# dot-comma-hyphen/oaxaca-blinder-rs

Hardware: NVIDIA B200
Metric: bootstrap_reps_per_sec (higher is better)
Workload: dtype f64

## Files before the change

### include/obboot.h

```cpp
#ifndef OBBOOT_H
#define OBBOOT_H
#include <stddef.h>
#include <stdint.h>

#ifdef __cplusplus
extern "C" {
#endif

#define OBBOOT_ABI_VERSION 6

typedef enum ob_status {
    OB_OK = 0,
    OB_ERR_POLARS = 1,
    OB_ERR_COLUMN_NOT_FOUND = 2,
    OB_ERR_INVALID_GROUP = 3,
    OB_ERR_NALGEBRA = 4,
    OB_ERR_DIAGNOSTIC = 5,
    OB_ERR_INSUFFICIENT_DATA = 6,
    OB_ERR_INVALID_ARG = 7,
    OB_ERR_CUDA = 8,
    OB_ERR_NCCL = 9,
    OB_ERR_NO_DEVICE = 10,
    OB_ERR_UNSUPPORTED = 11
} ob_status;
// ... 133 lines not shown
typedef enum { OB_CACHE_NONE = 0, OB_CACHE_FILLED = 1, OB_CACHE_OUTCOME_ONLY = 2, OB_CACHE_SOLVE_ONLY = 3 } ob_cache_use;
ob_status ob_gram_cache_create(ob_ctx* ctx, ob_gram_cache** out);
void ob_gram_cache_destroy(ob_gram_cache* c);
ob_status ob_gram_cache_last_use(const ob_gram_cache* c, int32_t* use, int64_t* bytes);
ob_status ob_bootstrap_run_cached(ob_ctx* ctx, const ob_design* design, const ob_boot_opts* opts, ob_gram_cache* cache,
                                  ob_result* res);

typedef struct ob_bayes_opts {
    const float* wt_a;
    const float* wt_b;
} ob_bayes_opts;
ob_status ob_bootstrap_run_bayes(ob_ctx* ctx, const ob_design* design, const ob_boot_opts* opts, const ob_bayes_opts* bayes,
                                 ob_gram_cache* cache, ob_result* res);

ob_status ob_reduce_stats(ob_ctx* ctx, const double* rep_stats, const int32_t* rep_status, int64_t reps, int32_t S,
                          const double* point_stats, int64_t* n_ok, double* std_err, double* p_value,
                          double* ci_lower, double* ci_upper, double* t_stat);

typedef struct ob_mm_opts {
    int32_t simulations;
    int32_t n_quantiles;
    const double* quantiles;
    int64_t reps;
    uint64_t seed;
    const uint32_t* idx_a;
    const uint32_t* idx_b;
    const double* taus;
    const uint32_t* draw_a;
    const uint32_t* draw_b;
    int64_t rep_begin;
    int64_t rep_end;
    int32_t skip_reduce;
    int32_t count_bits;
    int64_t max_workspace_bytes;
    int32_t shard_replicates;
} ob_mm_opts;

typedef struct ob_mm_result {
    double* point_stats;
    int64_t n_ok;
    double* std_err;
    double* p_value;
    double* ci_lower;
    double* ci_upper;
    double* t_stat;
    double* rep_stats;
    int32_t* rep_status;
    double* point_betas_a;
    double* point_betas_b;
    int32_t* point_qr_info_a;
    int32_t* point_qr_info_b;
    int64_t qr_total, qr_vertex, qr_approx, qr_failed, qr_iterations;
    double ms_counts, ms_qr, ms_effects, ms_reduce, ms_total;
    int32_t gpu_launches;
} ob_mm_result;

ob_status ob_mm_run(ob_ctx* ctx, const ob_design* design, const ob_mm_opts* opts, ob_mm_result* res);

#define OB_COMM_ID_BYTES 128
ob_status ob_replicate_shard(int64_t reps, int32_t world, int32_t rank, int64_t* rep_begin, int64_t* rep_end);
ob_status ob_comm_unique_id(uint8_t* id128);
ob_status ob_comm_init_nccl(ob_ctx* ctx, const uint8_t* id128, int32_t rank, int32_t world);
typedef struct ob_local_group ob_local_group;
ob_status ob_local_group_create(int32_t world, ob_local_group** out);
void ob_local_group_destroy(ob_local_group* group);
ob_status ob_comm_init_local(ob_ctx* ctx, ob_local_group* group, int32_t rank);
void ob_comm_destroy(ob_ctx* ctx);
ob_status ob_row_shard_plan(int64_t n_group, int32_t world, int32_t rank, int64_t* row_begin, int64_t* row_end);
ob_status ob_design_set_row_shard(ob_design* d, int64_t n_a_global, int64_t n_b_global, int32_t world, int32_t rank);

ob_status ob_design_allgather_rows(ob_ctx* ctx, const ob_design* local_slice, ob_design** out);

ob_status ob_design_row_shard(const ob_design* d, int64_t* n_a_global, int64_t* n_b_global, int32_t* world, int32_t* rank);

ob_status ob_design_redistribute_rows(ob_ctx* ctx, const ob_design* local_slice, ob_design** out);

int64_t ob_debug_gram_schedule(int32_t K, int64_t n_a, int64_t n_b, int64_t slots, int32_t world, int32_t rank, int32_t grid,
                               int64_t* out8, int64_t cap);

int64_t ob_debug_gram_columns(int32_t K, int32_t T, int32_t n_cont, const int32_t* cat_levels, int32_t n_cat,
                              uint16_t* pairs_out, int32_t* colmap_out, int64_t cap, int32_t* tiling_out);
int64_t ob_debug_gram_outcome_columns(int32_t K, int32_t T, uint16_t* pairs_out, int32_t* colmap_out, int64_t cap,
                                      int32_t* tiling_out);

ob_status ob_debug_counts(ob_ctx* ctx, const ob_design* d, uint64_t seed, int64_t rep, int32_t group,
                          uint16_t* counts_out);

ob_status ob_debug_bayes_weights(ob_ctx* ctx, const ob_design* d, uint64_t seed, int64_t rep, int32_t group, float* out);
ob_status ob_debug_counts_from_indices(ob_ctx* ctx, const ob_design* d, int32_t group, const uint32_t* idx, int64_t reps,
                                       int32_t count_bits, uint16_t* counts_out, int32_t* flags_out);

ob_status ob_debug_gram_cache_read(ob_ctx* ctx, const ob_gram_cache* c, int64_t* shape_out, double* xx_out, double* yy_out,
                                   int64_t* rows_out);

#ifdef __cplusplus
}
#endif
#endif
```

### oaxaca_blinder_rs_b200/csrc/api.cu

```cuda
#include "internal.h"

#include <algorithm>
#include <chrono>
#include <cmath>
#include <cstdio>
#include <cstring>
#include <exception>
#include <memory>
#include <atomic>
#include <mutex>
#include <optional>
#include <set>
#include <type_traits>

using namespace ob;

static constexpr int MAX_DESIGN_COLS = 280;

struct ob_ctx {
    int device = 0;
    int num_sms = 0;
    cudaStream_t stream = nullptr;
    cudaStream_t stream_side = nullptr;
    cudaStream_t stream_copy = nullptr;
    static constexpr int PACK_SLOTS = 8;
    int* h_pack_flags = nullptr;
    ob_design* pack_slot_owner[PACK_SLOTS] = {};
    unsigned pack_seq = 0;
    cudaMemPool_t pool = nullptr;
    cudaMemPool_t pool_pack = nullptr;
    cudaMemPool_t pool_design = nullptr;
    std::unique_ptr<Comm> comm;
    std::string err;
    std::mutex designs_mu;
    std::set<ob_design*> designs;
    std::set<ob_gram_cache*> caches;
};

struct ob_local_group { LocalGroup* g = nullptr; int world = 0; };

struct PendingPack;

struct ob_design {
    PendingPack* pending = nullptr;
    ob_status failed = OB_OK;
    std::string fail_msg;
    ob_ctx* owner = nullptr;
    cudaStream_t stream = nullptr;
    int device = 0;
    int K = 0, n_cont = 0, V = 0, ldx = 0;
    int T = 1;
    int K1 = 0;
    std::vector<int> cat_levels;
    bool weighted = false;
    int64_t n_frame = 0;
    int world = 1, rank = 0;
    double ms_h2d = 0.0, ms_pack = 0.0;
    GroupData g[2];
    int cl_strata = OB_CLUSTER_NONE;
    int64_t cl_units[2] = {0, 0};
    uint64_t id = 0, x_gen = 0, y_gen = 0;
};

struct ob_gram_cache {
    ob_ctx* owner = nullptr;
    int device = 0;
    int last_use = OB_CACHE_NONE;
    double* xx = nullptr; size_t xx_bytes = 0;
    double* yy = nullptr; size_t yy_bytes = 0;
    long long* rows = nullptr; size_t rows_bytes = 0;
    double* esum = nullptr; size_t esum_bytes = 0;
    bool xx_ok = false;
    uint64_t design_id = 0, x_gen = 0, seed = 0;
    int64_t reps = 0, rep_begin = 0, rep_end = 0, slots = 0;
    int shard_reps = 0, rep_world = 1, rep_rank = 0, row_world = 1, row_rank = 0, K = 0;
    int count_bytes = 1;
    bool bayes = false;
    bool y_ok = false;
    uint64_t y_gen = 0; int T = 0;
};

namespace {

thread_local ob_ctx* g_alloc_ctx = nullptr;
thread_local bool g_alloc_pack = false;

struct DevBuf {
    void* p = nullptr; size_t bytes = 0;
    ob_ctx* ctx = nullptr;
    bool pack = false;
    DevBuf() : ctx(g_alloc_ctx), pack(g_alloc_pack) {}
    explicit DevBuf(size_t b) : ctx(g_alloc_ctx), pack(g_alloc_pack) { alloc(b); }
    DevBuf(const DevBuf&) = delete;
    DevBuf& operator=(const DevBuf&) = delete;
    DevBuf(DevBuf&& o) noexcept : p(o.p), bytes(o.bytes), ctx(o.ctx), pack(o.pack) { o.p = nullptr; o.bytes = 0; }
    ~DevBuf() { release(); }
    void release() {
        if (p) { cudaFreeAsync(p, ctx->stream); p = nullptr; }
        bytes = 0;
    }
    void alloc(size_t b) {
        release();
        bytes = b;
        if (b) OB_CUDA(cudaMallocFromPoolAsync(&p, b, pack ? ctx->pool_pack : ctx->pool, ctx->stream));
    }
    template <typename T> T* as() const { return static_cast<T*>(p); }
};

struct StagedFrame {
    int64_t n = 0; int n_cont = 0, n_cat = 0;
    std::vector<DevBuf> cols, cats;
    DevBuf y, w, grp;
    bool weighted = false;
    double ms_h2d = 0.0;
};

}

struct PendingPack {
    StagedFrame sf;
    DevBuf d_bc, d_tot, d_flags, d_cont_ptrs, d_cat_ptrs, d_levels, d_dstart;
    std::vector<cudaEvent_t> chunk_done;
    int64_t ready_lo[2] = {0, 0};
    std::vector<int64_t> rows_ready[2];
    bool exchange_pending = false;
    DevBuf EX[2], Ew[2], Esrc[2];
    std::vector<size_t> ex_rows[2], ex_send_row[2], ex_recv_row[2];
    std::vector<long long> ex_frame_off;
    cudaEvent_t ev_begin = nullptr, ev_h2d_end = nullptr;
    int* h_flags = nullptr;
    int slot = -1;
    ~PendingPack() {
        for (cudaEvent_t e : chunk_done) cudaEventDestroy(e);
        if (ev_begin) cudaEventDestroy(ev_begin);
        if (ev_h2d_end) cudaEventDestroy(ev_h2d_end);
    }
};

namespace {

size_t pool_idle_bytes(ob_ctx* ctx) {
    unsigned long long reserved = 0, used = 0;
    cudaMemPoolGetAttribute(ctx->pool, cudaMemPoolAttrReservedMemCurrent, &reserved);
    cudaMemPoolGetAttribute(ctx->pool, cudaMemPoolAttrUsedMemCurrent, &used);
    return reserved > used ? (size_t)(reserved - used) : 0;
}

struct Timer {
    cudaEvent_t a, b; cudaStream_t st; double* acc;
    Timer(cudaStream_t s, double* accum) : st(s), acc(accum) {
        cudaEventCreate(&a); cudaEventCreate(&b); cudaEventRecord(a, st);
    }
    void stop() { cudaEventRecord(b, st); }
    void collect() { float ms = 0; cudaEventSynchronize(b); cudaEventElapsedTime(&ms, a, b); *acc += ms; }
    ~Timer() { cudaEventDestroy(a); cudaEventDestroy(b); }
};

struct Trace {
    bool on; std::chrono::steady_clock::time_point t0, last;
    Trace() : on(getenv("OBBOOT_TRACE") != nullptr), t0(std::chrono::steady_clock::now()), last(t0) {}
    void mark(const char* what, cudaStream_t st = nullptr, bool sync = false) {
        if (!on) return;
        if (sync) cudaStreamSynchronize(st);
        const auto now = std::chrono::steady_clock::now();
        fprintf(stderr, "[obboot] %-28s +%8.3f ms  (t = %9.3f ms)\n", what,
                std::chrono::duration<double, std::milli>(now - last).count(),
                std::chrono::duration<double, std::milli>(now - t0).count());
        last = now;
    }
};

template <typename F>
ob_status guarded(ob_ctx* ctx, F&& f) {
    try {
        if (ctx) OB_CUDA(cudaSetDevice(ctx->device));
        g_alloc_ctx = ctx;
        g_alloc_pack = false;
        f();
        return OB_OK;
    } catch (const CudaError& e) {
        if (ctx) {
            char buf[512];
            snprintf(buf, sizeof buf, "CUDA error: %s (%s) at %s:%d", cudaGetErrorString(e.code), e.what, e.file, e.line);
            ctx->err = buf;
        }
        cudaGetLastError();
        return (e.code == cudaErrorNoDevice || e.code == cudaErrorInsufficientDriver) ? OB_ERR_NO_DEVICE : OB_ERR_CUDA;
    } catch (const StatusError& e) {
        if (ctx) ctx->err = e.msg;
        return e.code;
    } catch (const std::bad_alloc&) {
        if (ctx) ctx->err = "host allocation failed";
        return OB_ERR_INVALID_ARG;
    }
}

[[noreturn]] void fail(ob_status c, const std::string& m) { throw StatusError{c, m}; }

void alloc_group(ob_ctx* ctx, GroupData& g, int64_t n, int ldx, bool weighted, bool zero_all = true) {
    cudaStream_t st = ctx->stream;
    g.n = n; g.n_pad = pad_rows(n);
    g.shard = row_shard(n, 0, 1);
    const size_t xbytes = sizeof(double) * (size_t)g.n_pad * ldx;
    const size_t tail_off = zero_all ? 0 : sizeof(double) * (size_t)n * ldx;
    OB_CUDA(cudaMallocFromPoolAsync((void**)&g.X, xbytes, ctx->pool_design, st));
    OB_CUDA(cudaMemsetAsync(reinterpret_cast<char*>(g.X) + tail_off, 0, xbytes - tail_off, st));
    if (weighted) {
        OB_CUDA(cudaMallocFromPoolAsync((void**)&g.w, sizeof(double) * (size_t)g.n_pad, ctx->pool_design, st));
        OB_CUDA(cudaMemsetAsync(g.w, 0, sizeof(double) * (size_t)g.n_pad, st));
        OB_CUDA(cudaMallocFromPoolAsync((void**)&g.Xs, xbytes, ctx->pool_design, st));
        OB_CUDA(cudaMemsetAsync(reinterpret_cast<char*>(g.Xs) + tail_off, 0, xbytes - tail_off, st));
    }
    OB_CUDA(cudaMallocFromPoolAsync((void**)&g.src, sizeof(uint32_t) * (size_t)g.n_pad, ctx->pool_design, st));
}

void design_register(ob_ctx* ctx, ob_design* d) {
    static std::atomic<uint64_t> next_id{0};
    d->id = ++next_id;
    d->owner = ctx;
    std::lock_guard<std::mutex> lk(ctx->designs_mu);
    ctx->designs.insert(d);
}

void design_release_device(ob_design* d) {
    cudaStream_t st = d->stream;
    for (auto& g : d->g) {
        if (g.X) cudaFreeAsync(g.X, st);
        if (g.w) cudaFreeAsync(g.w, st);
        if (g.Xs) cudaFreeAsync(g.Xs, st);
        if (g.src) cudaFreeAsync(g.src, st);
        if (g.y_raw) cudaFreeAsync(g.y_raw, st);
        if (g.hk_Z) cudaFreeAsync(g.hk_Z, st);
        if (g.hk_sel) cudaFreeAsync(g.hk_sel, st);
        if (g.hk_Xm) cudaFreeAsync(g.hk_Xm, st);
        if (g.uid) cudaFreeAsync(g.uid, st);
        g.X = g.w = g.Xs = g.y_raw = g.hk_Z = g.hk_Xm = nullptr; g.src = g.uid = nullptr; g.hk_sel = nullptr;
    }
}

void cache_release_device(ob_gram_cache* c) {
    if (c->owner) {
        cudaStream_t st = c->owner->stream;
        if (c->xx) cudaFreeAsync(c->xx, st);
        if (c->yy) cudaFreeAsync(c->yy, st);
        if (c->rows) cudaFreeAsync(c->rows, st);
        if (c->esum) cudaFreeAsync(c->esum, st);
    }
    c->xx = c->yy = nullptr; c->rows = nullptr; c->esum = nullptr; c->xx_bytes = c->yy_bytes = c->rows_bytes = c->esum_bytes = 0;
    c->xx_ok = c->y_ok = false;
}

void pending_exchange(ob_design* d) {
    PendingPack* P = d->pending;
    if (!P || !P->exchange_pending) return;
    ob_ctx* ctx = d->owner;
    Comm* comm = ctx->comm.get();
    if (!comm) fail(OB_ERR_NCCL, "the communicator of an asynchronous row-shard pack was destroyed before its exchange");
    cudaStream_t st = ctx->stream;
    const int world = comm->world, me = comm->rank;
    OB_CUDA(cudaStreamWaitEvent(st, P->chunk_done.back(), 0));
    for (int g = 0; g < 2; ++g) {
        GroupData& G = d->g[g];
        auto exchange = [&](const void* sendbuf, void* recvbuf, size_t row_bytes) {
            std::vector<size_t> b(P->ex_rows[g].size()), so((size_t)world), ro((size_t)world);
            for (size_t i = 0; i < b.size(); ++i) b[i] = P->ex_rows[g][i] * row_bytes;
            for (int r = 0; r < world; ++r) { so[r] = P->ex_send_row[g][r] * row_bytes; ro[r] = P->ex_recv_row[g][r] * row_bytes; }
            comm->alltoallv(sendbuf, so.data(), recvbuf, ro.data(), b.data(), st);
        };
        exchange(P->EX[g].p, G.X, sizeof(double) * (size_t)d->ldx);
        if (d->weighted) exchange(P->Ew[g].p, G.w, sizeof(double));
        exchange(P->Esrc[g].p, G.src, sizeof(uint32_t));
        for (int r = 0; r < world; ++r) {
            const int64_t rows = (int64_t)P->ex_rows[g][(size_t)r * world + me];
            if (!rows) continue;
            scale_rows_range_launch(G, d->ldx, (int64_t)P->ex_recv_row[g][r], rows, st);
        }
    }
    OB_CUDA(cudaStreamSynchronize(st));
    P->exchange_pending = false;
}

void pending_finish(ob_design* d, bool quiet = false) {
    PendingPack* P = d->pending;
    if (!P) return;
    ob_ctx* ctx = d->owner;
    if (P->exchange_pending && ctx && !quiet) pending_exchange(d);
    d->pending = nullptr;
    cudaEvent_t last = P->chunk_done.back();
    if (ctx) cudaStreamWaitEvent(ctx->stream, last, 0);
    const cudaError_t e = cudaEventSynchronize(last);
    float ms_all = 0, ms_h2d = 0;
    cudaEventElapsedTime(&ms_all, P->ev_begin, last);
    cudaEventElapsedTime(&ms_h2d, P->ev_begin, P->ev_h2d_end);
    d->ms_h2d = ms_h2d; d->ms_pack = ms_all - ms_h2d;
    const int f0 = P->h_flags[0], f1 = P->h_flags[1];
    if (ctx && P->slot >= 0 && ctx->pack_slot_owner[P->slot] == d) ctx->pack_slot_owner[P->slot] = nullptr;
    g_alloc_ctx = ctx;
    const auto t_del = std::chrono::steady_clock::now();
    delete P;
    if (getenv("OBBOOT_TRACE"))
        fprintf(stderr, "[obboot] async pack: staging released in %.3f ms (host)\n",
                std::chrono::duration<double, std::milli>(std::chrono::steady_clock::now() - t_del).count());
    if (e != cudaSuccess) { d->failed = OB_ERR_CUDA; d->fail_msg = std::string("asynchronous pack failed: ") + cudaGetErrorString(e); }
    else if (f0) { d->failed = OB_ERR_INVALID_GROUP; d->fail_msg = "Invalid group variable: Weights cannot be negative"; }
    else if (f1) { d->failed = OB_ERR_INVALID_ARG; d->fail_msg = "categorical code outside [0, levels)"; }
    if (d->failed != OB_OK && !quiet) fail(d->failed, d->fail_msg);
}

void design_alive(const ob_design* d) {
    if (!d->owner) fail(OB_ERR_INVALID_ARG, "this design's context has been destroyed (designs die with their context)");
    if (d->failed != OB_OK) fail(d->failed, d->fail_msg);
}

void design_ready(const ob_design* d) {
    design_alive(d);
    pending_finish(const_cast<ob_design*>(d));
}

const char* status_text(int s) {
    switch (s) {
    case OB_ERR_INVALID_GROUP: return "Invalid group variable: No data in groups for weighted coefficients.";
    case OB_ERR_NALGEBRA: return "Nalgebra error: Failed to perform Cholesky decomposition. Matrix may be singular or not positive definite due to multicollinearity.";
    case OB_ERR_INSUFFICIENT_DATA: return "Insufficient data: Insufficient data for OLS calculation: n_obs must be strictly greater than k";
    default: return "error";
    }
}


struct RepRange {
    bool shard_reps; int64_t rb, re, nrep;
    bool index_mode; int count_bytes;
};

template <typename Opts>
RepRange replicate_range(const ob_ctx* ctx, const ob_design* d, const Opts* o) {
    if (o->reps < 0) fail(OB_ERR_INVALID_ARG, "negative reps");
    RepRange r;
    r.shard_reps = o->shard_replicates != 0 && ctx->comm && ctx->comm->world > 1;
    if (r.shard_reps && (o->rep_begin != 0 || o->rep_end != 0 || o->skip_reduce))
        fail(OB_ERR_INVALID_ARG, "shard_replicates computes the shard itself: rep_begin / rep_end / skip_reduce must be 0");
    r.rb = o->rep_begin; r.re = o->rep_end > 0 ? o->rep_end : o->reps;
    if (r.rb < 0 || r.re < r.rb || r.re > o->reps) fail(OB_ERR_INVALID_ARG, "bad replicate shard");
    r.nrep = r.re - r.rb;
    r.index_mode = o->idx_a != nullptr || o->idx_b != nullptr;
    if (d->cl_strata == OB_CLUSTER_JOINT) {
        if (o->idx_b) fail(OB_ERR_INVALID_ARG, "a JOINT cluster design takes one unit stream: idx_a [reps x M] and idx_b = NULL");
    } else if (r.index_mode && r.nrep > 0 && (!o->idx_a || !o->idx_b)) fail(OB_ERR_INVALID_ARG, "index stream needs both idx_a and idx_b");
    if (o->count_bits != 0 && o->count_bits != 8 && o->count_bits != 16) fail(OB_ERR_INVALID_ARG, "count_bits must be 0, 8 or 16");
    if (o->count_bits == 16 && !gram_fits(d->ldx, 2)) fail(OB_ERR_UNSUPPORTED, "16-bit multiplicities need K + outcomes <= 268");
    r.count_bytes = o->count_bits == 16 ? 2 : 1;
    return r;
}

struct Batch {
    int64_t pn, slot_lo, slot_hi, bslots;
    int first_slot;
    int64_t brep;
    int64_t rep0;
    Batch(int64_t p0, int64_t ppb, int64_t panels_total, int64_t slots, int64_t rb)
        : pn(std::min(ppb, panels_total - p0)), slot_lo(p0 * BM), slot_hi(std::min(slots, (p0 + pn) * BM)),
          bslots(slot_hi - slot_lo), first_slot(p0 == 0 ? 1 : 0), brep(bslots - first_slot), rep0(rb + slot_lo - 1) {}
    int tail_mi() const {
        const int64_t last = bslots - (pn - 1) * BM;
        return (int)std::min<int64_t>(16, ((last + 7) / 8 + 3) / 4 * 4);
    }
};

struct ClusterWork {
    DevBuf U[2];
    long long* rows = nullptr;
};
int unit_mats(const ob_design* d) { return d->cl_strata == OB_CLUSTER_JOINT ? 1 : 2; }

template <typename Opts>
int generate_counts(const ob_design* d, const Opts* o, const Batch& b, int count_bytes, int64_t ppb, DevBuf (&C)[2],
                    DevBuf (&idx)[2], DevBuf& colsum, DevBuf& lut, int* flags, Comm* row_comm, double* ms_comm, cudaStream_t st,
                    ClusterWork* cw = nullptr) {
    CountsArgs ca[2];
    const int mats = cw ? unit_mats(d) : 2;
    for (int g = 0; g < mats; ++g) {
        const GroupData& G = d->g[g];
        ca[g].C = C[g].p; ca[g].count_bytes = count_bytes; ca[g].n = G.n; ca[g].n_pad = G.n_pad;
        ca[g].n_global = G.shard.n_global; ca[g].row_begin = G.shard.row_begin;
        ca[g].panels = (int)b.pn; ca[g].slots = b.bslots; ca[g].first_slot = b.first_slot; ca[g].rep0 = b.rep0;
        ca[g].group = g; ca[g].seed = o->seed;
        if (cw) {
            const int64_t M = d->cl_units[g];
            ca[g].C = cw->U[g].p; ca[g].n = ca[g].n_global = M; ca[g].n_pad = pad_rows(M); ca[g].row_begin = 0;
            ca[g].group = mats == 1 ? 2 : g;
        }
    }
    int launches = 0;
    auto expand = [&] {
        if (!cw) return;
        OB_CUDA(cudaMemsetAsync(cw->rows, 0, sizeof(long long) * 2 * (size_t)b.pn * BM, st));
        for (int g = 0; g < 2; ++g) {
            const int m = mats == 1 ? 0 : g;
            ExpandArgs ea{C[g].p, cw->U[m].p, d->g[g].uid, count_bytes, d->g[g].n, d->g[g].n_pad, pad_rows(d->cl_units[m]),
                          (int)b.pn, b.bslots, cw->rows + (size_t)g * b.pn * BM};
            counts_expand_launch(ea, st);
            launches += 1;
        }
    };
    if (o->idx_a || o->idx_b) {
        for (int g = 0; g < mats; ++g) {
            const uint32_t* h = g == 0 ? o->idx_a : o->idx_b;
            const int64_t n_glob = ca[g].n_global;
            const size_t nb = sizeof(uint32_t) * (size_t)std::max<int64_t>(b.brep, 1) * n_glob;
            if (idx[g].bytes < nb) idx[g].alloc(nb);
            if (b.brep > 0)
                OB_CUDA(cudaMemcpyAsync(idx[g].p, h + (size_t)(b.rep0 + b.first_slot) * n_glob,
                                        sizeof(uint32_t) * (size_t)b.brep * n_glob, cudaMemcpyHostToDevice, st));
            counts_from_indices(ca[g], idx[g].as<uint32_t>(), flags, st);
            launches += 1 + (b.brep > 0 ? (int)((b.brep + 32767) / 32768) : 0);
        }
        expand();
        return launches;
    }
    long long* sums[2] = {colsum.as<long long>(), colsum.as<long long>() + (size_t)ppb * BM};
    OB_CUDA(cudaMemsetAsync(colsum.p, 0, colsum.bytes, st));
    for (int g = 0; g < mats; ++g) {
        counts_philox_body_launch(ca[g], sums[g], lut.as<unsigned char>() + (size_t)g * counts_lut_bytes(), st);
        launches += 2;
    }
    if (row_comm) {
        Timer t_c(st, ms_comm);
        row_comm->allreduce(colsum.p, 2 * (size_t)ppb * BM, CommDType::I64, CommOp::SUM, st);
        t_c.stop(); OB_CUDA(cudaStreamSynchronize(st)); t_c.collect();
    }
    for (int g = 0; g < mats; ++g) {
        counts_philox_fixup_launch(ca[g], sums[g], flags, st);
        launches += b.brep > 0 ? 1 : 0;
    }
    expand();
    return launches;
}

struct BayesWork {
    DevBuf wt[2], part, esum, esum_local, gathered;
    int ranks_with_rows[2];
};
int generate_weights(const ob_design* d, const ob_boot_opts* o, const ob_bayes_opts* bo, const Batch& b, DevBuf (&C)[2],
                     BayesWork& w, int* flags, Comm* row_comm, double* ms_comm, cudaStream_t st) {
    const int64_t spad = b.pn * BM;
    int segs[2];
    int64_t leaf0 = 0;
    for (int g = 0; g < 2; ++g) {
        const GroupData& G = d->g[g];
        BayesArgs a;
        a.C = C[g].as<float>(); a.n = G.n; a.n_pad = G.n_pad; a.panels = (int)b.pn;
        a.n_global = G.shard.n_global; a.row_begin = G.shard.row_begin;
        a.slots = b.bslots; a.first_slot = b.first_slot; a.rep0 = b.rep0; a.group = g; a.seed = o->seed;
        a.segs = segs[g] = G.shard.leaf_hi - G.shard.leaf_lo; a.seg_rows = G.shard.seg_rows;
        a.wt = nullptr; a.flags = flags;
        a.part = w.part.as<double>() + (size_t)leaf0 * spad;
        leaf0 += a.segs;
        const float* h = bo ? (g == 0 ? bo->wt_a : bo->wt_b) : nullptr;
        if (h) {
            const size_t nb = sizeof(float) * (size_t)std::max<int64_t>(b.brep, 1) * a.n_global;
            if (w.wt[g].bytes < nb) w.wt[g].alloc(nb);
            if (b.brep > 0)
                OB_CUDA(cudaMemcpyAsync(w.wt[g].p, h + (size_t)(b.rep0 + b.first_slot) * a.n_global,
                                        sizeof(float) * (size_t)b.brep * a.n_global, cudaMemcpyHostToDevice, st));
            a.wt = w.wt[g].as<float>();
        }
// ... 1417 lines not shown
            if (rr.shard_reps) {
                Comm* cm = ctx->comm.get();
                ma.betas = allgather_shards(cm, nprob, (size_t)K, d_betas.as<double>() + (size_t)ma.p_begin * K, d_betas_all, st);
                ma.info = allgather_shards(cm, nprob, 1, d_info.as<int>() + ma.p_begin, d_info_all, st);
            }
            Timer t_eff(st, &res->ms_effects);
            mm_effects_launch(ma, d_rows_a.as<uint32_t>(), d_rows_b.as<uint32_t>(), nq, d_q.as<double>(), d_stats.as<double>() + (size_t)b.slot_lo * S,
                              d_status.as<int>() + b.slot_lo, nullptr, st);
            res->gpu_launches += 1;
            t_eff.stop();
            int flags[4];
            h_info.resize((size_t)2 * bslots * sims);
            OB_CUDA(cudaMemcpyAsync(flags, d_flags.p, sizeof flags, cudaMemcpyDeviceToHost, st));
            OB_CUDA(cudaMemcpyAsync(h_info.data(), ma.info, sizeof(int) * h_info.size(), cudaMemcpyDeviceToHost, st));
            if (p0 == 0 && (res->point_betas_a || res->point_betas_b)) {
                h_pbetas.resize((size_t)2 * sims * K);
                OB_CUDA(cudaMemcpyAsync(h_pbetas.data(), ma.betas, sizeof(double) * h_pbetas.size(), cudaMemcpyDeviceToHost, st));
            }
            OB_CUDA(cudaStreamSynchronize(st));
            t_counts.collect(); t_qr.collect(); t_eff.collect();
            saturated = check_batch_flags(flags, count_bytes, o->count_bits, d->ldx);
            if (saturated) break;
            if (p0 == 0 && (res->point_betas_a || res->point_betas_b))
                for (int s_ = 0; s_ < sims; ++s_) {
                    if (res->point_betas_a) memcpy(res->point_betas_a + (size_t)s_ * K, h_pbetas.data() + ((size_t)2 * s_ + 0) * K, sizeof(double) * (size_t)K);
                    if (res->point_betas_b) memcpy(res->point_betas_b + (size_t)s_ * K, h_pbetas.data() + ((size_t)2 * s_ + 1) * K, sizeof(double) * (size_t)K);
                }
            for (size_t i = 0; i < h_info.size(); ++i) {
                const int st_ = h_info[i] & 0xff;
                ++res->qr_total;
                if (st_ == 0) ++res->qr_vertex; else if (st_ == 1) ++res->qr_approx; else ++res->qr_failed;
                res->qr_iterations += (h_info[i] >> 8) & 0xff;
            }
            if (p0 == 0)
                for (int s_ = 0; s_ < sims; ++s_) {
                    if (res->point_qr_info_a) res->point_qr_info_a[s_] = h_info[(size_t)2 * s_];
                    if (res->point_qr_info_b) res->point_qr_info_b[s_] = h_info[(size_t)2 * s_ + 1];
                }
        }
        if (!saturated) break;
        count_bytes = 2;
        res->ms_counts = res->ms_qr = res->ms_effects = 0.0;
        res->qr_total = res->qr_vertex = res->qr_approx = res->qr_failed = res->qr_iterations = 0;
    }
    int point_status = 0;
    OB_CUDA(cudaMemcpyAsync(&point_status, d_status.p, sizeof(int), cudaMemcpyDeviceToHost, st));
    OB_CUDA(cudaStreamSynchronize(st));
    if (point_status != OB_OK)
        fail(OB_ERR_NALGEBRA, "Nalgebra error: Failed to estimate a sufficient number of quantile regressions.");
    };
    agree_on_status(rr.shard_reps ? ctx->comm.get() : nullptr, st, run_batches, "another rank of the replicate-sharded run failed");
    if (res->point_stats) OB_CUDA(cudaMemcpyAsync(res->point_stats, d_stats.p, sizeof(double) * S, cudaMemcpyDeviceToHost, st));
    const int64_t reps_all = rr.nrep;
    const double* stats_rows = d_stats.as<double>() + S;
    const int* status_rows = d_status.as<int>() + 1;
    if (!o->skip_reduce) {
        double* dst[5] = {res->std_err, res->p_value, res->ci_lower, res->ci_upper, res->t_stat};
        reduce_to_host(st, stats_rows, status_rows, reps_all, S, d_stats.as<double>(), dst, &res->n_ok, &res->ms_reduce);
        res->gpu_launches += 1;
    }
    if (reps_all > 0) {
        if (res->rep_stats) OB_CUDA(cudaMemcpyAsync(res->rep_stats, stats_rows, sizeof(double) * (size_t)reps_all * S, cudaMemcpyDeviceToHost, st));
        if (res->rep_status) OB_CUDA(cudaMemcpyAsync(res->rep_status, status_rows, sizeof(int) * (size_t)reps_all, cudaMemcpyDeviceToHost, st));
    }
    t_total.stop();
    OB_CUDA(cudaStreamSynchronize(st));
    t_total.collect();
}

}

extern "C" {

ob_status ob_mm_run(ob_ctx* ctx, const ob_design* d, const ob_mm_opts* o, ob_mm_result* res) {
    if (!ctx || !d || !o || !res) return OB_ERR_INVALID_ARG;
    return guarded(ctx, [&] {
        design_ready(d);
        if (d->cl_strata != OB_CLUSTER_NONE)
            fail(OB_ERR_UNSUPPORTED, "Machado-Mata on a clustered design: its row draws assume constant group sizes (detach the clusters)");
        mm_run(ctx, d, o, res);
    });
}

static void bootstrap_body(ob_ctx* ctx, const ob_design* d, const ob_boot_opts* o, ob_gram_cache* cache, ob_result* res,
                           bool bayes = false, const ob_bayes_opts* bo = nullptr) {
        design_alive(d);
        const bool bayes_explicit = bayes && bo && (bo->wt_a || bo->wt_b);
        if (bayes) {
            if (d->cl_strata != OB_CLUSTER_NONE)
                fail(OB_ERR_UNSUPPORTED, "Bayesian bootstrap on a clustered design: cluster weights are not built (detach the clusters)");
            if (d->K1 > 0)
                fail(OB_ERR_UNSUPPORTED, "Bayesian bootstrap on a design with a selection equation: the Heckman estimator is not built for it");
            if (o->idx_a || o->idx_b)
                fail(OB_ERR_INVALID_ARG, "the Bayesian bootstrap takes no index stream (idx_a / idx_b must be NULL; explicit weights go in ob_bayes_opts)");
            if (o->count_bits != 0) fail(OB_ERR_INVALID_ARG, "the Bayesian bootstrap has fp32 weights: count_bits must be 0");
            if (!gram_fits(d->ldx, 4))
                fail(OB_ERR_UNSUPPORTED, "design too wide for the Bayesian bootstrap: K + outcomes <= 236 with fp32 weights");
            if (cache && bayes_explicit)
                fail(OB_ERR_UNSUPPORTED, "a Gram cache needs the native weight stream (explicit weight streams cannot be keyed)");
        }
        if (cache && d->K1 > 0) fail(OB_ERR_UNSUPPORTED, "a Gram cache does not apply to designs with a selection equation (Heckman)");
        if (cache && (o->idx_a || o->idx_b)) fail(OB_ERR_UNSUPPORTED, "a Gram cache needs the native resampling stream (explicit index streams cannot be keyed)");
        if (d->K1 > 0) {
            design_ready(d);
            heckman_run(ctx, d, o, res);
            return;
        }
        cudaStream_t st = ctx->stream;
        const int K = d->K, T = d->T;
        const bool clustered = d->cl_strata != OB_CLUSTER_NONE;
        if (clustered && d->world > 1)
            fail(OB_ERR_UNSUPPORTED, "clusters on a row-sharded design (mode N): a unit's rows may sit on several ranks");
        if (o->ref_kind < 0 || o->ref_kind > 3) fail(OB_ERR_INVALID_ARG, "ref_kind out of range");
        if (o->n_norm < 0) fail(OB_ERR_INVALID_ARG, "negative n_norm");
        RepRange rr = replicate_range(ctx, d, o);
        if (o->shard_replicates && d->world > 1) fail(OB_ERR_INVALID_ARG, "shard_replicates on a row-sharded design (its communicator shards rows)");
        if (rr.shard_reps) { ob_replicate_shard(o->reps, ctx->comm->world, ctx->comm->rank, &rr.rb, &rr.re); rr.nrep = rr.re - rr.rb; }
        if (d->g[0].shard.n_global == 0 || d->g[1].shard.n_global == 0) fail(OB_ERR_INVALID_GROUP, "Invalid group variable: One group has no data");
        Comm* comm = d->world > 1 ? ctx->comm.get() : nullptr;
        if (d->world > 1 && (!comm || comm->world != d->world || comm->rank != d->rank))
            fail(OB_ERR_NCCL, "row-sharded design needs ob_comm_init_* on this context with the same world/rank");
        const int world = d->world;
        int n_base = 0, n_idx = 0;
        int mode = OB_CACHE_NONE;
        const int rep_world = rr.shard_reps ? ctx->comm->world : 1, rep_rank = rr.shard_reps ? ctx->comm->rank : 0;
        if (cache) {
            const bool xx_hit = cache->xx_ok && cache->design_id == d->id && cache->x_gen == d->x_gen && cache->seed == o->seed &&
                                cache->reps == o->reps && cache->rep_begin == rr.rb && cache->rep_end == rr.re &&
                                cache->shard_reps == (rr.shard_reps ? 1 : 0) && cache->rep_world == rep_world && cache->rep_rank == rep_rank &&
                                cache->row_world == d->world && cache->row_rank == d->rank && cache->K == d->K && cache->bayes == bayes &&
                                !(o->count_bits == 8 && cache->count_bytes == 2);
            mode = !xx_hit ? OB_CACHE_FILLED : (cache->y_ok && cache->y_gen == d->y_gen && cache->T == d->T) ? OB_CACHE_SOLVE_ONLY
                                                                                                           : OB_CACHE_OUTCOME_ONLY;
            if (Comm* ac = rr.shard_reps ? ctx->comm.get() : comm) mode = allreduce_scalar(ac, mode, CommOp::MIN, st);
        }
        const bool solve_only = mode == OB_CACHE_SOLVE_ONLY, outcome_only = mode == OB_CACHE_OUTCOME_ONLY;
        for (int v = 0; v < o->n_norm; ++v) {
            n_base += o->norm_has_base[v] ? 1 : 0;
            if (o->norm_off[v + 1] < o->norm_off[v]) fail(OB_ERR_INVALID_ARG, "norm_off not monotone");
        }
        if (o->n_norm) n_idx = o->norm_off[o->n_norm];
        for (int t = 0; t < n_idx; ++t)
            if (o->norm_idx[t] < 0 || o->norm_idx[t] >= K) fail(OB_ERR_INVALID_ARG, "norm_idx outside the design");
        const int D = K + n_base, S = 5 + 2 * D;
        const int SE = T * S, KE = T * K;
        int count_bytes = bayes ? 4 : rr.count_bytes;
        if (outcome_only && o->count_bits == 0) count_bytes = cache->count_bytes;
        if (bayes && rr.nrep > 0 && bayes_explicit && (!bo->wt_a || !bo->wt_b))
            fail(OB_ERR_INVALID_ARG, "an explicit weight stream needs both wt_a and wt_b");

        res->ms_counts = res->ms_gram = res->ms_solve = res->ms_reduce = res->ms_total = res->ms_gram_kernel = res->ms_comm = 0.0;
        res->gpu_launches = 0;
        res->n_ok = 0;
        Timer t_total(st, &res->ms_total);
        Trace tr;

        const int nn = std::max(o->n_norm, 1);
        DevBuf d_nm(sizeof(int) * nn), d_noff(sizeof(int) * (nn + 1)), d_nidx(sizeof(int) * std::max(n_idx, 1)), d_nhb(sizeof(int) * nn);
        if (o->n_norm) {
            OB_CUDA(cudaMemcpyAsync(d_nm.p, o->norm_m, sizeof(int) * o->n_norm, cudaMemcpyHostToDevice, st));
            OB_CUDA(cudaMemcpyAsync(d_noff.p, o->norm_off, sizeof(int) * (o->n_norm + 1), cudaMemcpyHostToDevice, st));
            if (n_idx) OB_CUDA(cudaMemcpyAsync(d_nidx.p, o->norm_idx, sizeof(int) * n_idx, cudaMemcpyHostToDevice, st));
            OB_CUDA(cudaMemcpyAsync(d_nhb.p, o->norm_has_base, sizeof(int) * o->n_norm, cudaMemcpyHostToDevice, st));
        }

        const int64_t slots = 1 + rr.nrep;
        const bool want_beta = res->rep_beta_a || res->rep_beta_b || res->beta_a || res->beta_b;
        DevBuf d_stats(sizeof(double) * (size_t)slots * SE), d_status(sizeof(int) * (size_t)slots);
        DevBuf d_ba(want_beta ? sizeof(double) * (size_t)slots * KE : 0), d_bb(want_beta ? sizeof(double) * (size_t)slots * KE : 0);
        const size_t PE = 5 * (size_t)K + 1;
        DevBuf d_point(sizeof(double) * PE * T);
        DevBuf d_flags(sizeof(int) * 4);

        const int nx = gram_cache_xx_cells(K), ny = gram_cache_y_cells(K, T);
        size_t cache_new_bytes = 0;
        if (mode == OB_CACHE_FILLED) {
            cache_release_device(cache);
            cache->xx_bytes = sizeof(double) * 2 * (size_t)slots * nx;
            OB_CUDA(cudaMallocFromPoolAsync((void**)&cache->xx, cache->xx_bytes, ctx->pool_design, st));
            cache_new_bytes += cache->xx_bytes;
            if (clustered) {
                cache->rows_bytes = sizeof(long long) * 2 * (size_t)slots;
                OB_CUDA(cudaMallocFromPoolAsync((void**)&cache->rows, cache->rows_bytes, ctx->pool_design, st));
                cache_new_bytes += cache->rows_bytes;
            }
            if (bayes) {
                cache->esum_bytes = sizeof(double) * 2 * (size_t)slots;
                OB_CUDA(cudaMallocFromPoolAsync((void**)&cache->esum, cache->esum_bytes, ctx->pool_design, st));
                cache_new_bytes += cache->esum_bytes;
            }
        }
        if (mode == OB_CACHE_FILLED || outcome_only) {
            cache->y_ok = false;
            const size_t yb = sizeof(double) * 2 * (size_t)slots * ny;
            if (cache->yy_bytes != yb) {
                if (cache->yy) cudaFreeAsync(cache->yy, st);
                cache->yy = nullptr; cache->yy_bytes = yb;
                OB_CUDA(cudaMallocFromPoolAsync((void**)&cache->yy, yb, ctx->pool_design, st));
                cache_new_bytes += yb;
            }
        }

        const GramColumns gcols = solve_only ? GramColumns() : outcome_only ? gram_outcome_columns(K, T)
                                                                              : gram_columns(K, T, d->n_cont, d->cat_levels);
        const int ntiles = gcols.ntiles;
        const int Pld = gram_pld(K, T);
        const int64_t panels_total = (slots + BM - 1) / BM;
        const int64_t n_pad[2] = {d->g[0].n_pad, d->g[1].n_pad};
        const int64_t n_glob[2] = {d->g[0].shard.n_global, d->g[1].shard.n_global};
        const int mats = clustered ? unit_mats(d) : 0;
        int64_t u_pad_all = 0;
        for (int m = 0; m < mats; ++m) u_pad_all += pad_rows(d->cl_units[m]);
        const int64_t idx_len = clustered ? d->cl_units[0] + (mats == 2 ? d->cl_units[1] : 0) : n_glob[0] + n_glob[1];
        int ranks_with_rows[2];
        for (int g = 0; g < 2; ++g)
            ranks_with_rows[g] = (d->g[g].shard.segs + d->g[g].shard.leaf_span - 1) / d->g[g].shard.leaf_span;
        const int64_t local_leaves = (int64_t)(d->g[0].shard.leaf_hi - d->g[0].shard.leaf_lo) +
                                     (d->g[1].shard.leaf_hi - d->g[1].shard.leaf_lo);
        auto per_panel_bytes = [&](int cb) {
            double cl = clustered ? (solve_only ? 0.0 : (double)u_pad_all * BM * cb) + 2.0 * BM * 8.0 : 0.0;
            if (bayes)
                cl = 2.0 * BM * 8.0 + (solve_only ? 0.0 : (double)local_leaves * BM * 8.0 + (comm ? world + 1 : 0) * 2.0 * BM * 8.0 +
                                                          (bayes_explicit ? (double)(n_glob[0] + n_glob[1]) * BM * 4.0 : 0.0));
            if (solve_only) return 2.0 * BM * Pld * 8.0 + cl;
            return (double)(n_pad[0] + n_pad[1]) * BM * cb + (rr.index_mode ? (double)idx_len * BM * 4.0 : 0.0) +
                   2.0 * BM * Pld * 8.0 * (comm ? world + 2 : 1) + (double)local_leaves * ntiles * (BM * BN * 8.0) + 2.0 * BM * 8.0 + cl;
        };
        double budget = (double)o->max_workspace_bytes - (double)cache_new_bytes;
        if (o->max_workspace_bytes <= 0) {
            const double idle = (double)pool_idle_bytes(ctx);
            const double need_all = per_panel_bytes(count_bytes) * (double)panels_total;
            if (idle >= 1.02 * need_all) budget = 1.01 * need_all;
            else {
                size_t free_b = 0, total_b = 0;
                OB_CUDA(cudaMemGetInfo(&free_b, &total_b));
                budget = 0.6 * ((double)free_b + idle) - (double)cache_new_bytes;
            }
        }
        DevBuf d_lut(2 * counts_lut_bytes());

        std::vector<double> point(PE * T);
        cudaEvent_t ev_point = nullptr;
        struct EvGuard { cudaEvent_t& e; ~EvGuard() { if (e) cudaEventDestroy(e); } } ev_point_guard{ev_point};
        OB_CUDA(cudaEventCreateWithFlags(&ev_point, cudaEventDisableTiming));
        auto run_batches = [&] {
        for (int attempt = 0; attempt < 2; ++attempt) {
            const double per_panel = per_panel_bytes(count_bytes);
            int64_t ppb = (int64_t)std::floor(budget / per_panel);
            ppb = std::max<int64_t>(1, std::min<int64_t>(ppb, panels_total));
            if (comm) ppb = allreduce_scalar(comm, (long long)ppb, CommOp::MIN, st);
            tr.mark("setup", st, true);
            DevBuf d_C[2], d_idx[2], d_colsum, d_gram, d_gram_local, d_gathered, d_rows;
            ClusterWork cw;
            BayesWork bw;
            bw.ranks_with_rows[0] = ranks_with_rows[0]; bw.ranks_with_rows[1] = ranks_with_rows[1];
            const size_t gram_elems = 2 * (size_t)ppb * BM * Pld;
            bool saturated = false;
            GramPlan plan; int64_t plan_panels = -1;
            DevBuf d_partials, d_pairs, d_colmap, d_cmap;
            auto allocate_workspace = [&] {
                if (!solve_only) {
                    if (!bayes) d_colsum.alloc(sizeof(long long) * 2 * (size_t)ppb * BM);
                    for (int g = 0; g < 2; ++g) d_C[g].alloc((size_t)ppb * n_pad[g] * BM * count_bytes);
                    for (int m = 0; m < mats; ++m) cw.U[m].alloc((size_t)ppb * pad_rows(d->cl_units[m]) * BM * count_bytes);
                }
                if (clustered) { d_rows.alloc(sizeof(long long) * 2 * (size_t)ppb * BM); cw.rows = d_rows.as<long long>(); }
                if (bayes) {
                    bw.esum.alloc(sizeof(double) * 2 * (size_t)ppb * BM);
                    if (!solve_only) bw.part.alloc(sizeof(double) * (size_t)std::max<int64_t>(local_leaves, 1) * ppb * BM);
                    if (!solve_only && comm) { bw.esum_local.alloc(sizeof(double) * 2 * (size_t)ppb * BM); bw.gathered.alloc(sizeof(double) * 2 * (size_t)ppb * BM * world); }
                }
                d_gram.alloc(sizeof(double) * gram_elems);
                if (cache) {
                    const std::vector<int32_t> cmap = gram_cache_map(K, T);
                    d_cmap.alloc(sizeof(int32_t) * cmap.size());
                    OB_CUDA(cudaMemcpyAsync(d_cmap.p, cmap.data(), sizeof(int32_t) * cmap.size(), cudaMemcpyHostToDevice, st));
                }
                if (solve_only) { OB_CUDA(cudaStreamSynchronize(st)); return; }
                if (comm) { d_gram_local.alloc(sizeof(double) * gram_elems); d_gathered.alloc(sizeof(double) * gram_elems * world); }
                plan = gram_make_plan(K, T, d->ldx, (int)std::min<int64_t>(ppb, panels_total), d->g, count_bytes, ctx->num_sms, gcols);
                plan_panels = plan.panels;
                d_partials.alloc(sizeof(double) * (size_t)std::max<int64_t>(plan.num_partials, 1) * BM * BN);
                d_pairs.alloc(sizeof(uint16_t) * gcols.pairs.size());
                d_colmap.alloc(sizeof(int32_t) * gcols.colmap.size());
                OB_CUDA(cudaMemcpyAsync(d_pairs.p, gcols.pairs.data(), sizeof(uint16_t) * gcols.pairs.size(), cudaMemcpyHostToDevice, st));
                OB_CUDA(cudaMemcpyAsync(d_colmap.p, gcols.colmap.data(), sizeof(int32_t) * gcols.colmap.size(), cudaMemcpyHostToDevice, st));
                OB_CUDA(cudaStreamSynchronize(st));
            };
            agree_on_status(comm, st, allocate_workspace, "another rank of the row-sharded run could not allocate its workspace");

            tr.mark("workspace + pair table", st, true);
            for (int64_t p0 = 0; p0 < panels_total && !saturated; p0 += ppb) {
                const Batch b(p0, ppb, panels_total, slots, rr.rb);
                const int64_t pn = b.pn, bslots = b.bslots;
                OB_CUDA(cudaMemsetAsync(d_flags.p, 0, sizeof(int) * 4, st));

                Timer t_counts(st, &res->ms_counts);
                if (!solve_only && bayes)
                    res->gpu_launches += generate_weights(d, o, bo, b, d_C, bw, d_flags.as<int>(), comm, &res->ms_comm, st);
                else if (!solve_only)
                    res->gpu_launches += generate_counts(d, o, b, count_bytes, ppb, d_C, d_idx, d_colsum, d_lut, d_flags.as<int>(), comm,
                                                         &res->ms_comm, st, clustered ? &cw : nullptr);
                t_counts.stop();
                tr.mark("counts", st, true);

                if (!solve_only && plan_panels != pn) {
                    plan = gram_make_plan(K, T, d->ldx, (int)pn, d->g, count_bytes, ctx->num_sms, gcols);
                    plan_panels = pn;
                    d_partials.alloc(sizeof(double) * (size_t)std::max<int64_t>(plan.num_partials, 1) * BM * BN);
                }
                Timer t_gram(st, &res->ms_gram);
                GramArgs ga;
                for (int g = 0; g < 2; ++g) { ga.X[g] = d->g[g].gram_operand(); ga.C[g] = d_C[g].p; }
                ga.count_bytes = count_bytes; ga.partials = d_partials.as<double>();
                ga.d_pairs = d_pairs.as<uint16_t>(); ga.d_colmap = d_colmap.as<int32_t>();
                ga.gram = comm ? d_gram_local.as<double>() : d_gram.as<double>();
                ga.tail_mi = b.tail_mi();
                struct EventPair {
                    cudaEvent_t a = nullptr, b = nullptr;
                    EventPair() { OB_CUDA(cudaEventCreate(&a)); OB_CUDA(cudaEventCreate(&b)); }
                    ~EventPair() { if (a) cudaEventDestroy(a); if (b) cudaEventDestroy(b); }
                } ev;
                ob_design* dm = const_cast<ob_design*>(d);
                if (solve_only) {
                    OB_CUDA(cudaEventRecord(ev.a, st));
                    OB_CUDA(cudaMemsetAsync(d_gram.p, 0, sizeof(double) * 2 * (size_t)pn * BM * Pld, st));
                    OB_CUDA(cudaEventRecord(ev.b, st));
                } else if (PendingPack* P = dm->pending) {
                    int la[2] = {0, 0}, na[2] = {0, 0};
                    const bool split = P->chunk_done.size() > 1;
                    for (int g = 0; g < 2; ++g) {
                        if (!split || plan.segs[g] == 0) continue;
                        const int64_t sr = plan.seg_rows[g];
                        const int64_t lo = (P->ready_lo[g] + sr - 1) / sr, hi = std::min<int64_t>(plan.segs[g], P->rows_ready[g][0] / sr);
                        if (hi > lo) { la[g] = (int)lo; na[g] = (int)(hi - lo); }
                    }
                    EventPair evA, evB;
                    OB_CUDA(cudaEventRecord(ev.a, st));
                    if (na[0] + na[1] > 0) {
                        OB_CUDA(cudaStreamWaitEvent(st, P->chunk_done.front(), 0));
                        if (tr.on) OB_CUDA(cudaEventRecord(evA.a, st));
                        gram_launch_leaves(plan, ga, la, na, st);
                        if (tr.on) OB_CUDA(cudaEventRecord(evA.b, st));
                        res->gpu_launches += 1;
                    }
                    OB_CUDA(cudaStreamWaitEvent(st, P->chunk_done.back(), 0));
                    pending_exchange(dm);
                    if (tr.on) OB_CUDA(cudaEventRecord(evB.a, st));
                    {
                        int lo0[2] = {0, 0}, n0[2] = {na[0] ? la[0] : 0, na[1] ? la[1] : 0};
                        int lo1[2] = {la[0] + na[0], la[1] + na[1]}, n1[2] = {plan.segs[0] - lo1[0], plan.segs[1] - lo1[1]};
                        if (n0[0] + n0[1] > 0) { gram_launch_leaves(plan, ga, lo0, n0, st); res->gpu_launches += 1; }
                        gram_launch_leaves(plan, ga, lo1, n1, st);
                    }
                    OB_CUDA(cudaEventRecord(ev.b, st));
                    gram_reduce_launch(plan, ga, st);
                    res->gpu_launches += 2;
                    if (tr.on) {
                        OB_CUDA(cudaEventSynchronize(ev.b));
                        auto rel = [&](cudaEvent_t e) { float ms = -1.f; if (cudaEventElapsedTime(&ms, P->ev_begin, e) != cudaSuccess) { cudaGetLastError(); ms = -1.f; } return ms; };
                        fprintf(stderr, "[obboot] async pack (ms after its start): chunk 0 packed %.1f, upload done %.1f, all packed %.1f | "
                                        "first gram launch %.1f..%.1f (leaves %d+%d of %d+%d), rest %.1f..%.1f\n",
                                rel(P->chunk_done.front()), rel(P->ev_h2d_end), rel(P->chunk_done.back()), rel(evA.a), rel(evA.b), na[0], na[1],
                                plan.segs[0], plan.segs[1], rel(evB.a), rel(ev.b));
                    }
                    pending_finish(dm);
                } else {
                    gram_launch(plan, ga, st, ev.a, ev.b);
                    res->gpu_launches += 2;
                }
                t_gram.stop();
                tr.mark("gram", st, true);
                if (comm && !solve_only) {
                    Timer t_c(st, &res->ms_comm);
                    const size_t batch_elems = 2 * (size_t)pn * BM * Pld;
                    comm->allgather(d_gram_local.p, d_gathered.p, sizeof(double) * batch_elems, st);
                    gram_combine_launch(d_gathered.as<double>(), world, ranks_with_rows, (int64_t)pn * BM * Pld, d_gram.as<double>(), st);
                    res->gpu_launches += 1;
                    t_c.stop(); OB_CUDA(cudaStreamSynchronize(st)); t_c.collect();
                }
                if (cache) {
                    Timer t_cc(st, &res->ms_gram);
                    GramCacheCopy cc{d_gram.as<double>(), pn * BM, Pld, b.slot_lo, bslots, cache->xx, cache->yy, slots,
                                     d_cmap.as<int32_t>(), nx, ny, 0, nx + ny};
                    for (int g = 0; clustered && g < 2 && (mode == OB_CACHE_FILLED || solve_only); ++g) {
                        long long* batch_rows = d_rows.as<long long>() + (size_t)g * pn * BM;
                        long long* kept = cache->rows + (size_t)g * slots + b.slot_lo;
                        OB_CUDA(cudaMemcpyAsync(solve_only ? batch_rows : kept, solve_only ? kept : batch_rows, sizeof(long long) * (size_t)bslots,
                                                cudaMemcpyDeviceToDevice, st));
                    }
                    for (int g = 0; bayes && g < 2 && (mode == OB_CACHE_FILLED || solve_only); ++g) {
                        double* batch_esum = bw.esum.as<double>() + (size_t)g * pn * BM;
                        double* kept = cache->esum + (size_t)g * slots + b.slot_lo;
                        OB_CUDA(cudaMemcpyAsync(solve_only ? batch_esum : kept, solve_only ? kept : batch_esum, sizeof(double) * (size_t)bslots,
                                                cudaMemcpyDeviceToDevice, st));
                    }
                    if (mode == OB_CACHE_FILLED) gram_cache_extract_launch(cc, st);
                    else if (solve_only) gram_cache_assemble_launch(cc, st);
                    else {
                        cc.c_hi = nx; gram_cache_assemble_launch(cc, st);
                        cc.c_lo = nx; cc.c_hi = nx + ny; gram_cache_extract_launch(cc, st);
                        res->gpu_launches += 1;
                    }
                    res->gpu_launches += 1;
                    t_cc.stop(); OB_CUDA(cudaStreamSynchronize(st)); t_cc.collect();
                }

                Timer t_solve(st, &res->ms_solve);
                SolveArgs sa;
                sa.gram = d_gram.as<double>(); sa.slots_pad = pn * BM; sa.Pld = Pld; sa.slots = bslots;
                sa.K = K; sa.n_cont = d->n_cont; sa.ref_kind = o->ref_kind; sa.T = T;
                sa.n_norm = o->n_norm; sa.d_norm_m = d_nm.as<int>(); sa.d_norm_off = d_noff.as<int>();
                sa.d_norm_idx = d_nidx.as<int>(); sa.d_norm_has_base = d_nhb.as<int>();
                sa.n_base = n_base; sa.S = S; sa.weighted = d->weighted ? 1 : 0;
                sa.na = (double)n_glob[0]; sa.nb = (double)n_glob[1];
                sa.rows = clustered ? d_rows.as<long long>() : nullptr;
                sa.esum = bayes ? bw.esum.as<double>() : nullptr;
                sa.stats = d_stats.as<double>() + (size_t)b.slot_lo * SE;
                sa.status = d_status.as<int>() + b.slot_lo;
                sa.beta_a = want_beta ? d_ba.as<double>() + (size_t)b.slot_lo * KE : nullptr;
                sa.beta_b = want_beta ? d_bb.as<double>() + (size_t)b.slot_lo * KE : nullptr;
                sa.point_extra = (p0 == 0) ? d_point.as<double>() : nullptr;
                DevBuf d_solve_scratch(solve_scratch_bytes(K, o->ref_kind == OB_REF_POOLED, o->n_norm, T, bslots));
                sa.scratch = d_solve_scratch.as<double>();
                solve_launch(sa, st);
                res->gpu_launches += 1;
                t_solve.stop();

                if (comm) comm->allreduce(d_flags.p, 4, CommDType::I32, CommOp::MAX, st);
                int flags[4];
                OB_CUDA(cudaMemcpyAsync(flags, d_flags.p, sizeof flags, cudaMemcpyDeviceToHost, st));
                OB_CUDA(cudaStreamSynchronize(st));
                tr.mark("solve + flags", st, false);
                t_counts.collect(); t_gram.collect(); t_solve.collect();
                { float ms = 0; cudaEventElapsedTime(&ms, ev.a, ev.b); res->ms_gram_kernel += ms; }
                saturated = check_batch_flags(flags, count_bytes, o->count_bits, d->ldx);
            }
            if (!saturated) break;
            count_bytes = 2;
            res->ms_counts = res->ms_gram = res->ms_solve = res->ms_gram_kernel = res->ms_comm = 0.0;
        }

        tr.mark("batches done (buffers freed)", st, true);
        int point_status = 0;
        OB_CUDA(cudaMemcpyAsync(&point_status, d_status.p, sizeof(int), cudaMemcpyDeviceToHost, st));
        OB_CUDA(cudaMemcpyAsync(point.data(), d_point.p, sizeof(double) * point.size(), cudaMemcpyDeviceToHost, st));
        OB_CUDA(cudaStreamSynchronize(st));
        if (point_status != OB_OK) fail((ob_status)point_status, status_text(point_status));
        };

        agree_on_status(rr.shard_reps ? ctx->comm.get() : nullptr, st, run_batches, "another rank of the replicate-sharded run failed");
        if (cache) {
            if (mode == OB_CACHE_FILLED) {
                cache->design_id = d->id; cache->x_gen = d->x_gen; cache->seed = o->seed;
                cache->reps = o->reps; cache->rep_begin = rr.rb; cache->rep_end = rr.re; cache->slots = slots;
                cache->shard_reps = rr.shard_reps ? 1 : 0; cache->rep_world = rep_world; cache->rep_rank = rep_rank;
                cache->row_world = d->world; cache->row_rank = d->rank; cache->K = K; cache->count_bytes = count_bytes;
                cache->bayes = bayes;
                cache->xx_ok = true;
            }
            if (!solve_only) { cache->y_gen = d->y_gen; cache->T = T; cache->y_ok = true; }
            cache->last_use = mode;
        }
        res->total_gap = point[5 * K];
        if (res->xa_mean) memcpy(res->xa_mean, point.data(), sizeof(double) * K);
        if (res->xb_mean) memcpy(res->xb_mean, point.data() + K, sizeof(double) * K);
        for (int t = 0; t < T; ++t) {
            if (res->beta_star) memcpy(res->beta_star + (size_t)t * K, point.data() + t * PE + 2 * K, sizeof(double) * K);
            if (res->total_gap_multi) res->total_gap_multi[t] = point[t * PE + 5 * K];
        }

        DevBuf d_res;
        struct SideJoin { cudaStream_t s; bool armed = false; ~SideJoin() { if (armed) cudaStreamSynchronize(s); } } side_join{ctx->stream_side};
        if (res->residuals_b) {
            side_join.armed = true;
            d_res.alloc(sizeof(double) * (size_t)std::max<int64_t>(d->g[1].n, 1) * T);
            cudaStream_t s2 = ctx->stream_side;
            OB_CUDA(cudaEventRecord(ev_point, st));
            OB_CUDA(cudaStreamWaitEvent(s2, ev_point, 0));
            for (int t = 0; t < T; ++t)
                residuals_launch(d->g[1], K, K + t, d->ldx, d_point.as<double>() + t * PE + 4 * K, d_res.as<double>() + (size_t)t * d->g[1].n, s2);
            res->gpu_launches += T;
            if (d->g[1].n) OB_CUDA(cudaMemcpyAsync(res->residuals_b, d_res.p, sizeof(double) * (size_t)d->g[1].n * T, cudaMemcpyDeviceToHost, s2));
        }
        if (res->point_stats) OB_CUDA(cudaMemcpyAsync(res->point_stats, d_stats.p, sizeof(double) * SE, cudaMemcpyDeviceToHost, st));
        if (res->beta_a) OB_CUDA(cudaMemcpyAsync(res->beta_a, d_ba.p, sizeof(double) * KE, cudaMemcpyDeviceToHost, st));
        if (res->beta_b) OB_CUDA(cudaMemcpyAsync(res->beta_b, d_bb.p, sizeof(double) * KE, cudaMemcpyDeviceToHost, st));
        tr.mark("point + residuals queued", st, false);

        const int64_t reps_all = rr.shard_reps ? o->reps : rr.nrep;
        DevBuf d_gstats, d_gstatus, d_gba, d_gbb;
        const double* stats_rows = d_stats.as<double>() + SE;
        const int* status_rows = d_status.as<int>() + 1;
        const double* ba_rows = want_beta ? d_ba.as<double>() + KE : nullptr;
        const double* bb_rows = want_beta ? d_bb.as<double>() + KE : nullptr;
        if (rr.shard_reps) {
            Timer t_c(st, &res->ms_comm);
            Comm* cm = ctx->comm.get();
            stats_rows = allgather_shards(cm, o->reps, SE, stats_rows, d_gstats, st);
            status_rows = allgather_shards(cm, o->reps, 1, status_rows, d_gstatus, st);
            if (res->rep_beta_a) ba_rows = allgather_shards(cm, o->reps, KE, ba_rows, d_gba, st);
            if (res->rep_beta_b) bb_rows = allgather_shards(cm, o->reps, KE, bb_rows, d_gbb, st);
            t_c.stop(); OB_CUDA(cudaStreamSynchronize(st)); t_c.collect();
            tr.mark("replicate all-gather", st, false);
        }

        if (!o->skip_reduce) {
            double* dst[5] = {res->std_err, res->p_value, res->ci_lower, res->ci_upper, res->t_stat};
            reduce_to_host(st, stats_rows, status_rows, reps_all, SE, d_stats.as<double>(), dst, &res->n_ok, &res->ms_reduce);
            res->gpu_launches += 1;
        }
        if (reps_all > 0) {
            if (res->rep_stats) OB_CUDA(cudaMemcpyAsync(res->rep_stats, stats_rows, sizeof(double) * (size_t)reps_all * SE, cudaMemcpyDeviceToHost, st));
            if (res->rep_status) OB_CUDA(cudaMemcpyAsync(res->rep_status, status_rows, sizeof(int) * (size_t)reps_all, cudaMemcpyDeviceToHost, st));
            if (res->rep_beta_a) OB_CUDA(cudaMemcpyAsync(res->rep_beta_a, ba_rows, sizeof(double) * (size_t)reps_all * KE, cudaMemcpyDeviceToHost, st));
            if (res->rep_beta_b) OB_CUDA(cudaMemcpyAsync(res->rep_beta_b, bb_rows, sizeof(double) * (size_t)reps_all * KE, cudaMemcpyDeviceToHost, st));
        }
        if (res->residuals_b) {
            OB_CUDA(cudaEventRecord(ev_point, ctx->stream_side));
            OB_CUDA(cudaStreamWaitEvent(st, ev_point, 0));
        }
        t_total.stop();
        OB_CUDA(cudaStreamSynchronize(st));
        t_total.collect();
        tr.mark("reduce + replicate D2H", st, false);
}

ob_status ob_bootstrap_run(ob_ctx* ctx, const ob_design* d, const ob_boot_opts* o, ob_result* res) {
    if (!ctx || !d || !o || !res) return OB_ERR_INVALID_ARG;
    return guarded(ctx, [&] { bootstrap_body(ctx, d, o, nullptr, res); });
}

ob_status ob_gram_cache_create(ob_ctx* ctx, ob_gram_cache** out) {
    if (!ctx || !out) return OB_ERR_INVALID_ARG;
    auto* c = new ob_gram_cache;
    c->owner = ctx; c->device = ctx->device;
    {
        std::lock_guard<std::mutex> lk(ctx->designs_mu);
        ctx->caches.insert(c);
    }
    *out = c;
// ... 29 lines not shown
        if (cache->owner != ctx) fail(OB_ERR_INVALID_ARG, "this Gram cache belongs to another context");
        try {
            bootstrap_body(ctx, d, o, cache, res);
        } catch (...) {
            cache_release_device(cache);
            cache->last_use = OB_CACHE_NONE;
            throw;
        }
    });
}

ob_status ob_bootstrap_run_bayes(ob_ctx* ctx, const ob_design* d, const ob_boot_opts* o, const ob_bayes_opts* bo,
                                 ob_gram_cache* cache, ob_result* res) {
    if (!ctx || !d || !o || !res) return OB_ERR_INVALID_ARG;
    return guarded(ctx, [&] {
        if (!cache) { bootstrap_body(ctx, d, o, nullptr, res, true, bo); return; }
        if (cache->owner != ctx) fail(OB_ERR_INVALID_ARG, "this Gram cache belongs to another context");
        try {
            bootstrap_body(ctx, d, o, cache, res, true, bo);
        } catch (...) {
            cache_release_device(cache);
            cache->last_use = OB_CACHE_NONE;
            throw;
        }
    });
}

ob_status ob_reduce_stats(ob_ctx* ctx, const double* rep_stats, const int32_t* rep_status, int64_t reps, int32_t S,
                          const double* point_stats, int64_t* n_ok, double* std_err, double* p_value,
                          double* ci_lower, double* ci_upper, double* t_stat) {
    if (!ctx || S < 1 || reps < 0 || !point_stats || (reps && (!rep_stats || !rep_status))) return OB_ERR_INVALID_ARG;
    return guarded(ctx, [&] {
        cudaStream_t st = ctx->stream;
        DevBuf d_stats(sizeof(double) * (size_t)std::max<int64_t>(reps, 1) * S), d_status(sizeof(int) * (size_t)std::max<int64_t>(reps, 1));
        DevBuf d_point(sizeof(double) * S);
        if (reps) {
            OB_CUDA(cudaMemcpyAsync(d_stats.p, rep_stats, sizeof(double) * (size_t)reps * S, cudaMemcpyHostToDevice, st));
            OB_CUDA(cudaMemcpyAsync(d_status.p, rep_status, sizeof(int) * (size_t)reps, cudaMemcpyHostToDevice, st));
        }
        OB_CUDA(cudaMemcpyAsync(d_point.p, point_stats, sizeof(double) * S, cudaMemcpyHostToDevice, st));
        double* dst[5] = {std_err, p_value, ci_lower, ci_upper, t_stat};
        reduce_to_host(st, d_stats.as<double>(), d_status.as<int>(), reps, S, d_point.as<double>(), dst, n_ok, nullptr);
    });
}

int64_t ob_debug_gram_columns(int32_t K, int32_t T, int32_t n_cont, const int32_t* cat_levels, int32_t n_cat,
                              uint16_t* pairs_out, int32_t* colmap_out, int64_t cap, int32_t* tiling_out) {
    if (K < 1 || T < 1 || n_cont < 0 || n_cat < 0 || (n_cat > 0 && !cat_levels) || K + T > 65535) return -1;
    const GramColumns gc = gram_columns(K, T, n_cont, std::vector<int>(cat_levels, cat_levels + n_cat));
    const int64_t len = (int64_t)gc.colmap.size();
    for (int64_t c = 0; c < len && c < cap; ++c) {
        if (pairs_out) { pairs_out[2 * c] = gc.pairs[2 * (size_t)c]; pairs_out[2 * c + 1] = gc.pairs[2 * (size_t)c + 1]; }
        if (colmap_out) colmap_out[c] = gc.colmap[(size_t)c];
    }
    if (tiling_out) { tiling_out[0] = gc.Pc; tiling_out[1] = gc.nfull; tiling_out[2] = gc.tail_q; }
    return len;
}

int64_t ob_debug_gram_outcome_columns(int32_t K, int32_t T, uint16_t* pairs_out, int32_t* colmap_out, int64_t cap,
                                      int32_t* tiling_out) {
    if (K < 1 || T < 1 || K + T > 65535) return -1;
    const GramColumns gc = gram_outcome_columns(K, T);
    const int64_t len = (int64_t)gc.colmap.size();
    for (int64_t c = 0; c < len && c < cap; ++c) {
        if (pairs_out) { pairs_out[2 * c] = gc.pairs[2 * (size_t)c]; pairs_out[2 * c + 1] = gc.pairs[2 * (size_t)c + 1]; }
        if (colmap_out) colmap_out[c] = gc.colmap[(size_t)c];
    }
    if (tiling_out) { tiling_out[0] = gc.Pc; tiling_out[1] = gc.nfull; tiling_out[2] = gc.tail_q; }
    return len;
}

int64_t ob_debug_gram_schedule(int32_t K, int64_t n_a, int64_t n_b, int64_t slots, int32_t world, int32_t rank, int32_t grid,
                               int64_t* out8, int64_t cap) {
    if (K < 1 || n_a < 0 || n_b < 0 || slots < 1 || world < 1 || (world & (world - 1)) || world > MAX_WORLD || rank < 0 ||
        rank >= world || grid < 1) return -1;
    GroupData gd[2];
    const int64_t ns[2] = {n_a, n_b};
    for (int g = 0; g < 2; ++g) {
        gd[g].shard = row_shard(ns[g], rank, world);
        gd[g].n = gd[g].shard.n_local; gd[g].n_pad = pad_rows(gd[g].n);
    }
    const int64_t panels = (slots + BM - 1) / BM;
    return gram_schedule_debug(K, (int)panels, slots - (panels - 1) * BM, gd, grid, out8, cap);
}

ob_status ob_debug_counts(ob_ctx* ctx, const ob_design* d, uint64_t seed, int64_t rep, int32_t group,
                          uint16_t* counts_out) {
    if (!ctx || !d || !counts_out || group < 0 || group > 1 || rep < 0) return OB_ERR_INVALID_ARG;
    return guarded(ctx, [&] {
        design_ready(d);
        cudaStream_t st = ctx->stream;
        const GroupData& G = d->g[group];
        DevBuf d_C((size_t)G.n_pad * BM * 2), d_colsum(sizeof(long long) * BM), d_flags(sizeof(int) * 4), d_lut(counts_lut_bytes());
        OB_CUDA(cudaMemsetAsync(d_flags.p, 0, sizeof(int) * 4, st));
        CountsArgs ca;
        ca.C = d_C.p; ca.count_bytes = 2; ca.n = G.n; ca.n_pad = G.n_pad; ca.panels = 1; ca.slots = 2;
        ca.first_slot = 1; ca.rep0 = rep - 1; ca.group = group; ca.seed = seed;
        ca.n_global = G.shard.n_global; ca.row_begin = G.shard.row_begin;
        if (d->world > 1) fail(OB_ERR_UNSUPPORTED, "ob_debug_counts on a row-sharded design");
        DevBuf d_U, d_rows;
        const int m = d->cl_strata == OB_CLUSTER_JOINT ? 0 : group;
        if (d->cl_strata != OB_CLUSTER_NONE) {
            const int64_t M = d->cl_units[m];
            d_U.alloc((size_t)pad_rows(M) * BM * 2);
            d_rows.alloc(sizeof(long long) * 2 * BM);
            ca.C = d_U.p; ca.n = ca.n_global = M; ca.n_pad = pad_rows(M); ca.row_begin = 0;
            ca.group = d->cl_strata == OB_CLUSTER_JOINT ? 2 : group;
        }
        OB_CUDA(cudaMemsetAsync(d_colsum.p, 0, d_colsum.bytes, st));
        counts_philox_body_launch(ca, d_colsum.as<long long>(), d_lut.as<unsigned char>(), st);
        counts_philox_fixup_launch(ca, d_colsum.as<long long>(), d_flags.as<int>(), st);
        if (d->cl_strata != OB_CLUSTER_NONE) {
            OB_CUDA(cudaMemsetAsync(d_rows.p, 0, d_rows.bytes, st));
            ExpandArgs ea{d_C.p, d_U.p, G.uid, 2, G.n, G.n_pad, ca.n_pad, 1, 2, d_rows.as<long long>()};
            counts_expand_launch(ea, st);
        }
        OB_CUDA(cudaMemcpy2DAsync(counts_out, sizeof(uint16_t), d_C.as<uint16_t>() + 1, sizeof(uint16_t) * BM,
                                  sizeof(uint16_t), (size_t)G.n, cudaMemcpyDeviceToHost, st));
        OB_CUDA(cudaStreamSynchronize(st));
    });
}

ob_status ob_debug_bayes_weights(ob_ctx* ctx, const ob_design* d, uint64_t seed, int64_t rep, int32_t group, float* out) {
    if (!ctx || !d || !out || group < 0 || group > 1 || rep < 0) return OB_ERR_INVALID_ARG;
    return guarded(ctx, [&] {
        design_ready(d);
        if (d->world > 1) fail(OB_ERR_UNSUPPORTED, "ob_debug_bayes_weights on a row-sharded design");
        cudaStream_t st = ctx->stream;
        const GroupData& G = d->g[group];
        const int segs = G.shard.leaf_hi - G.shard.leaf_lo;
        DevBuf d_C((size_t)G.n_pad * BM * sizeof(float)), d_part(sizeof(double) * (size_t)std::max(segs, 1) * BM);
        BayesArgs a;
        a.C = d_C.as<float>(); a.n = G.n; a.n_pad = G.n_pad; a.panels = 1;
        a.n_global = G.shard.n_global; a.row_begin = G.shard.row_begin;
        a.slots = 2; a.first_slot = 1; a.rep0 = rep - 1; a.group = group; a.seed = seed;
        a.segs = segs; a.seg_rows = G.shard.seg_rows; a.wt = nullptr; a.part = d_part.as<double>();
        bayes_weights_launch(a, st);
        OB_CUDA(cudaMemcpy2DAsync(out, sizeof(float), d_C.as<float>() + 1, sizeof(float) * BM, sizeof(float), (size_t)G.n,
                                  cudaMemcpyDeviceToHost, st));
        OB_CUDA(cudaStreamSynchronize(st));
    });
}

ob_status ob_debug_counts_from_indices(ob_ctx* ctx, const ob_design* d, int32_t group, const uint32_t* idx, int64_t reps,
                                       int32_t count_bits, uint16_t* counts_out, int32_t* flags_out) {
    if (!ctx || !d || !counts_out || group < 0 || group > 1 || reps < 0 || (reps && !idx) || (count_bits != 8 && count_bits != 16))
        return OB_ERR_INVALID_ARG;
    return guarded(ctx, [&] {
        design_ready(d);
        cudaStream_t st = ctx->stream;
        const GroupData& G = d->g[group];
        const int cb = count_bits / 8;
        const int64_t slots = 1 + reps, panels = (slots + BM - 1) / BM;
        const int64_t n_glob = G.shard.n_global;
        DevBuf d_C((size_t)panels * G.n_pad * BM * cb), d_flags(sizeof(int) * 4);
        DevBuf d_idx(sizeof(uint32_t) * (size_t)std::max<int64_t>(reps * n_glob, 1));
        OB_CUDA(cudaMemsetAsync(d_flags.p, 0, sizeof(int) * 4, st));
        if (reps) OB_CUDA(cudaMemcpyAsync(d_idx.p, idx, sizeof(uint32_t) * (size_t)reps * n_glob, cudaMemcpyHostToDevice, st));
        CountsArgs ca;
        ca.C = d_C.p; ca.count_bytes = cb; ca.n = G.n; ca.n_pad = G.n_pad; ca.panels = (int)panels; ca.slots = slots;
        ca.first_slot = 1; ca.rep0 = -1; ca.group = group; ca.seed = 0;
        ca.n_global = n_glob; ca.row_begin = G.shard.row_begin;
        counts_from_indices(ca, d_idx.as<uint32_t>(), d_flags.as<int>(), st);
        std::vector<uint8_t> h((size_t)panels * G.n_pad * BM * cb);
        int flags[4];
        OB_CUDA(cudaMemcpyAsync(h.data(), d_C.p, h.size(), cudaMemcpyDeviceToHost, st));
// ... 38 lines not shown
```

### oaxaca_blinder_rs_b200/csrc/gram.cu

```cuda
#include "common.cuh"
#include "internal.h"

#include <algorithm>
#include <cstdlib>
#include <type_traits>

namespace ob {

constexpr int LGS = 18;
constexpr int LDA2 = 148;
constexpr int A_TILE = KT * LDA2;

struct GramKernelParams {
    const double* X[2];
    const void* C[2];
    long long n_pad[2];
    int segs[2];
    int seg_lo[2], seg_n[2];
    int seg_rows[2];
    long long units0;
    long long units_total;
    int ldx, panels, ntiles;
    int nfull, tail_q;
    int tail_mi;
    double* partials;
    const uint16_t* pairs;
};

template <typename CountT>
__device__ __forceinline__ double count_to_f64(CountT c, const double* __restrict__ tab) {
    if constexpr (std::is_same<CountT, float>::value) {
        const uint32_t f = __float_as_uint(c);
        return __hiloint2double(f ? (int)((f >> 3) + (896u << 20)) : 0, (int)(f << 29));
    } else if constexpr (sizeof(CountT) == 1) {
        return tab[(unsigned)c];
    } else {
        return __hiloint2double(0x43300000, (int)(unsigned)c) - 4503599627370496.0;
    }
}

constexpr int WS_R = 3;
constexpr int WS_PRODUCER_WARPS = 4;
constexpr int WS_THREADS = GRAM_THREADS + 32 * WS_PRODUCER_WARPS;
#define OB_WS_CONSUMER_REGS 224
#define OB_WS_PRODUCER_REGS 56

struct GramUnit { const double* Xg; const void* Cg; double* out; int nstages, nt, mi, tq; };

__host__ __device__ __forceinline__ bool ws_decode(const GramKernelParams& p, long long i, int ldx, size_t count_bytes, GramUnit& u) {
    const int pt = p.tail_mi < 16 ? 1 : 0, pf = p.panels - pt;
    const long long segs01 = (long long)p.seg_n[0] + p.seg_n[1];
    const long long n0 = segs01 * pf * p.nfull, n1 = segs01 * pt * p.nfull;
    const long long n2 = p.tail_q ? segs01 * pf : 0, n3 = p.tail_q ? segs01 * pt : 0;
    if (i >= n0 + n1 + n2 + n3) return false;
    int np, p0, nt_cnt, nt0;
    if (i < n0) { np = pf; p0 = 0; nt_cnt = p.nfull; nt0 = 0; }
    else if ((i -= n0) < n1) { np = pt; p0 = pf; nt_cnt = p.nfull; nt0 = 0; }
    else if ((i -= n1) < n2) { np = pf; p0 = 0; nt_cnt = 1; nt0 = p.nfull; }
    else { i -= n2; np = pt; p0 = pf; nt_cnt = 1; nt0 = p.nfull; }
    const long long per_seg = (long long)np * nt_cnt;
    const long long g0 = (long long)p.seg_n[0] * per_seg;
    const int g = i >= g0 ? 1 : 0;
    const long long r = i - (g ? g0 : 0);
    const int sidx = (int)(r / per_seg);
    const long long r2 = r - (long long)sidx * per_seg;
    const int seg = (g ? p.seg_lo[1] : p.seg_lo[0]) + sidx;
    const int panel = p0 + (int)(r2 / nt_cnt), nt = nt0 + (int)(r2 % nt_cnt);
    const int segs = g ? p.segs[1] : p.segs[0], seg_rows = g ? p.seg_rows[1] : p.seg_rows[0];
    const long long n_pad = g ? p.n_pad[1] : p.n_pad[0];
    const long long row0 = (long long)seg * seg_rows;
    const long long row1 = row0 + seg_rows < n_pad ? row0 + seg_rows : n_pad;
    u.nstages = (int)((row1 - row0) / KT);
    u.nt = nt; u.tq = (p.tail_q && nt == p.nfull) ? p.tail_q : 4;
    u.mi = panel >= pf ? p.tail_mi : 16;
    u.Xg = (g ? p.X[1] : p.X[0]) + row0 * ldx;
    u.Cg = reinterpret_cast<const unsigned char*>(g ? p.C[1] : p.C[0]) + (((long long)panel * n_pad + row0) * BM) * (long long)count_bytes;
    u.out = p.partials + (size_t)((g ? p.units0 : 0) + ((long long)panel * segs + seg) * p.ntiles + nt) * (BM * BN);
    return true;
}

template <typename CountT, int LDXC, int NI, int MI, int R>
__device__ __forceinline__ void ws_consume_unit(const GramKernelParams& p, const GramUnit& u, const double* As, const double* Xs,
                                                uint64_t* full, uint64_t* ready, uint64_t* consumed, int ldx_rt, uint32_t& jc,
                                                int sub0, int tw) {
    constexpr int KSTEPS = KT / 4;
    const int lane = threadIdx.x & 31;
    const int lk = lane & 3, lg = lane >> 2;
    const int ldx = LDXC ? LDXC : ldx_rt;
    int oj[NI], ol[NI];
#pragma unroll
    for (int s = 0; s < NI; ++s) {
        const int col = u.nt * BN + (sub0 + s) * 8 + lg;
        const uint32_t pr = *reinterpret_cast<const uint32_t*>(p.pairs + 2 * col);
        oj[s] = pr & 0xFFFFu; ol[s] = pr >> 16;
    }
    double acc[MI][NI][2];
#pragma unroll
    for (int i = 0; i < MI; ++i)
#pragma unroll
        for (int s = 0; s < NI; ++s) { acc[i][s][0] = 0.0; acc[i][s][1] = 0.0; }

    for (int s = 0; s < u.nstages; ++s) {
        const uint32_t slot = jc % R, par = (jc / R) & 1u;
        mbar_wait(&full[slot], par);
        mbar_wait(&ready[slot], par);
        const double* abase = As + (size_t)slot * A_TILE + lk * LDA2 + lg * LGS;
        const double* xbase = Xs + (size_t)slot * KT * ldx + lk * ldx;
#pragma unroll
        for (int kk = 0; kk < KSTEPS; ++kk) {
            double a[MI], b[NI];
            const double* arow = abase + kk * 4 * LDA2;
            const double* xrow = xbase + kk * 4 * ldx;
#pragma unroll
            for (int i = 0; i < MI; i += 2) {
                const double2 v = *reinterpret_cast<const double2*>(arow + i);
                a[i] = v.x; a[i + 1] = v.y;
            }
#pragma unroll
            for (int t = 0; t < NI; ++t) b[t] = xrow[oj[t]] * xrow[ol[t]];
#pragma unroll
            for (int i = 0; i < MI; ++i)
#pragma unroll
                for (int t = 0; t < NI; ++t) dmma884(acc[i][t][0], acc[i][t][1], a[i], b[t]);
        }
        __syncwarp();
        if (lane == 0) mbar_arrive(&consumed[slot]);
        ++jc;
    }
#pragma unroll
    for (int i = 0; i < MI; ++i)
#pragma unroll
        for (int t = 0; t < NI; ++t) {
            const int m = i * 8 + lg, n = (sub0 + t) * 8 + 2 * lk;
            *reinterpret_cast<double2*>(u.out + m * tw + n) = make_double2(acc[i][t][0], acc[i][t][1]);
        }
}

template <typename CountT, int LDXC, int NI, int R>
__device__ __forceinline__ void ws_consume_dispatch(const GramKernelParams& p, const GramUnit& u, const double* As, const double* Xs,
                                                    uint64_t* full, uint64_t* ready, uint64_t* consumed, int ldx_rt, uint32_t& jc,
                                                    int sub0, int tw) {
    switch (u.mi) {
    case 4: ws_consume_unit<CountT, LDXC, NI, 4, R>(p, u, As, Xs, full, ready, consumed, ldx_rt, jc, sub0, tw); break;
    case 8: ws_consume_unit<CountT, LDXC, NI, 8, R>(p, u, As, Xs, full, ready, consumed, ldx_rt, jc, sub0, tw); break;
    case 12: ws_consume_unit<CountT, LDXC, NI, 12, R>(p, u, As, Xs, full, ready, consumed, ldx_rt, jc, sub0, tw); break;
    default: ws_consume_unit<CountT, LDXC, NI, 16, R>(p, u, As, Xs, full, ready, consumed, ldx_rt, jc, sub0, tw); break;
    }
}

template <int R>
__device__ __forceinline__ void ws_idle_unit(const GramUnit& u, uint64_t* full, uint64_t* consumed, uint32_t& jc) {
    const int lane = threadIdx.x & 31;
    for (int s = 0; s < u.nstages; ++s) {
        const uint32_t slot = jc % R, par = (jc / R) & 1u;
        mbar_wait(&full[slot], par);
        __syncwarp();
        if (lane == 0) mbar_arrive(&consumed[slot]);
        ++jc;
    }
}
// ... 57 lines not shown
        while (is_ok && ji < (uint32_t)R) issue_next();
        while (wi_ok) {
            const uint32_t slot = jw % R, par = (jw / R) & 1u;
            mbar_wait(&full[slot], par);
            {
                const CountT* src = Cr + (size_t)slot * KT * BM;
                double* dst = As + (size_t)slot * A_TILE;
#pragma unroll 4
                for (int it = lane; it < (KT / WS_PRODUCER_WARPS) * 8 * 8; it += 32) {
                    const int e = it >> 6, rem = it & 63, r = pw * (KT / WS_PRODUCER_WARPS) + (rem >> 3), lgq = rem & 7;
                    const CountT* sp = src + r * BM + lgq;
                    double2 o;
                    o.x = count_to_f64<CountT>(sp[e * 16], Tab);
                    o.y = count_to_f64<CountT>(sp[e * 16 + 8], Tab);
                    *reinterpret_cast<double2*>(dst + r * LDA2 + lgq * LGS + e * 2) = o;
                }
            }
            __syncwarp();
            if (lane == 0) mbar_arrive(&ready[slot]);
            ++jw;
            if (++wi_s == wi_u.nstages) { wi_s = 0; wi_i += gridDim.x; wi_ok = ws_decode(p, wi_i, ldx, sizeof(CountT), wi_u); }
            if (is_ok && ji <= jw + (uint32_t)(R - 2)) {
                const uint32_t prev = ji - R;
                if (pw == 0) mbar_wait(&consumed[prev % R], (prev / R) & 1u);
                issue_next();
            }
        }
    }
}

static constexpr size_t gram_ws_smem(int ldx, int count_bytes, int ring = WS_R) {
    return sizeof(double) * ((size_t)ring * A_TILE + 256 + (size_t)ring * KT * ldx) + (size_t)ring * KT * BM * count_bytes +
           sizeof(uint64_t) * 3 * ring;
}
constexpr size_t GRAM_SMEM_MAX = 227 * 1024;
constexpr int gram_ring_f32(int ldx) { return gram_ws_smem(ldx, 4, WS_R) <= GRAM_SMEM_MAX ? WS_R : 2; }

bool gram_fits(int ldx, int count_bytes) { return gram_ws_smem(ldx, count_bytes, 2) <= GRAM_SMEM_MAX; }

template <int LEN>
__device__ __forceinline__ double2 tree_sum(const double2* __restrict__ base, size_t stride, int lo, int cnt);

__device__ __noinline__ double2 tree_sum64_call(const double2* __restrict__ base, size_t stride, int lo, int cnt);

template <int LEN>
__device__ __forceinline__ double2 tree_sum(const double2* __restrict__ base, size_t stride, int lo, int cnt) {
    if constexpr (LEN == 1) {
        return base[(size_t)lo * stride];
    } else if constexpr (LEN == 128) {
        double2 a = tree_sum64_call(base, stride, lo, cnt);
        if (lo + 64 < cnt) {
            const double2 b = tree_sum64_call(base, stride, lo + 64, cnt);
            a.x += b.x; a.y += b.y;
        }
        return a;
    } else {
        double2 a = tree_sum<LEN / 2>(base, stride, lo, cnt);
        if (lo + LEN / 2 < cnt) {
            const double2 b = tree_sum<LEN / 2>(base, stride, lo + LEN / 2, cnt);
            a.x += b.x; a.y += b.y;
        }
        return a;
    }
}

__device__ __noinline__ double2 tree_sum64_call(const double2* __restrict__ base, size_t stride, int lo, int cnt) {
    return tree_sum<64>(base, stride, lo, cnt);
}

__device__ __forceinline__ double2 tree_sum_span(const double2* __restrict__ base, size_t stride, int cnt, int span) {
    switch (span) {
    case 256: return tree_sum<256>(base, stride, 0, cnt);
    case 128: return tree_sum<128>(base, stride, 0, cnt);
    case 64: return tree_sum<64>(base, stride, 0, cnt);
    case 32: return tree_sum<32>(base, stride, 0, cnt);
    case 16: return tree_sum<16>(base, stride, 0, cnt);
    case 8: return tree_sum<8>(base, stride, 0, cnt);
    case 4: return tree_sum<4>(base, stride, 0, cnt);
    case 2: return tree_sum<2>(base, stride, 0, cnt);
    default: return tree_sum<1>(base, stride, 0, cnt);
    }
}

__global__ void __launch_bounds__(256) gram_reduce_kernel(const double* __restrict__ partials, int segs0, int segs1,
                                                          double* __restrict__ gram, int panels, int ntiles, int span,
                                                          int Pld, int tail_q, const int32_t* __restrict__ colmap) {
    const int tile_id = blockIdx.x;
    const int tiles_g = panels * ntiles;
    const int g = tile_id / tiles_g, t = tile_id - g * tiles_g;
    const int panel = t / ntiles, nt = t - panel * ntiles;
    const int cnt = g ? segs1 : segs0;
    const size_t first = (g ? (size_t)tiles_g * segs0 : 0) + (size_t)panel * cnt * ntiles + nt;
    const size_t slots_pad = (size_t)panels * BM;
    const int tw = (tail_q && nt == ntiles - 1) ? tail_q * BQ : BN;
    for (int e = threadIdx.x + blockIdx.y * blockDim.x; e < BM * tw / 2; e += blockDim.x * gridDim.y) {
        double2 s = make_double2(0.0, 0.0);
        if (cnt > 0) s = tree_sum_span(reinterpret_cast<const double2*>(partials + first * (BM * BN)) + e, (size_t)ntiles * (BM * BN / 2), cnt, span);
        const int m = (2 * e) / tw, n = (2 * e) % tw;
        double* dst = gram + ((size_t)g * slots_pad + (size_t)panel * BM + m) * (size_t)Pld;
        const int c0 = colmap[nt * BN + n], c1 = colmap[nt * BN + n + 1];
        if (c0 >= 0) dst[c0] = s.x;
        if (c1 >= 0) dst[c1] = s.y;
    }
}

__global__ void __launch_bounds__(256) leaf_sum_kernel(const double* __restrict__ part, int segs0, int segs1, long long half,
                                                       int span, double* __restrict__ out) {
    for (long long e = (long long)blockIdx.x * blockDim.x + threadIdx.x; e < 2 * half; e += (long long)gridDim.x * blockDim.x) {
        const int g = e >= half ? 1 : 0;
        const int cnt = g ? segs1 : segs0;
        const double2* base = reinterpret_cast<const double2*>(part + (g ? (size_t)segs0 * 2 * half : 0)) + (e - (g ? half : 0));
        reinterpret_cast<double2*>(out)[e] = cnt > 0 ? tree_sum_span(base, (size_t)half, cnt, span) : make_double2(0.0, 0.0);
    }
}

__global__ void __launch_bounds__(256) gram_combine_kernel(const double* __restrict__ gathered, int world, int ranks0,
                                                           int ranks1, long long per_group2, double* __restrict__ gram) {
    const long long total = 2 * per_group2;
    for (long long e = (long long)blockIdx.x * blockDim.x + threadIdx.x; e < total; e += (long long)gridDim.x * blockDim.x) {
        const int g = e >= per_group2 ? 1 : 0;
        const int cnt = g ? ranks1 : ranks0;
        double2 s = make_double2(0.0, 0.0);
        if (cnt > 0) s = tree_sum_span(reinterpret_cast<const double2*>(gathered) + e, (size_t)total, cnt, world);
        reinterpret_cast<double2*>(gram)[e] = s;
    }
}

GramColumns gram_columns(int K, int T, int n_cont, const std::vector<int>& cat_levels) {
    std::vector<int> block((size_t)K, -1);
    {
        int64_t dummies = 0;
        for (int m : cat_levels) dummies += m > 1 ? m - 1 : 0;
        if (!cat_levels.empty() && 1 + (int64_t)n_cont + dummies == K) {
            int c = 1 + n_cont;
            for (size_t q = 0; q < cat_levels.size(); ++q)
                for (int lvl = 1; lvl < cat_levels[q]; ++lvl) block[(size_t)c++] = (int)q;
        }
    }
    GramColumns gc;
    std::vector<uint16_t> pj, pl; std::vector<int32_t> cm;
    for (int j = 0; j < K; ++j) {
        const int64_t base = pair_base(K, T, j);
        for (int l = j; l < K; ++l) {
            if (l > j && block[(size_t)j] >= 0 && block[(size_t)j] == block[(size_t)l]) continue;
            pj.push_back((uint16_t)j); pl.push_back((uint16_t)l); cm.push_back((int32_t)(base + (l - j)));
        }
        for (int o = 0; o < T; ++o) { pj.push_back((uint16_t)j); pl.push_back((uint16_t)(K + o)); cm.push_back((int32_t)(base + (K - j) + o)); }
    }
    pj.push_back((uint16_t)K); pl.push_back((uint16_t)K); cm.push_back((int32_t)(num_pairs(K, T) - 1));
    gc.Pc = (int)cm.size();
    gram_col_tiling(gc.Pc, gc.nfull, gc.tail_q);
    gc.ntiles = gc.nfull + (gc.tail_q > 0);
    const size_t cols = (size_t)gc.ntiles * BN;
    gc.pairs.assign(cols * 2, (uint16_t)K);
    gc.colmap.assign(cols, -1);
    for (size_t c = 0; c < cm.size(); ++c) { gc.pairs[2 * c] = pj[c]; gc.pairs[2 * c + 1] = pl[c]; gc.colmap[c] = cm[c]; }
    return gc;
}

GramColumns gram_outcome_columns(int K, int T) {
    GramColumns gc;
    std::vector<uint16_t> pj, pl; std::vector<int32_t> cm;
    for (int j = 0; j < K; ++j) {
        const int64_t base = pair_base(K, T, j);
        for (int o = 0; o < T; ++o) { pj.push_back((uint16_t)j); pl.push_back((uint16_t)(K + o)); cm.push_back((int32_t)(base + (K - j) + o)); }
    }
    pj.push_back((uint16_t)K); pl.push_back((uint16_t)K); cm.push_back((int32_t)(num_pairs(K, T) - 1));
    gc.Pc = (int)cm.size();
    gram_col_tiling(gc.Pc, gc.nfull, gc.tail_q);
    gc.ntiles = gc.nfull + (gc.tail_q > 0);
    const size_t cols = (size_t)gc.ntiles * BN;
    gc.pairs.assign(cols * 2, (uint16_t)K);
    gc.colmap.assign(cols, -1);
    for (size_t c = 0; c < cm.size(); ++c) { gc.pairs[2 * c] = pj[c]; gc.pairs[2 * c + 1] = pl[c]; gc.colmap[c] = cm[c]; }
    return gc;
}

std::vector<int32_t> gram_cache_map(int K, int T) {
    std::vector<int32_t> m;
    m.reserve((size_t)gram_cache_xx_cells(K) + gram_cache_y_cells(K, T));
    for (int j = 0; j < K; ++j)
        for (int l = j; l < K; ++l) m.push_back((int32_t)(pair_base(K, T, j) + (l - j)));
    for (int j = 0; j < K; ++j)
        for (int o = 0; o < T; ++o) m.push_back((int32_t)(pair_base(K, T, j) + (K - j) + o));
    m.push_back((int32_t)(num_pairs(K, T) - 1));
    return m;
}

template <bool TO_CACHE>
__device__ __forceinline__ void gram_cache_copy_cells(const GramCacheCopy& a) {
    const long long ncell = a.c_hi - a.c_lo, per_g = a.nslots * ncell, total = 2 * per_g;
    for (long long e = (long long)blockIdx.x * blockDim.x + threadIdx.x; e < total; e += (long long)gridDim.x * blockDim.x) {
        const int g = e >= per_g ? 1 : 0;
        const long long r = e - (g ? per_g : 0);
        const long long s = r / ncell;
        const int c = a.c_lo + (int)(r - s * ncell);
        double* gcell = a.gram + ((size_t)g * a.slots_pad + (size_t)s) * (size_t)a.Pld + a.map[c];
        const size_t slot = (size_t)g * a.cslots + (size_t)(a.slot_lo + s);
        double* ccell = c < a.nx ? a.xx + slot * a.nx + c : a.yy + slot * a.ny + (c - a.nx);
        if (TO_CACHE) *ccell = *gcell; else *gcell = *ccell;
    }
}
__global__ void __launch_bounds__(256) gram_cache_extract_kernel(const GramCacheCopy a) { gram_cache_copy_cells<true>(a); }
__global__ void __launch_bounds__(256) gram_cache_assemble_kernel(const GramCacheCopy a) { gram_cache_copy_cells<false>(a); }

static void gram_cache_copy(const GramCacheCopy& a, bool to_cache, cudaStream_t st) {
    const long long total = 2 * a.nslots * (long long)(a.c_hi - a.c_lo);
    if (total <= 0) return;
    const unsigned blocks = (unsigned)std::min<long long>((total + 255) / 256, 148 * 8);
    if (to_cache) gram_cache_extract_kernel<<<blocks, 256, 0, st>>>(a);
    else gram_cache_assemble_kernel<<<blocks, 256, 0, st>>>(a);
    OB_CUDA(cudaGetLastError());
}
void gram_cache_extract_launch(const GramCacheCopy& a, cudaStream_t st) { gram_cache_copy(a, true, st); }
void gram_cache_assemble_launch(const GramCacheCopy& a, cudaStream_t st) { gram_cache_copy(a, false, st); }

GramPlan gram_make_plan(int K, int T, int ldx, int panels, const GroupData gd[2], int count_bytes, int num_sms,
                        const GramColumns& cols) {
    GramPlan pl;
    pl.K = K; pl.T = T; pl.ldx = ldx; pl.panels = panels;
    pl.nfull = cols.nfull; pl.tail_q = cols.tail_q; pl.ntiles = cols.ntiles;
    pl.Pld = gram_pld(K, T);
    int64_t total = 0;
    pl.leaf_span = gd[0].shard.leaf_span;
    for (int g = 0; g < 2; ++g) {
        pl.n_pad[g] = gd[g].n_pad;
        pl.segs[g] = gd[g].shard.leaf_hi - gd[g].shard.leaf_lo;
        pl.seg_rows[g] = gd[g].shard.seg_rows;
        pl.units[g] = (int64_t)pl.segs[g] * panels * pl.ntiles;
        total += pl.units[g];
    }
    pl.grid = (int)std::min<int64_t>(num_sms, std::max<int64_t>(total, 1));
    pl.ring = gram_ws_smem(pl.ldx, count_bytes, WS_R) <= GRAM_SMEM_MAX ? WS_R : 2;
    pl.smem_bytes = gram_ws_smem(pl.ldx, count_bytes, pl.ring);
    pl.num_partials = (int64_t)total;
    return pl;
}

static GramKernelParams gram_params(const GramPlan& pl, const GramArgs& a, const int seg_lo[2], const int seg_n[2]) {
    GramKernelParams p;
    for (int g = 0; g < 2; ++g) {
        p.X[g] = a.X[g]; p.C[g] = a.C[g];
        p.n_pad[g] = pl.n_pad[g]; p.segs[g] = pl.segs[g]; p.seg_rows[g] = pl.seg_rows[g];
        p.seg_lo[g] = seg_lo ? seg_lo[g] : 0; p.seg_n[g] = seg_n ? seg_n[g] : pl.segs[g];
    }
    p.units0 = pl.units[0];
    p.units_total = pl.units[0] + pl.units[1];
    p.ldx = pl.ldx; p.panels = pl.panels; p.ntiles = pl.ntiles;
    p.nfull = pl.nfull; p.tail_q = pl.tail_q;
    p.partials = a.partials; p.pairs = a.d_pairs;
    p.tail_mi = a.tail_mi >= 1 && a.tail_mi <= 16 ? a.tail_mi : 16;
    return p;
}

void gram_launch_leaves(const GramPlan& pl, const GramArgs& a, const int seg_lo[2], const int seg_n[2], cudaStream_t st) {
    const GramKernelParams p = gram_params(pl, a, seg_lo, seg_n);
    const int64_t units = ((int64_t)p.seg_n[0] + p.seg_n[1]) * pl.panels * pl.ntiles;
    if (units <= 0) return;
    const int grid = (int)std::min<int64_t>(pl.grid, units);
    const size_t ws_smem = pl.smem_bytes;
    if (!gram_fits(pl.ldx, a.count_bytes))
        throw StatusError{OB_ERR_UNSUPPORTED, "design too wide for the Gram kernel's shared-memory ring (K + outcomes <= 280 with "
                                              "8-bit multiplicities, <= 268 with 16-bit, <= 236 with fp32 Bayesian weights)"};
    auto launch_ws = [&](auto kernel) {
        OB_CUDA(cudaFuncSetAttribute(kernel, cudaFuncAttributeMaxDynamicSharedMemorySize, (int)ws_smem));
        kernel<<<grid, WS_THREADS, ws_smem, st>>>(p);
    };
#define OB_GRAM_WS_CASE(L) case L: if (a.count_bytes == 4) launch_ws(gram_ws_kernel<float, L, gram_ring_f32(L)>); \
                                   else if (a.count_bytes == 1) launch_ws(gram_ws_kernel<uint8_t, L>); else launch_ws(gram_ws_kernel<uint16_t, L>); break;
    switch (pl.ldx) {
        OB_GRAM_WS_CASE(12) OB_GRAM_WS_CASE(20) OB_GRAM_WS_CASE(28) OB_GRAM_WS_CASE(36) OB_GRAM_WS_CASE(44) OB_GRAM_WS_CASE(52)
        OB_GRAM_WS_CASE(60) OB_GRAM_WS_CASE(68) OB_GRAM_WS_CASE(76) OB_GRAM_WS_CASE(84) OB_GRAM_WS_CASE(92)
        default:
            if (a.count_bytes == 4) { if (pl.ring == WS_R) launch_ws(gram_ws_kernel<float, 0, WS_R>); else launch_ws(gram_ws_kernel<float, 0, 2>); }
            else if (pl.ring == WS_R) { if (a.count_bytes == 1) launch_ws(gram_ws_kernel<uint8_t, 0, WS_R>); else launch_ws(gram_ws_kernel<uint16_t, 0, WS_R>); }
            else { if (a.count_bytes == 1) launch_ws(gram_ws_kernel<uint8_t, 0, 2>); else launch_ws(gram_ws_kernel<uint16_t, 0, 2>); }
    }
#undef OB_GRAM_WS_CASE
    OB_CUDA(cudaGetLastError());
}

void gram_reduce_launch(const GramPlan& pl, const GramArgs& a, cudaStream_t st) {
    OB_CUDA(cudaMemsetAsync(a.gram, 0, sizeof(double) * 2 * (size_t)pl.panels * BM * (size_t)pl.Pld, st));
    dim3 rgw(2 * pl.panels * pl.ntiles, 16);
    gram_reduce_kernel<<<rgw, 256, 0, st>>>(a.partials, pl.segs[0], pl.segs[1], a.gram, pl.panels, pl.ntiles, pl.leaf_span,
                                            pl.Pld, pl.tail_q, a.d_colmap);
    OB_CUDA(cudaGetLastError());
}

void gram_launch(const GramPlan& pl, const GramArgs& a, cudaStream_t st, cudaEvent_t ev_main_begin, cudaEvent_t ev_main_end) {
    if (ev_main_begin) OB_CUDA(cudaEventRecord(ev_main_begin, st));
    gram_launch_leaves(pl, a, nullptr, nullptr, st);
    if (ev_main_end) OB_CUDA(cudaEventRecord(ev_main_end, st));
    gram_reduce_launch(pl, a, st);
}

void leaf_sum_launch(const double* part, const int segs[2], int64_t slots_pad, int span, double* out, cudaStream_t st) {
    const long long half = slots_pad / 2;
    const unsigned blocks = (unsigned)std::min<long long>((2 * half + 255) / 256, 148 * 8);
    leaf_sum_kernel<<<std::max(blocks, 1u), 256, 0, st>>>(part, segs[0], segs[1], half, span, out);
    OB_CUDA(cudaGetLastError());
}

void gram_combine_launch(const double* gathered, int world, const int ranks_with_rows[2], int64_t per_group_elems,
                         double* gram, cudaStream_t st) {
    const long long per2 = per_group_elems / 2;
    const unsigned blocks = (unsigned)std::min<long long>((2 * per2 + 255) / 256, 148 * 8);
    gram_combine_kernel<<<std::max(blocks, 1u), 256, 0, st>>>(gathered, world, ranks_with_rows[0], ranks_with_rows[1], per2, gram);
    OB_CUDA(cudaGetLastError());
}

int64_t gram_schedule_debug(int K, int panels, int64_t slots_last_panel, const GroupData gd[2], int grid, int64_t* out7, int64_t cap) {
    const GramColumns cols = gram_columns(K, 1, K - 1, std::vector<int>());
    GramPlan pl = gram_make_plan(K, 1, design_ldx(K + 1), panels, gd, 1, grid, cols);
    GramKernelParams p{};
    for (int g = 0; g < 2; ++g) { p.n_pad[g] = pl.n_pad[g]; p.segs[g] = pl.segs[g]; p.seg_rows[g] = pl.seg_rows[g]; p.seg_lo[g] = 0; p.seg_n[g] = pl.segs[g]; }
    p.units0 = pl.units[0]; p.units_total = pl.units[0] + pl.units[1];
    p.ldx = pl.ldx; p.panels = pl.panels; p.ntiles = pl.ntiles; p.nfull = pl.nfull; p.tail_q = pl.tail_q;
    p.tail_mi = (int)std::min<int64_t>(16, ((slots_last_panel + 7) / 8 + 3) / 4 * 4);
    p.partials = nullptr;
    int64_t count = 0;
    for (int b = 0; b < grid; ++b) {
        GramUnit u;
        for (long long i = b; ws_decode(p, i, pl.ldx, 1, u); i += grid) {
            if (count < cap) {
                const long long idx = (long long)(u.out - (double*)nullptr) / (BM * BN);
                const int g = idx >= p.units0 ? 1 : 0;
                const long long r = idx - (g ? p.units0 : 0);
                const int segs = p.segs[g];
                const long long sweep = r / p.ntiles;
                int64_t* o = out7 + 8 * count;
                o[0] = b; o[1] = g; o[2] = sweep / segs; o[3] = r % p.ntiles; o[4] = sweep % segs; o[5] = u.nstages; o[6] = u.mi; o[7] = u.tq < 4 ? u.tq : 0;
            }
            ++count;
        }
    }
    return count;
}

}
```

### oaxaca_blinder_rs_b200/csrc/internal.h

```cpp
#pragma once
#include <cstdint>
#include <cuda_runtime.h>
#include <string>
#include <vector>

#include "../../include/obboot.h"

namespace ob {

constexpr int BM = 128;
constexpr int BN = 128;
constexpr int KT = 32;
constexpr int GRAM_THREADS = 256;

struct CudaError { cudaError_t code; const char* what; const char* file; int line; };

#define OB_CUDA(expr)                                                          \
    do {                                                                       \
        cudaError_t e__ = (expr);                                              \
        if (e__ != cudaSuccess) throw ::ob::CudaError{e__, #expr, __FILE__, __LINE__}; \
    } while (0)

struct StatusError { ob_status code; std::string msg; };

inline int64_t num_pairs(int K, int T) { return (int64_t)K * (K + 1) / 2 + (int64_t)K * T + 1; }
inline int design_ldx(int V) { int l = V; while ((l & 7) != 4) ++l; return l; }
inline int64_t pair_base(int K, int T, int j) { return (int64_t)j * (K + T) - (int64_t)j * (j - 1) / 2; }

constexpr int MAX_SEGS = 256;
constexpr int MAX_WORLD = 64;
inline int64_t pad_rows(int64_t n) { return n <= KT ? KT : (n + KT - 1) / KT * KT; }
inline void segment_rows(int64_t n_pad, int& segs, int& seg_rows) {
    const int64_t stages = n_pad / KT;
    int64_t s = stages / 4 < 1 ? 1 : (stages / 4 > MAX_SEGS ? MAX_SEGS : stages / 4);
    const int64_t per = (stages + s - 1) / s;
    s = (stages + per - 1) / per;
    segs = (int)s; seg_rows = (int)(per * KT);
}
struct RowShard {
    int64_t n_global = 0;
    int64_t row_begin = 0;
    int64_t n_local = 0;
    int segs = 1, seg_rows = KT;
    int leaf_lo = 0, leaf_hi = 1;
    int leaf_span = MAX_SEGS;
};
inline RowShard row_shard(int64_t n_global, int rank, int world) {
    RowShard r;
    r.n_global = n_global;
    const int64_t n_pad = pad_rows(n_global);
    segment_rows(n_pad, r.segs, r.seg_rows);
    r.leaf_span = MAX_SEGS / world;
    r.leaf_lo = rank * r.leaf_span < r.segs ? rank * r.leaf_span : r.segs;
    r.leaf_hi = (rank + 1) * r.leaf_span < r.segs ? (rank + 1) * r.leaf_span : r.segs;
    const int64_t lo = (int64_t)r.leaf_lo * r.seg_rows, hi = (int64_t)r.leaf_hi * r.seg_rows;
    r.row_begin = lo < n_global ? lo : n_global;
    const int64_t row_end = hi < n_global ? hi : n_global;
    r.n_local = row_end - r.row_begin;
    return r;
}

struct GroupData {
    int64_t n = 0;
    int64_t n_pad = 0;
    RowShard shard;
    double* X = nullptr;
    double* w = nullptr;
    double* Xs = nullptr;
    uint32_t* src = nullptr;
    double* y_raw = nullptr;
    double* hk_Z = nullptr; uint8_t* hk_sel = nullptr; double* hk_Xm = nullptr;
    uint32_t* uid = nullptr;
    const double* gram_operand() const { return Xs ? Xs : X; }
};

struct CountsArgs {
    void* C; int count_bytes; int64_t n; int64_t n_pad; int panels;
    int64_t n_global = 0;
    int64_t row_begin = 0;
    int64_t slots;
    int first_slot;
    int64_t rep0;
    int group; uint64_t seed;
};
void counts_clear(const CountsArgs& a, cudaStream_t st);
void counts_from_indices(const CountsArgs& a, const uint32_t* d_idx, int* d_overflow, cudaStream_t st);
size_t counts_lut_bytes();
void counts_philox_body_launch(const CountsArgs& a, long long* d_colsum, unsigned char* d_lut, cudaStream_t st);
void counts_philox_fixup_launch(const CountsArgs& a, const long long* d_colsum, int* d_flags, cudaStream_t st);

struct BayesArgs {
    float* C; int64_t n, n_pad; int panels;
    int64_t n_global, row_begin;
    int64_t slots; int first_slot; int64_t rep0;
    int group; uint64_t seed;
    int segs, seg_rows;
    const float* wt;
    double* part;
    int* flags = nullptr;
};
void bayes_weights_launch(const BayesArgs& a, cudaStream_t st);

void cluster_gather_launch(const int32_t* d_codes_frame, const uint32_t* src, int64_t n, int32_t n_codes, uint32_t* uid,
                           uint8_t* present, int* d_flags, cudaStream_t st);
void cluster_scan_launch(const uint8_t* present, int32_t n_codes, uint32_t* unit, long long* d_units, cudaStream_t st);
void cluster_remap_launch(uint32_t* uid, int64_t n, const uint32_t* unit, cudaStream_t st);
struct ExpandArgs {
    void* C; const void* U; const uint32_t* uid; int count_bytes;
    int64_t n, n_pad, u_pad; int panels; int64_t slots;
    long long* rows;
};
void counts_expand_launch(const ExpandArgs& a, cudaStream_t st);

constexpr int BQ = 32;
struct GramColumns {
    int Pc = 0;
    int nfull = 0, tail_q = 0;
    int ntiles = 0;
    std::vector<uint16_t> pairs;
    std::vector<int32_t> colmap;
};
GramColumns gram_columns(int K, int T, int n_cont, const std::vector<int>& cat_levels);
GramColumns gram_outcome_columns(int K, int T);

inline int gram_cache_xx_cells(int K) { return K * (K + 1) / 2; }
inline int gram_cache_y_cells(int K, int T) { return K * T + 1; }
std::vector<int32_t> gram_cache_map(int K, int T);
struct GramCacheCopy {
    double* gram; int64_t slots_pad; int Pld;
    int64_t slot_lo, nslots;
    double* xx; double* yy; int64_t cslots;
    const int32_t* map; int nx, ny;
    int c_lo, c_hi;
};
void gram_cache_extract_launch(const GramCacheCopy& a, cudaStream_t st);
void gram_cache_assemble_launch(const GramCacheCopy& a, cudaStream_t st);
struct GramPlan {
    int K, T, ldx, panels, ntiles;
    int nfull, tail_q, Pld;
    int64_t n_pad[2];
    int segs[2], seg_rows[2];
    int leaf_span;
    int64_t units[2];
    int grid;
    int64_t num_partials;
    size_t smem_bytes; int ring;
};
inline void gram_col_tiling(int64_t Pc, int& nfull, int& tail_q) {
    const int64_t quanta = (Pc + BQ - 1) / BQ;
    nfull = (int)(quanta / 4); tail_q = (int)(quanta % 4);
}
inline int gram_ntiles(int K, int T) { int f, q; gram_col_tiling(num_pairs(K, T), f, q); return f + (q > 0); }
inline int gram_pld(int K, int T) { return (int)((num_pairs(K, T) + BQ - 1) / BQ * BQ); }
GramPlan gram_make_plan(int K, int T, int ldx, int panels, const GroupData g[2], int count_bytes, int num_sms,
                        const GramColumns& cols);
bool gram_fits(int ldx, int count_bytes);
struct GramArgs {
    const double* X[2]; const void* C[2];
    int count_bytes;
    double* partials;
    const uint16_t* d_pairs;
    const int32_t* d_colmap;
    double* gram;
    int tail_mi = 16;
};
void gram_launch(const GramPlan& plan, const GramArgs& args, cudaStream_t st, cudaEvent_t ev_main_begin = nullptr,
                 cudaEvent_t ev_main_end = nullptr);
void gram_launch_leaves(const GramPlan& plan, const GramArgs& args, const int seg_lo[2], const int seg_n[2], cudaStream_t st);
void gram_reduce_launch(const GramPlan& plan, const GramArgs& args, cudaStream_t st);
void leaf_sum_launch(const double* part, const int segs[2], int64_t slots_pad, int span, double* out, cudaStream_t st);
void gram_combine_launch(const double* gathered, int world, const int ranks_with_rows[2], int64_t per_group_elems,
                         double* gram, cudaStream_t st);
int64_t gram_schedule_debug(int K, int panels, int64_t slots_last_panel, const GroupData gd[2], int grid, int64_t* out8, int64_t cap);

struct SolveArgs {
    const double* gram;
    int64_t slots_pad; int Pld;
    int64_t slots;
    int K, n_cont, ref_kind;
    int T = 1;
    int n_norm; const int* d_norm_m; const int* d_norm_off; const int* d_norm_idx; const int* d_norm_has_base;
    int n_base; int S;
    int weighted;
    double na, nb;
    const long long* rows = nullptr;
    const double* esum = nullptr;
    double* stats;
    int* status;
    double* beta_a; double* beta_b;
    double* point_extra;
    double* scratch = nullptr;
};
void solve_launch(const SolveArgs& a, cudaStream_t st);
size_t solve_smem_bytes(int K, bool pooled, int n_norm);
size_t solve_scratch_bytes(int K, bool pooled, int n_norm, int T, int64_t slots);

constexpr int64_t REDUCE_MAX_REPS = 16384;
void reduce_stats_launch(const double* stats, const int* status, int64_t reps, int S,
                         const double* point_stats, double* out5S, long long* n_ok, cudaStream_t st,
                         double* d_scratch = nullptr);
size_t reduce_stats_scratch_bytes(int64_t reps, int S);

struct PackArgs {
    int64_t n; int n_cont, n_cat;
    const double* const* d_cont;
    const int32_t* const* d_cat;
    const int32_t* d_cat_levels;
    const int32_t* d_dummy_start;
    const double* d_y; const double* d_w; const uint8_t* d_group;
    int K, ldx;
};
int pack_num_blocks(int64_t n);
void pack_count_scan(const PackArgs& a, long long* d_block_counts, long long* d_totals, int* d_flags, cudaStream_t st);
struct PackWindow {
    long long shift[2], n_local[2], lo_add[2], hi_base[2];
    double* EX[2]; double* Ew[2]; uint32_t* Esrc[2];
    uint32_t src_add;
};
void pack_scatter(const PackArgs& a, const long long* d_block_base, GroupData ga, GroupData gb, int* d_flags,
                  cudaStream_t st, int blk0 = 0, int blk1 = -1, const PackWindow* win = nullptr);
constexpr int PACK_BLOCK_ROWS = 128;
void iota_launch(uint32_t* dst, int64_t n, uint32_t first, cudaStream_t st);
void add_u32_launch(uint32_t* p, int64_t n, uint32_t add, cudaStream_t st);
void update_outcome_launch(const GroupData& g, int K, int ldx, const double* d_y_frame, cudaStream_t st);
void scale_rows_launch(const GroupData& g, int ldx, cudaStream_t st);
void scale_rows_range_launch(const GroupData& g, int ldx, int64_t row0, int64_t rows, cudaStream_t st);
void residuals_launch(const GroupData& g, int K, int ycol, int ldx, const double* d_beta, double* d_out, cudaStream_t st);
void relayout_launch(const double* src, int ld_src, double* dst, int ld_dst, int64_t rows, int K, cudaStream_t st);

constexpr int INGEST_MAX_COLS = 288;
struct IngestScanArgs {
    long long n;
    int n_valid; const uint8_t* valid[INGEST_MAX_COLS];
    int n_nan; const double* nan_cols[INGEST_MAX_COLS];
    int n_dict; const int32_t* codes[INGEST_MAX_COLS];
    int dict_size[INGEST_MAX_COLS];
    uint8_t* present[INGEST_MAX_COLS];
    uint8_t* row_valid;
    long long* kept;
    int* flags;
};
struct IngestApplyArgs {
    long long n; int n_cat;
    const uint8_t* row_valid;
    const int32_t* group_codes; const int32_t* group_map;
    int32_t* cat_codes[INGEST_MAX_COLS];
    const int32_t* remap; int remap_off[INGEST_MAX_COLS];
    uint8_t* group_out;
    int* flags;
};
void ingest_scan_launch(const IngestScanArgs& a, cudaStream_t st);
void ingest_apply_launch(const IngestApplyArgs& a, cudaStream_t st);

enum class CommDType { I32, I64, F64 };
enum class CommOp { SUM, MAX, MIN };
struct Comm {
    int rank = 0, world = 1;
    virtual ~Comm() = default;
    virtual void allreduce(void* buf, size_t count, CommDType dt, CommOp op, cudaStream_t st) = 0;
    virtual void allgather(const void* send, void* recv, size_t bytes, cudaStream_t st) = 0;
    virtual void allgatherv(const void* send, void* recv, const size_t* offsets, const size_t* sizes, cudaStream_t st) = 0;
    virtual void alltoallv(const void* send, const size_t* send_off, void* recv, const size_t* recv_off, const size_t* bytes,
                           cudaStream_t st) = 0;
};
struct LocalGroup;
LocalGroup* local_group_create(int world);
void local_group_destroy(LocalGroup* g);
Comm* comm_create_local(LocalGroup* g, int rank, int device);
void nccl_unique_id(uint8_t* id128);
Comm* comm_create_nccl(const uint8_t* id128, int rank, int world);

constexpr int HK_MAX_SEL = 8;
struct HkGroup { const double* Z; const uint8_t* sel; int64_t n, n_pad; };
int hk_num_chunks(int64_t n);
void hk_gather_launch(const uint32_t* src, int64_t n, int K1, const double* const* d_pred, const double* d_outcome, double* Z, uint8_t* sel,
                      int* d_flags, cudaStream_t st);
void hk_mask_launch(const double* X, const uint8_t* sel, double* Xm, int64_t rows, int ldx, cudaStream_t st);
void hk_probit_accum_launch(const HkGroup& g, int K1, const void* C, int count_bytes, int panels, const double* gamma, const int* active,
                            int64_t slots_pad, double* partial, cudaStream_t st);
void hk_probit_update_launch(const double* partial, int nchunks, int panels, int K1, int64_t slots, double tol, int last_iter, double* gamma,
                             int* active, int* pstatus, int* n_active, cudaStream_t st);
void hk_terms_launch(const HkGroup& g, const double* X, int ldx, int ycol, int K1, const void* C, int count_bytes, int panels, const double* gamma,
                     double* L, double* partial, cudaStream_t st);
void hk_xterm_launch(const HkGroup& g, const double* X, int ldx, int K, int panels, const double* L, double* partial, cudaStream_t st);
void hk_reduce_launch(const double* partial, int nchunks, int panels, int nacc, double* out, int64_t slots_pad, cudaStream_t st);
struct HkSolveArgs {
    const double* gram; int64_t slots_pad; int Pld; int64_t slots;
    int K, K1, ref_kind;
    const double* terms[2]; const double* xterm[2]; const double* gamma[2]; const int* pstatus[2];
    double na, nb; int S;
    double* stats; int* status; double* beta_a; double* beta_b; double* point_extra;
};
void hk_solve_launch(const HkSolveArgs& a, cudaStream_t st);

constexpr int MM_MAX_COLS = 47;
constexpr int MM_MAX_SIMS = 4096;
struct MmArgs {
    const double* X[2]; const void* C[2]; int64_t n[2], n_pad[2];
    int ldx, K, count_bytes, sims;
    int64_t slots;
    const double* taus;
    double* state; int64_t state_stride;
    double* betas; int* info;
    int* counter;
    int64_t p_begin, p_end;
};
int mm_state_vectors();
int mm_blocks_per_sm(int K, int64_t rows);
void mm_qr_launch(const MmArgs& m, int grid, cudaStream_t st);
void mm_streams_launch(const MmArgs& m, long long pass0, int first_slot, uint64_t seed, double* taus, uint32_t* rows_a, uint32_t* rows_b, cudaStream_t st);
void mm_effects_launch(const MmArgs& m, const uint32_t* rows_a, const uint32_t* rows_b, int nq, const double* d_quantiles,
// ... 8 lines not shown
```

### oaxaca_blinder_rs_b200/csrc/pack.cu

```cuda
#include "common.cuh"
#include "internal.h"

#include <algorithm>

namespace ob {

constexpr int PK_ROWS = 128;
constexpr int PK_THREADS = 256;

__global__ void __launch_bounds__(PK_THREADS) pack_count_kernel(const uint8_t* __restrict__ group,
                                                                const double* __restrict__ w, long long n,
                                                                long long* __restrict__ block_counts,
                                                                int* __restrict__ flags) {
    __shared__ int ca, cb;
    if (threadIdx.x == 0) { ca = 0; cb = 0; }
    __syncthreads();
    const long long row0 = (long long)blockIdx.x * PK_ROWS;
    int a = 0, b = 0;
    for (int t = threadIdx.x; t < PK_ROWS; t += PK_THREADS) {
        const long long i = row0 + t;
        if (i < n) {
            const uint8_t g = group[i];
            a += g == 0; b += g == 1;
            if (w && g <= 1 && w[i] < 0.0) atomicOr(&flags[0], 1);
        }
    }
    if (a) atomicAdd(&ca, a);
    if (b) atomicAdd(&cb, b);
    __syncthreads();
    if (threadIdx.x == 0) { block_counts[2 * blockIdx.x] = ca; block_counts[2 * blockIdx.x + 1] = cb; }
}

__global__ void __launch_bounds__(1024) pack_scan_kernel(long long* __restrict__ bc, int nblocks, long long* totals) {
    __shared__ long long part[2][1024];
    const int t = threadIdx.x;
    const int per = (nblocks + 1023) / 1024;
    const int lo = t * per, hi = min(lo + per, nblocks);
    long long sa = 0, sb = 0;
    for (int i = lo; i < hi; ++i) { sa += bc[2 * i]; sb += bc[2 * i + 1]; }
    part[0][t] = sa; part[1][t] = sb;
    __syncthreads();
    if (t < 2) {
        long long run = 0;
        for (int i = 0; i < 1024; ++i) { const long long v = part[t][i]; part[t][i] = run; run += v; }
        totals[t] = run;
    }
    __syncthreads();
    long long ra = part[0][t], rb = part[1][t];
    for (int i = lo; i < hi; ++i) {
        const long long va = bc[2 * i], vb = bc[2 * i + 1];
        bc[2 * i] = ra; bc[2 * i + 1] = rb;
        ra += va; rb += vb;
    }
}

struct PackKernelParams {
    long long n; int n_cont, n_cat, K, ldx;
    const double* const* cont; const int32_t* const* cat; const int32_t* cat_levels; const int32_t* dummy_start;
    const double* y; const double* w; const uint8_t* group;
    const long long* block_base;
    int blk0;
    double* XA; double* XB; double* wA; double* wB;
    double* XsA; double* XsB;
    uint32_t* srcA; uint32_t* srcB;
    int* flags;
    long long shift[2], n_local[2], lo_add[2], hi_base[2];
    double* EX[2]; double* Ew[2]; uint32_t* Esrc[2];
    uint32_t src_add;
    int tile_cols;
};

__global__ void __launch_bounds__(PK_THREADS) pack_scatter_kernel(const PackKernelParams p) {
    extern __shared__ __align__(16) double tile[];
    __shared__ int lrank[PK_ROWS];
    __shared__ uint8_t lgrp[PK_ROWS];
    __shared__ int srcA[PK_ROWS], srcB[PK_ROWS];
    __shared__ int cnt[2];
    __shared__ const double* scont[288];
    const int V = p.K + 1, ts = V | 1;
    const int blk = blockIdx.x + p.blk0;
    const long long row0 = (long long)blk * PK_ROWS;
    const int rows = (int)min((long long)PK_ROWS, p.n - row0);
    const int tid = threadIdx.x;

    __shared__ int wcount[4][2];
    if (tid < PK_ROWS) {
// ... 154 lines not shown

void scale_rows_range_launch(const GroupData& g, int ldx, int64_t row0, int64_t rows, cudaStream_t st) {
    if (!g.Xs || rows <= 0) return;
    const long long total = rows * (long long)ldx;
    scale_rows_kernel<<<(unsigned)std::min<long long>((total + 255) / 256, 148 * 32), 256, 0, st>>>(g.X + row0 * ldx, g.w + row0, g.Xs + row0 * ldx,
                                                                                                  total, ldx);
    OB_CUDA(cudaGetLastError());
}

__global__ void __launch_bounds__(256) iota_kernel(uint32_t* __restrict__ dst, long long n, uint32_t first) {
    for (long long i = (long long)blockIdx.x * blockDim.x + threadIdx.x; i < n; i += (long long)gridDim.x * blockDim.x)
        dst[i] = first + (uint32_t)i;
}

__global__ void __launch_bounds__(256) add_u32_kernel(uint32_t* __restrict__ p, long long n, uint32_t add) {
    for (long long i = (long long)blockIdx.x * blockDim.x + threadIdx.x; i < n; i += (long long)gridDim.x * blockDim.x) p[i] += add;
}

void add_u32_launch(uint32_t* p, int64_t n, uint32_t add, cudaStream_t st) {
    if (n == 0 || add == 0) return;
    add_u32_kernel<<<(unsigned)std::min<long long>((n + 255) / 256, 148 * 16), 256, 0, st>>>(p, n, add);
    OB_CUDA(cudaGetLastError());
}

void iota_launch(uint32_t* dst, int64_t n, uint32_t first, cudaStream_t st) {
    if (n == 0) return;
    iota_kernel<<<(unsigned)std::min<long long>((n + 255) / 256, 148 * 16), 256, 0, st>>>(dst, n, first);
    OB_CUDA(cudaGetLastError());
}

__global__ void __launch_bounds__(256) update_outcome_kernel(double* __restrict__ X, double* __restrict__ Xs,
                                                             const double* __restrict__ w, const uint32_t* __restrict__ src,
                                                             const double* __restrict__ y, long long n, int K, int ldx) {
    for (long long r = (long long)blockIdx.x * blockDim.x + threadIdx.x; r < n; r += (long long)gridDim.x * blockDim.x) {
        const double v = y[src[r]];
        X[r * ldx + K] = v;
        if (Xs) Xs[r * ldx + K] = sqrt(w[r]) * v;
    }
}

void update_outcome_launch(const GroupData& g, int K, int ldx, const double* d_y_frame, cudaStream_t st) {
    if (g.n == 0) return;
    update_outcome_kernel<<<(unsigned)std::min<long long>((g.n + 255) / 256, 148 * 16), 256, 0, st>>>(g.X, g.Xs, g.w, g.src, d_y_frame,
                                                                                                     g.n, K, ldx);
    OB_CUDA(cudaGetLastError());
}

__global__ void __launch_bounds__(256) relayout_kernel(const double* __restrict__ src, int ld_src, double* __restrict__ dst, int ld_dst,
                                                       long long rows, int K) {
    const long long total = rows * ld_dst;
    for (long long e = (long long)blockIdx.x * blockDim.x + threadIdx.x; e < total; e += (long long)gridDim.x * blockDim.x) {
        const long long r = e / ld_dst; const int c = (int)(e - r * ld_dst);
        dst[e] = c < K ? src[r * ld_src + c] : 0.0;
    }
}

void relayout_launch(const double* src, int ld_src, double* dst, int ld_dst, int64_t rows, int K, cudaStream_t st) {
    if (rows == 0) return;
    const long long total = rows * (long long)ld_dst;
    relayout_kernel<<<(unsigned)std::min<long long>((total + 255) / 256, 148 * 32), 256, 0, st>>>(src, ld_src, dst, ld_dst, rows, K);
    OB_CUDA(cudaGetLastError());
}

__global__ void __launch_bounds__(256) residuals_kernel(const double* __restrict__ X, long long n, int K, int ycol, int ldx,
                                                        const double* __restrict__ beta, double* __restrict__ out) {
    const long long warp = ((long long)blockIdx.x * blockDim.x + threadIdx.x) >> 5;
    const int lane = threadIdx.x & 31;
    if (warp >= n) return;
    const double* row = X + warp * ldx;
    double s = 0.0;
    for (int j = lane; j < K; j += 32) s += row[j] * beta[j];
#pragma unroll
    for (int o = 16; o > 0; o >>= 1) s += __shfl_xor_sync(0xffffffffu, s, o);
    if (lane == 0) out[warp] = row[ycol] - s;
}

void residuals_launch(const GroupData& g, int K, int ycol, int ldx, const double* d_beta, double* d_out, cudaStream_t st) {
    if (g.n == 0) return;
    const long long threads = g.n * 32;
    residuals_kernel<<<(unsigned)((threads + 255) / 256), 256, 0, st>>>(g.X, g.n, K, ycol, ldx, d_beta, d_out);
    OB_CUDA(cudaGetLastError());
}

}
```

### oaxaca_blinder_rs_b200/csrc/resample.cu

```cuda
#include "common.cuh"
#include "internal.h"

#include <cstdlib>

#include <cmath>

namespace ob {

constexpr int KMAX = 24;

struct PoissonTable {
    unsigned long long T[KMAX];
    unsigned short T16[KMAX];
    int lambda_zero;
};

enum : uint32_t { STREAM_BODY = 0x0B0D1u, STREAM_REFINE = 0x0F19Eu, STREAM_FIXUP = 0x0F1Cu };

constexpr int LUT_BITS = 14;
constexpr int LUT_SIZE = 1 << LUT_BITS;
constexpr unsigned AMBIG = 255u;

__device__ __forceinline__ int cdf_count(unsigned long long U, const PoissonTable& t) {
    int c = 0;
#pragma unroll 1
    for (int k = 0; k < KMAX; ++k) c += (U >= t.T[k]) ? 1 : 0;
    return c;
}

struct PoissonDev { unsigned long long T[KMAX]; unsigned int T16[KMAX]; };

__global__ void __launch_bounds__(256) counts_lut_kernel(const PoissonTable tab, unsigned char* __restrict__ lut) {
    const int b = blockIdx.x * blockDim.x + threadIdx.x;
    if (b >= LUT_SIZE) return;
    if (b < KMAX) {
        PoissonDev* d = reinterpret_cast<PoissonDev*>(lut + LUT_SIZE);
        d->T[b] = tab.T[b]; d->T16[b] = tab.T16[b];
    }
    const unsigned long long lo = (unsigned long long)b << (64 - LUT_BITS);
    const unsigned long long hi = lo | ((1ull << (64 - LUT_BITS)) - 1ull);
    const int cl = cdf_count(lo, tab), ch = cdf_count(hi, tab);
    lut[b] = (unsigned char)(cl == ch ? cl : AMBIG);
}

__device__ __noinline__ unsigned poisson_resolve(uint32_t u16, const PoissonDev* __restrict__ t, uint64_t row, uint32_t c1,
                                                 uint64_t rep, uint32_t k0, uint32_t k1) {
    unsigned c = 0; bool tie = false;
#pragma unroll 1
    for (int k = 0; k < KMAX; ++k) { c += (u16 > t->T16[k]) ? 1u : 0u; tie |= (u16 == t->T16[k]); }
    if (!tie) return c;
    const Philox4 r = philox4x32_10((uint32_t)row, c1, (uint32_t)rep, STREAM_REFINE ^ (uint32_t)(rep >> 32), k0, k1);
    const unsigned long long U = ((unsigned long long)u16 << 48) | ((unsigned long long)r.x << 16) | (r.y >> 16);
    c = 0;
#pragma unroll 1
    for (int k = 0; k < KMAX; ++k) c += (U >= t->T[k]) ? 1u : 0u;
    return c;
}

template <typename CountT, int SH>
__global__ void __launch_bounds__(256, 3) counts_philox_body(CountT* __restrict__ C, long long n, long long n_pad,
                                                          long long slots, long long rep0, int first_slot, int group,
                                                          uint32_t k0, uint32_t k1, int lambda_zero,
                                                          const unsigned char* __restrict__ lut_g,
                                                          long long* __restrict__ colsum, int rows_per_block,
                                                          long long row_begin_global) {
    __shared__ __align__(16) unsigned char lut[LUT_SIZE];
    __shared__ int ssum[BM];
    for (int b = threadIdx.x; b < LUT_SIZE / 16; b += blockDim.x)
        reinterpret_cast<uint4*>(lut)[b] = reinterpret_cast<const uint4*>(lut_g)[b];
    if (threadIdx.x < BM) ssum[threadIdx.x] = 0;
    __syncthreads();

    const int panel = blockIdx.y;
    const int q = threadIdx.x & 7;
    const int rl = threadIdx.x >> 3;
    const long long slot0 = (long long)panel * BM + q * 16;
    const long long row_begin = (long long)blockIdx.x * rows_per_block;
    const uint32_t c1base = ((uint32_t)group << 8);
    const long long sid_lo = rep0 + 1 + slot0;
    const long long oct_first = (sid_lo - SH) >> 3;
    constexpr int NOCT = SH ? 3 : 2;
    unsigned valid = 0;
#pragma unroll
    for (int e = 0; e < 16; ++e)
        if (slot0 + e >= first_slot && slot0 + e < slots) valid |= 1u << e;
    const bool point_slot = (slot0 == 0 && first_slot == 1);
    int sums[16];
#pragma unroll
    for (int e = 0; e < 16; ++e) sums[e] = 0;

    for (long long row = row_begin + rl; row < row_begin + rows_per_block && row < n_pad; row += 32) {
        unsigned cnt[16];
#pragma unroll
        for (int e = 0; e < 16; ++e) cnt[e] = 0;
        if (row < n) {
            const unsigned long long grow = (unsigned long long)(row + row_begin_global);
            const uint32_t c1 = c1base | (uint32_t)(grow >> 32);
            if (!lambda_zero && valid) {
                uint32_t w[4 * NOCT];
#pragma unroll
                for (int gi = 0; gi < NOCT; ++gi) {
                    const long long oc = oct_first + gi;
                    const Philox4 r = philox4x32_10((uint32_t)grow, c1, (uint32_t)oc, STREAM_BODY ^ (uint32_t)(oc >> 32), k0, k1);
                    w[4 * gi] = r.x; w[4 * gi + 1] = r.y; w[4 * gi + 2] = r.z; w[4 * gi + 3] = r.w;
                }
                unsigned any = 0;
#pragma unroll
                for (int e = 0; e < 16; ++e) {
                    const int h = SH + e;
                    const uint32_t idx = (h & 1) ? (w[h >> 1] >> (32 - LUT_BITS)) : ((w[h >> 1] >> (16 - LUT_BITS)) & (LUT_SIZE - 1));
                    cnt[e] = lut[idx];
                    any |= cnt[e];
                }
                if (any & 0x80u) {
#pragma unroll
                    for (int e = 0; e < 16; ++e) {
                        if (cnt[e] != AMBIG) continue;
                        const int h = SH + e;
                        const uint32_t u16 = (h & 1) ? (w[h >> 1] >> 16) : (w[h >> 1] & 0xFFFFu);
                        cnt[e] = poisson_resolve(u16, reinterpret_cast<const PoissonDev*>(lut_g + LUT_SIZE), grow, c1,
                                                 (uint64_t)(rep0 + slot0 + e), k0, k1);
                    }
                }
                if (valid != 0xFFFFu) {
#pragma unroll
                    for (int e = 0; e < 16; ++e) cnt[e] = (valid & (1u << e)) ? cnt[e] : 0u;
                }
            }
            if (point_slot) cnt[0] = 1;
#pragma unroll
            for (int e = 0; e < 16; ++e) sums[e] += (int)cnt[e];
        }
        CountT* dst = C + ((long long)panel * n_pad + row) * BM + q * 16;
        if (sizeof(CountT) == 1) {
            uint4 v;
            v.x = cnt[0] | (cnt[1] << 8) | (cnt[2] << 16) | (cnt[3] << 24);
            v.y = cnt[4] | (cnt[5] << 8) | (cnt[6] << 16) | (cnt[7] << 24);
            v.z = cnt[8] | (cnt[9] << 8) | (cnt[10] << 16) | (cnt[11] << 24);
            v.w = cnt[12] | (cnt[13] << 8) | (cnt[14] << 16) | (cnt[15] << 24);
            *reinterpret_cast<uint4*>(dst) = v;
        } else {
            uint4 v0, v1;
            v0.x = cnt[0] | (cnt[1] << 16); v0.y = cnt[2] | (cnt[3] << 16);
            v0.z = cnt[4] | (cnt[5] << 16); v0.w = cnt[6] | (cnt[7] << 16);
            v1.x = cnt[8] | (cnt[9] << 16); v1.y = cnt[10] | (cnt[11] << 16);
            v1.z = cnt[12] | (cnt[13] << 16); v1.w = cnt[14] | (cnt[15] << 16);
            reinterpret_cast<uint4*>(dst)[0] = v0;
            reinterpret_cast<uint4*>(dst)[1] = v1;
        }
    }
#pragma unroll
    for (int e = 0; e < 16; ++e) {
        int s = sums[e];
        s += __shfl_xor_sync(0xffffffffu, s, 8);
        s += __shfl_xor_sync(0xffffffffu, s, 16);
        if ((threadIdx.x & 31) < 8 && s != 0) atomicAdd(&ssum[q * 16 + e], s);
    }
    __syncthreads();
    if (threadIdx.x < BM) {
        const long long slot = (long long)panel * BM + threadIdx.x;
        const int s = ssum[threadIdx.x];
        if (s != 0 && slot < slots) atomicAdd(reinterpret_cast<unsigned long long*>(colsum + slot), (unsigned long long)s);
    }
}

template <typename CountT>
__device__ __forceinline__ bool bump_count(CountT* C, long long elem) {
    unsigned int* word = reinterpret_cast<unsigned int*>(C) + (elem * (long long)sizeof(CountT)) / 4;
    const int shift = (int)((elem * (long long)sizeof(CountT)) & 3) * 8;
    const unsigned old = atomicAdd(word, 1u << shift);
    const unsigned mask = sizeof(CountT) == 1 ? 0xFFu : 0xFFFFu;
    return ((old >> shift) & mask) == mask;
}

template <typename CountT>
__global__ void __launch_bounds__(256) counts_philox_fixup(CountT* __restrict__ C, long long n, long long n_pad,
                                                           long long slots, long long rep0, int first_slot, int group,
                                                           uint32_t k0, uint32_t k1,
                                                           const long long* __restrict__ colsum, int* __restrict__ flags,
                                                           long long n_global, long long row_begin_global) {
    const long long slot = first_slot + blockIdx.x;
    if (slot >= slots) return;
    const long long need = n_global - colsum[slot];
    if (need < 0) { if (threadIdx.x == 0 && blockIdx.y == 0) atomicOr(&flags[0], 1); return; }
    const long long rep = rep0 + slot;
    const long long panel = slot / BM, col = slot % BM;
    const uint32_t c1base = ((uint32_t)group << 8);
    for (long long j = (long long)blockIdx.y * blockDim.x + threadIdx.x; j < need; j += (long long)gridDim.y * blockDim.x) {
        const Philox4 r = philox4x32_10((uint32_t)j, c1base | (uint32_t)((unsigned long long)j >> 32), (uint32_t)rep,
                                        STREAM_FIXUP ^ (uint32_t)((unsigned long long)rep >> 32), k0, k1);
        const unsigned long long U = ((unsigned long long)r.x << 32) | r.y;
        const long long row = (long long)__umul64hi(U, (unsigned long long)n_global) - row_begin_global;
        if (row < 0 || row >= n) continue;
        if (bump_count<CountT>(C, (panel * n_pad + row) * BM + col)) atomicOr(&flags[1], 1);
    }
}

template <typename CountT>
__global__ void __launch_bounds__(256) counts_point_kernel(CountT* __restrict__ C, long long n) {
    const long long i = (long long)blockIdx.x * blockDim.x + threadIdx.x;
    if (i < n) C[i * BM] = 1;
}

template <typename CountT>
__global__ void __launch_bounds__(256) counts_index_kernel(CountT* __restrict__ C, long long n, long long n_pad,
                                                           long long r0, int first_slot,
                                                           const uint32_t* __restrict__ idx, int* __restrict__ flags,
                                                           long long n_global, long long row_begin_global) {
    const long long r = r0 + blockIdx.y;
    const long long slot = first_slot + r, panel = slot / BM, col = slot % BM;
    for (long long i = (long long)blockIdx.x * blockDim.x + threadIdx.x; i < n_global; i += (long long)gridDim.x * blockDim.x) {
        long long row = idx[r * n_global + i];
        if (row >= n_global) { atomicOr(&flags[2], 1); continue; }
        row -= row_begin_global;
        if (row < 0 || row >= n) continue;
        if (bump_count<CountT>(C, (panel * n_pad + row) * BM + col)) atomicOr(&flags[1], 1);
    }
}

constexpr uint32_t STREAM_BAYES = 0x0BA7E5u;

__device__ __forceinline__ float exp1_from_u32(uint32_t u) {
    return -logf(((float)(u >> 9) + 0.5f) * 0x1p-23f);
}

template <int SH, bool EXPLICIT>
__global__ void __launch_bounds__(256) bayes_weights_kernel(const BayesArgs a, uint32_t k0, uint32_t k1) {
    __shared__ double red[8][BM];
    const int leaf = blockIdx.x, panel = blockIdx.y;
    const int q = threadIdx.x & 31, rl = threadIdx.x >> 5;
    const long long slot0 = (long long)panel * BM + 4 * q;
    const long long r_lo = (long long)leaf * a.seg_rows;
    const long long r_hi = r_lo + a.seg_rows < a.n_pad ? r_lo + a.seg_rows : a.n_pad;
    unsigned valid = 0;
#pragma unroll
    for (int e = 0; e < 4; ++e)
        if (slot0 + e >= a.first_slot && slot0 + e < a.slots) valid |= 1u << e;
    const bool point_slot = slot0 == 0 && a.first_slot == 1;
    const long long quad0 = (a.rep0 + 1 + slot0 - SH) >> 2;
    constexpr int NQ = SH ? 2 : 1;
    const uint32_t c1base = (uint32_t)a.group << 8;
    double acc[4] = {0.0, 0.0, 0.0, 0.0};
    for (long long row = r_lo + rl; row < r_hi; row += 8) {
        float E[4] = {0.f, 0.f, 0.f, 0.f};
        if (row < a.n) {
            const unsigned long long grow = (unsigned long long)(row + a.row_begin);
            if (EXPLICIT) {
#pragma unroll
                for (int e = 0; e < 4; ++e) {
                    if (!(valid & (1u << e))) continue;
                    E[e] = a.wt[(size_t)(slot0 + e - a.first_slot) * a.n_global + grow];
                    if (!(E[e] >= 1.17549435e-38f && E[e] <= 3.40282347e38f)) { atomicOr(&a.flags[3], 1); E[e] = 0.f; }
                }
            } else if (valid) {
                const uint32_t c1 = c1base | (uint32_t)(grow >> 32);
                uint32_t w[4 * NQ];
#pragma unroll
                for (int h = 0; h < NQ; ++h) {
                    const long long qd = quad0 + h;
                    const Philox4 r = philox4x32_10((uint32_t)grow, c1, (uint32_t)qd, STREAM_BAYES ^ (uint32_t)((unsigned long long)qd >> 32), k0, k1);
                    w[4 * h] = r.x; w[4 * h + 1] = r.y; w[4 * h + 2] = r.z; w[4 * h + 3] = r.w;
                }
#pragma unroll
                for (int e = 0; e < 4; ++e) E[e] = (valid & (1u << e)) ? exp1_from_u32(w[SH + e]) : 0.f;
            }
            if (point_slot) E[0] = 1.f;
        }
        *reinterpret_cast<float4*>(a.C + ((long long)panel * a.n_pad + row) * BM + 4 * q) = make_float4(E[0], E[1], E[2], E[3]);
#pragma unroll
        for (int e = 0; e < 4; ++e) acc[e] += (double)E[e];
    }
#pragma unroll
    for (int e = 0; e < 4; ++e) red[rl][4 * q + e] = acc[e];
    __syncthreads();
    if (threadIdx.x < BM) {
        double s = red[0][threadIdx.x];
#pragma unroll
        for (int l = 1; l < 8; ++l) s += red[l][threadIdx.x];
        a.part[(size_t)leaf * a.panels * BM + (size_t)panel * BM + threadIdx.x] = s;
    }
}

void bayes_weights_launch(const BayesArgs& a, cudaStream_t st) {
    if (a.segs <= 0 || a.panels <= 0) return;
    const uint32_t k0 = (uint32_t)a.seed, k1 = (uint32_t)(a.seed >> 32);
    const dim3 grid((unsigned)a.segs, (unsigned)a.panels);
    if (a.wt) {
        bayes_weights_kernel<0, true><<<grid, 256, 0, st>>>(a, k0, k1);
    } else {
        switch ((int)(((a.rep0 + 1) % 4 + 4) % 4)) {
        case 0: bayes_weights_kernel<0, false><<<grid, 256, 0, st>>>(a, k0, k1); break;
        case 1: bayes_weights_kernel<1, false><<<grid, 256, 0, st>>>(a, k0, k1); break;
        case 2: bayes_weights_kernel<2, false><<<grid, 256, 0, st>>>(a, k0, k1); break;
        default: bayes_weights_kernel<3, false><<<grid, 256, 0, st>>>(a, k0, k1); break;
        }
    }
    OB_CUDA(cudaGetLastError());
}

void counts_clear(const CountsArgs& a, cudaStream_t st) {
    OB_CUDA(cudaMemsetAsync(a.C, 0, (size_t)a.panels * a.n_pad * BM * a.count_bytes, st));
}

void counts_from_indices(const CountsArgs& a, const uint32_t* d_idx, int* d_flags, cudaStream_t st) {
    counts_clear(a, st);
    const int pb = (int)((a.n + 255) / 256);
    const int pbg = (int)std::max<long long>((a.n_global + 255) / 256, 1);
    const long long reps = a.slots - a.first_slot;
    if (a.first_slot == 1 && pb > 0) {
        if (a.count_bytes == 1) counts_point_kernel<uint8_t><<<pb, 256, 0, st>>>((uint8_t*)a.C, a.n);
        else counts_point_kernel<uint16_t><<<pb, 256, 0, st>>>((uint16_t*)a.C, a.n);
        OB_CUDA(cudaGetLastError());
    }
    for (long long done = 0; done < reps; done += 32768) {
        const long long nb = std::min<long long>(reps - done, 32768);
        dim3 grid((unsigned)std::min<long long>(pbg, 1024), (unsigned)nb);
        if (a.count_bytes == 1)
            counts_index_kernel<uint8_t><<<grid, 256, 0, st>>>((uint8_t*)a.C, a.n, a.n_pad, done, a.first_slot, d_idx, d_flags,
                                                               a.n_global, a.row_begin);
        else
            counts_index_kernel<uint16_t><<<grid, 256, 0, st>>>((uint16_t*)a.C, a.n, a.n_pad, done, a.first_slot, d_idx, d_flags,
                                                                a.n_global, a.row_begin);
        OB_CUDA(cudaGetLastError());
    }
}

static PoissonTable make_table(long long n) {
    PoissonTable t{};
    const long double delta = ceill(8.0L * sqrtl((long double)n));
    if (delta >= (long double)n) { t.lambda_zero = 1; return t; }
    const long double lam = ((long double)n - delta) / (long double)n;
    long double p = expl(-lam), cdf = 0.0L;
    const long double two64 = 18446744073709551616.0L;
    for (int k = 0; k < KMAX; ++k) {
        cdf += p;
        long double v = floorl(cdf * two64);
        t.T[k] = (v >= two64 || cdf >= 1.0L) ? 0xFFFFFFFFFFFFFFFFull : (unsigned long long)v;
        t.T16[k] = (unsigned short)(t.T[k] >> 48);
        p = p * lam / (long double)(k + 1);
    }
    t.lambda_zero = 0;
    return t;
}

size_t counts_lut_bytes() { return LUT_SIZE + ((sizeof(PoissonDev) + 255) / 256) * 256; }

void counts_philox_body_launch(const CountsArgs& a, long long* d_colsum, unsigned char* d_lut, cudaStream_t st) {
    const PoissonTable tab = make_table(a.n_global);
    counts_lut_kernel<<<LUT_SIZE / 256, 256, 0, st>>>(tab, d_lut);
    OB_CUDA(cudaGetLastError());
    const uint32_t k0 = (uint32_t)a.seed, k1 = (uint32_t)(a.seed >> 32);
    const int rows_per_block = 2048;
    dim3 grid((unsigned)((a.n_pad + rows_per_block - 1) / rows_per_block), (unsigned)a.panels);
    const int sh = (int)((((a.rep0 + 1) % 8) + 8) % 8);
    auto body = [&](auto ct) {
        using CT = decltype(ct);
#define OB_BODY(SHV) counts_philox_body<CT, SHV><<<grid, 256, 0, st>>>((CT*)a.C, a.n, a.n_pad, a.slots, a.rep0, \
            a.first_slot, a.group, k0, k1, tab.lambda_zero, d_lut, d_colsum, rows_per_block, a.row_begin)
        switch (sh) {
        case 0: OB_BODY(0); break; case 1: OB_BODY(1); break; case 2: OB_BODY(2); break; case 3: OB_BODY(3); break;
        case 4: OB_BODY(4); break; case 5: OB_BODY(5); break; case 6: OB_BODY(6); break; default: OB_BODY(7);
        }
#undef OB_BODY
    };
    if (a.count_bytes == 1) body(uint8_t{}); else body(uint16_t{});
    OB_CUDA(cudaGetLastError());
}

void counts_philox_fixup_launch(const CountsArgs& a, const long long* d_colsum, int* d_flags, cudaStream_t st) {
    const long long nrep = a.slots - a.first_slot;
    if (nrep <= 0) return;
    const uint32_t k0 = (uint32_t)a.seed, k1 = (uint32_t)(a.seed >> 32);
    dim3 fgrid((unsigned)nrep, 16);
    if (a.count_bytes == 1)
        counts_philox_fixup<uint8_t><<<fgrid, 256, 0, st>>>((uint8_t*)a.C, a.n, a.n_pad, a.slots, a.rep0, a.first_slot,
                                                            a.group, k0, k1, d_colsum, d_flags, a.n_global, a.row_begin);
    else
        counts_philox_fixup<uint16_t><<<fgrid, 256, 0, st>>>((uint16_t*)a.C, a.n, a.n_pad, a.slots, a.rep0, a.first_slot,
                                                             a.group, k0, k1, d_colsum, d_flags, a.n_global, a.row_begin);
    OB_CUDA(cudaGetLastError());
}

}
```

Measured before the change: 1247.

## Sort rows by categorical cell to shrink Gram work on one-hot columns

```diff
diff --git a/include/obboot.h b/include/obboot.h
--- a/include/obboot.h
+++ b/include/obboot.h
@@ -239,6 +239,12 @@
                               uint16_t* pairs_out, int32_t* colmap_out, int64_t cap, int32_t* tiling_out);
 int64_t ob_debug_gram_outcome_columns(int32_t K, int32_t T, uint16_t* pairs_out, int32_t* colmap_out, int64_t cap,
                                       int32_t* tiling_out);
+int64_t ob_debug_gram_cell_columns(int32_t K, int32_t T, int32_t n_cont, const int32_t* cat_levels, int32_t n_cat, int32_t outcome_only,
+                                   uint16_t* pairs_out, int32_t* colmap_out, int32_t* src_out, uint64_t* mask_out, int64_t cap,
+                                   int32_t* tiling_out);
+int64_t ob_debug_gram_cell_schedule(int32_t K, int32_t T, int32_t n_cont, const int32_t* cat_levels, int32_t n_cat,
+                                    const uint8_t* cell_a, int64_t n_a, const uint8_t* cell_b, int64_t n_b, int64_t slots,
+                                    int32_t grid, int64_t* out10, int64_t cap, int64_t* n_cpad_out);
 
 ob_status ob_debug_counts(ob_ctx* ctx, const ob_design* d, uint64_t seed, int64_t rep, int32_t group,
                           uint16_t* counts_out);
diff --git a/oaxaca_blinder_rs_b200/csrc/api.cu b/oaxaca_blinder_rs_b200/csrc/api.cu
--- a/oaxaca_blinder_rs_b200/csrc/api.cu
+++ b/oaxaca_blinder_rs_b200/csrc/api.cu
@@ -9,9 +9,9 @@
 #include <memory>
 #include <atomic>
 #include <mutex>
+#include <type_traits>
 #include <optional>
 #include <set>
-#include <type_traits>
 
 using namespace ob;
 
@@ -60,6 +60,8 @@
     int cl_strata = OB_CLUSTER_NONE;
     int64_t cl_units[2] = {0, 0};
     uint64_t id = 0, x_gen = 0, y_gen = 0;
+    CellLayout cells;
+    int cells_state = 0;
 };
 
 struct ob_gram_cache {
@@ -76,6 +78,7 @@
     int shard_reps = 0, rep_world = 1, rep_rank = 0, row_world = 1, row_rank = 0, K = 0;
     int count_bytes = 1;
     bool bayes = false;
+    bool cells = false;
     bool y_ok = false;
     uint64_t y_gen = 0; int T = 0;
 };
@@ -236,6 +239,16 @@
         if (g.uid) cudaFreeAsync(g.uid, st);
         g.X = g.w = g.Xs = g.y_raw = g.hk_Z = g.hk_Xm = nullptr; g.src = g.uid = nullptr; g.hk_sel = nullptr;
     }
+    CellLayout& cl = d->cells;
+    for (int g = 0; g < 2; ++g) {
+        if (cl.perm[g]) cudaFreeAsync(cl.perm[g], st);
+        if (cl.inv_perm[g]) cudaFreeAsync(cl.inv_perm[g], st);
+        if (cl.leaf_off[g]) cudaFreeAsync(cl.leaf_off[g], st);
+        cl.perm[g] = cl.inv_perm[g] = nullptr; cl.leaf_off[g] = nullptr;
+    }
+    if (cl.runs) cudaFreeAsync(cl.runs, st);
+    if (cl.leaf_run) cudaFreeAsync(cl.leaf_run, st);
+    cl.runs = nullptr; cl.leaf_run = nullptr; cl.ncells = 0;
 }
 
 void cache_release_device(ob_gram_cache* c) {
@@ -375,12 +388,13 @@
 template <typename Opts>
 int generate_counts(const ob_design* d, const Opts* o, const Batch& b, int count_bytes, int64_t ppb, DevBuf (&C)[2],
                     DevBuf (&idx)[2], DevBuf& colsum, DevBuf& lut, int* flags, Comm* row_comm, double* ms_comm, cudaStream_t st,
-                    ClusterWork* cw = nullptr) {
+                    ClusterWork* cw = nullptr, const CellLayout* cl = nullptr) {
     CountsArgs ca[2];
     const int mats = cw ? unit_mats(d) : 2;
     for (int g = 0; g < mats; ++g) {
         const GroupData& G = d->g[g];
         ca[g].C = C[g].p; ca[g].count_bytes = count_bytes; ca[g].n = G.n; ca[g].n_pad = G.n_pad;
+        if (cl) { ca[g].n_pad = cl->n_cpad[g]; ca[g].perm = cl->perm[g]; ca[g].inv_perm = cl->inv_perm[g]; }
         ca[g].n_global = G.shard.n_global; ca[g].row_begin = G.shard.row_begin;
         ca[g].panels = (int)b.pn; ca[g].slots = b.bslots; ca[g].first_slot = b.first_slot; ca[g].rep0 = b.rep0;
         ca[g].group = g; ca[g].seed = o->seed;
@@ -1964,6 +1978,63 @@
     });
 }
 
+const CellLayout* design_cells(ob_ctx* ctx, const ob_design* dc, int T, Comm* comm) {
+    ob_design* d = const_cast<ob_design*>(dc);
+    if (d->K1 > 0 || d->cl_strata != OB_CLUSTER_NONE || d->cells_state < 0) return nullptr;
+    if (gram_cell_columns(d->K, T, d->n_cont, d->cat_levels, false).nt_run < 0) return nullptr;
+    if (d->cells_state > 0) return &d->cells;
+    const GramColumns c1 = gram_cell_columns(d->K, 1, d->n_cont, d->cat_levels, false), dense1 = gram_columns(d->K, 1, d->n_cont, d->cat_levels);
+    const int64_t qc = gram_quanta(c1), qd = gram_quanta(dense1);
+    const int64_t n_all = d->g[0].shard.n_global + d->g[1].shard.n_global;
+    const int64_t n_pad_all = pad_rows(d->g[0].shard.n_global) + pad_rows(d->g[1].shard.n_global);
+    if (c1.nt_run < 0 || dense1.nfull < 1 || d->g[0].shard.n_global >= INT32_MAX || d->g[1].shard.n_global >= INT32_MAX ||
+        n_all * qc >= n_pad_all * qd) {
+        d->cells_state = -1;
+        return nullptr;
+    }
+    pending_finish(d);
+    cudaStream_t st = ctx->stream;
+    CellLayout& cl = d->cells;
+    cl.ncells = cell_count(d->cat_levels);
+    cl.h_runs.clear();
+    cl.h_leaf_run.clear();
+    std::vector<int32_t> perm[2], inv[2];
+    for (int g = 0; g < 2; ++g) {
+        const GroupData& G = d->g[g];
+        std::vector<uint8_t> h_cell((size_t)G.n);
+        {
+            DevBuf d_cell((size_t)std::max<int64_t>(G.n, 1));
+            cell_ids_launch(G.X, G.n, d->ldx, d->n_cont, d->cat_levels, d_cell.as<uint8_t>(), st);
+            if (G.n) OB_CUDA(cudaMemcpyAsync(h_cell.data(), d_cell.p, (size_t)G.n, cudaMemcpyDeviceToHost, st));
+            OB_CUDA(cudaStreamSynchronize(st));
+        }
+        const int segs = G.shard.leaf_hi - G.shard.leaf_lo;
+        const size_t r0 = cl.h_runs.size();
+        cl.n_cpad[g] = cell_order(h_cell.data(), G.n, segs, G.shard.seg_rows, cl.ncells, perm[g], inv[g], cl.h_leaf_off[g], cl.h_runs);
+        cl.nruns[g] = (int)(cl.h_runs.size() - r0);
+        size_t r = r0;
+        for (int s = 0; s <= segs; ++s) {
+            while (r < cl.h_runs.size() && cl.h_runs[r].row0 < cl.h_leaf_off[g][(size_t)s]) ++r;
+            cl.h_leaf_run.push_back((int32_t)r);
+        }
+    }
+    int64_t n_cpad_all = cl.n_cpad[0] + cl.n_cpad[1];
+    if (comm) n_cpad_all = allreduce_scalar(comm, (long long)n_cpad_all, CommOp::SUM, st);
+    if (n_cpad_all * qc >= n_pad_all * qd) { d->cells_state = -1; cl.ncells = 0; return nullptr; }
+    auto upload = [&](auto*& dst, const auto& v) {
+        using E = typename std::remove_reference<decltype(v)>::type::value_type;
+        const size_t b = sizeof(E) * std::max<size_t>(v.size(), 1);
+        OB_CUDA(cudaMallocFromPoolAsync((void**)&dst, b, ctx->pool_design, st));
+        if (!v.empty()) OB_CUDA(cudaMemcpyAsync((void*)dst, v.data(), sizeof(E) * v.size(), cudaMemcpyHostToDevice, st));
+    };
+    for (int g = 0; g < 2; ++g) { upload(cl.perm[g], perm[g]); upload(cl.inv_perm[g], inv[g]); upload(cl.leaf_off[g], cl.h_leaf_off[g]); }
+    upload(cl.runs, cl.h_runs);
+    upload(cl.leaf_run, cl.h_leaf_run);
+    OB_CUDA(cudaStreamSynchronize(st));
+    d->cells_state = 1;
+    return &cl;
+}
+
 static void bootstrap_body(ob_ctx* ctx, const ob_design* d, const ob_boot_opts* o, ob_gram_cache* cache, ob_result* res,
                            bool bayes = false, const ob_bayes_opts* bo = nullptr) {
         design_alive(d);
@@ -2016,6 +2087,8 @@
                                                                                                            : OB_CACHE_OUTCOME_ONLY;
             if (Comm* ac = rr.shard_reps ? ctx->comm.get() : comm) mode = allreduce_scalar(ac, mode, CommOp::MIN, st);
         }
+        const CellLayout* cells = (bayes || mode == OB_CACHE_SOLVE_ONLY) ? nullptr : design_cells(ctx, d, T, comm);
+        if (mode == OB_CACHE_OUTCOME_ONLY && cache->cells != (cells != nullptr)) mode = OB_CACHE_FILLED;
         const bool solve_only = mode == OB_CACHE_SOLVE_ONLY, outcome_only = mode == OB_CACHE_OUTCOME_ONLY;
         for (int v = 0; v < o->n_norm; ++v) {
             n_base += o->norm_has_base[v] ? 1 : 0;
@@ -2083,12 +2156,14 @@
             }
         }
 
-        const GramColumns gcols = solve_only ? GramColumns() : outcome_only ? gram_outcome_columns(K, T)
-                                                                              : gram_columns(K, T, d->n_cont, d->cat_levels);
+        const GramColumns gcols = solve_only ? GramColumns()
+                                  : cells ? gram_cell_columns(K, T, d->n_cont, d->cat_levels, outcome_only)
+                                  : outcome_only ? gram_outcome_columns(K, T) : gram_columns(K, T, d->n_cont, d->cat_levels);
         const int ntiles = gcols.ntiles;
         const int Pld = gram_pld(K, T);
         const int64_t panels_total = (slots + BM - 1) / BM;
-        const int64_t n_pad[2] = {d->g[0].n_pad, d->g[1].n_pad};
+        const int64_t n_pad[2] = {cells ? cells->n_cpad[0] : d->g[0].n_pad, cells ? cells->n_cpad[1] : d->g[1].n_pad};
+        const int64_t cell_runs = cells ? (int64_t)cells->nruns[0] + cells->nruns[1] : 0;
         const int64_t n_glob[2] = {d->g[0].shard.n_global, d->g[1].shard.n_global};
         const int mats = clustered ? unit_mats(d) : 0;
         int64_t u_pad_all = 0;
@@ -2106,20 +2181,29 @@
                                                           (bayes_explicit ? (double)(n_glob[0] + n_glob[1]) * BM * 4.0 : 0.0));
             if (solve_only) return 2.0 * BM * Pld * 8.0 + cl;
             return (double)(n_pad[0] + n_pad[1]) * BM * cb + (rr.index_mode ? (double)idx_len * BM * 4.0 : 0.0) +
-                   2.0 * BM * Pld * 8.0 * (comm ? world + 2 : 1) + (double)local_leaves * ntiles * (BM * BN * 8.0) + 2.0 * BM * 8.0 + cl;
+                   2.0 * BM * Pld * 8.0 * (comm ? world + 2 : 1) + (double)(local_leaves * ntiles + cell_runs) * (BM * BN * 8.0) + 2.0 * BM * 8.0 + cl;
         };
-        double budget = (double)o->max_workspace_bytes - (double)cache_new_bytes;
+        DevBuf d_Xc[2];
+        const size_t xc_bytes = cells && !solve_only ? sizeof(double) * (size_t)(n_pad[0] + n_pad[1]) * d->ldx : 0;
+        double budget = (double)o->max_workspace_bytes - (double)(cache_new_bytes + xc_bytes);
         if (o->max_workspace_bytes <= 0) {
             const double idle = (double)pool_idle_bytes(ctx);
-            const double need_all = per_panel_bytes(count_bytes) * (double)panels_total;
+            const double need_all = per_panel_bytes(count_bytes) * (double)panels_total + (double)xc_bytes;
             if (idle >= 1.02 * need_all) budget = 1.01 * need_all;
             else {
                 size_t free_b = 0, total_b = 0;
                 OB_CUDA(cudaMemGetInfo(&free_b, &total_b));
-                budget = 0.6 * ((double)free_b + idle) - (double)cache_new_bytes;
+                budget = 0.6 * ((double)free_b + idle) - (double)(cache_new_bytes + xc_bytes);
             }
         }
         DevBuf d_lut(2 * counts_lut_bytes());
+        if (xc_bytes) {
+            for (int g = 0; g < 2; ++g) {
+                d_Xc[g].alloc(sizeof(double) * (size_t)n_pad[g] * d->ldx);
+                gather_rows_launch(d->g[g].gram_operand(), cells->perm[g], n_pad[g], d->g[g].n, d->ldx, d_Xc[g].as<double>(), st);
+                res->gpu_launches += 1;
+            }
+        }
 
         std::vector<double> point(PE * T);
         cudaEvent_t ev_point = nullptr;
@@ -2139,7 +2223,7 @@
             const size_t gram_elems = 2 * (size_t)ppb * BM * Pld;
             bool saturated = false;
             GramPlan plan; int64_t plan_panels = -1;
-            DevBuf d_partials, d_pairs, d_colmap, d_cmap;
+            DevBuf d_partials, d_pairs, d_colmap, d_cmap, d_run_partials, d_src, d_mask;
             auto allocate_workspace = [&] {
                 if (!solve_only) {
                     if (!bayes) d_colsum.alloc(sizeof(long long) * 2 * (size_t)ppb * BM);
@@ -2160,9 +2244,18 @@
                 }
                 if (solve_only) { OB_CUDA(cudaStreamSynchronize(st)); return; }
                 if (comm) { d_gram_local.alloc(sizeof(double) * gram_elems); d_gathered.alloc(sizeof(double) * gram_elems * world); }
-                plan = gram_make_plan(K, T, d->ldx, (int)std::min<int64_t>(ppb, panels_total), d->g, count_bytes, ctx->num_sms, gcols);
+                plan = gram_make_plan(K, T, d->ldx, (int)std::min<int64_t>(ppb, panels_total), d->g, count_bytes, ctx->num_sms, gcols, cells);
                 plan_panels = plan.panels;
                 d_partials.alloc(sizeof(double) * (size_t)std::max<int64_t>(plan.num_partials, 1) * BM * BN);
+                if (cells) {
+                    d_run_partials.alloc(sizeof(double) * (size_t)std::max<int64_t>(plan.num_run_partials, 1) * BM * BN);
+                    d_src.alloc(sizeof(int32_t) * std::max<size_t>(gcols.src.size(), 1));
+                    d_mask.alloc(sizeof(uint64_t) * std::max<size_t>(gcols.mask.size(), 1));
+                    if (!gcols.src.empty()) {
+                        OB_CUDA(cudaMemcpyAsync(d_src.p, gcols.src.data(), sizeof(int32_t) * gcols.src.size(), cudaMemcpyHostToDevice, st));
+                        OB_CUDA(cudaMemcpyAsync(d_mask.p, gcols.mask.data(), sizeof(uint64_t) * gcols.mask.size(), cudaMemcpyHostToDevice, st));
+                    }
+                }
                 d_pairs.alloc(sizeof(uint16_t) * gcols.pairs.size());
                 d_colmap.alloc(sizeof(int32_t) * gcols.colmap.size());
                 OB_CUDA(cudaMemcpyAsync(d_pairs.p, gcols.pairs.data(), sizeof(uint16_t) * gcols.pairs.size(), cudaMemcpyHostToDevice, st));
@@ -2182,18 +2275,21 @@
                     res->gpu_launches += generate_weights(d, o, bo, b, d_C, bw, d_flags.as<int>(), comm, &res->ms_comm, st);
                 else if (!solve_only)
                     res->gpu_launches += generate_counts(d, o, b, count_bytes, ppb, d_C, d_idx, d_colsum, d_lut, d_flags.as<int>(), comm,
-                                                         &res->ms_comm, st, clustered ? &cw : nullptr);
+                                                         &res->ms_comm, st, clustered ? &cw : nullptr, cells);
                 t_counts.stop();
                 tr.mark("counts", st, true);
 
                 if (!solve_only && plan_panels != pn) {
-                    plan = gram_make_plan(K, T, d->ldx, (int)pn, d->g, count_bytes, ctx->num_sms, gcols);
+                    plan = gram_make_plan(K, T, d->ldx, (int)pn, d->g, count_bytes, ctx->num_sms, gcols, cells);
                     plan_panels = pn;
                     d_partials.alloc(sizeof(double) * (size_t)std::max<int64_t>(plan.num_partials, 1) * BM * BN);
+                    if (cells) d_run_partials.alloc(sizeof(double) * (size_t)std::max<int64_t>(plan.num_run_partials, 1) * BM * BN);
                 }
                 Timer t_gram(st, &res->ms_gram);
                 GramArgs ga;
-                for (int g = 0; g < 2; ++g) { ga.X[g] = d->g[g].gram_operand(); ga.C[g] = d_C[g].p; }
+                for (int g = 0; g < 2; ++g) { ga.X[g] = cells ? d_Xc[g].as<double>() : d->g[g].gram_operand(); ga.C[g] = d_C[g].p; }
+                ga.cells = cells; ga.run_partials = d_run_partials.as<double>();
+                ga.d_src = d_src.as<int32_t>(); ga.d_mask = d_mask.as<unsigned long long>();
                 ga.count_bytes = count_bytes; ga.partials = d_partials.as<double>();
                 ga.d_pairs = d_pairs.as<uint16_t>(); ga.d_colmap = d_colmap.as<int32_t>();
                 ga.gram = comm ? d_gram_local.as<double>() : d_gram.as<double>();
@@ -2338,7 +2434,7 @@
                 cache->reps = o->reps; cache->rep_begin = rr.rb; cache->rep_end = rr.re; cache->slots = slots;
                 cache->shard_reps = rr.shard_reps ? 1 : 0; cache->rep_world = rep_world; cache->rep_rank = rep_rank;
                 cache->row_world = d->world; cache->row_rank = d->rank; cache->K = K; cache->count_bytes = count_bytes;
-                cache->bayes = bayes;
+                cache->bayes = bayes; cache->cells = cells != nullptr;
                 cache->xx_ok = true;
             }
             if (!solve_only) { cache->y_gen = d->y_gen; cache->T = T; cache->y_ok = true; }
@@ -2534,6 +2630,42 @@
     }
     const int64_t panels = (slots + BM - 1) / BM;
     return gram_schedule_debug(K, (int)panels, slots - (panels - 1) * BM, gd, grid, out8, cap);
+}
+
+int64_t ob_debug_gram_cell_columns(int32_t K, int32_t T, int32_t n_cont, const int32_t* cat_levels, int32_t n_cat, int32_t outcome_only,
+                                   uint16_t* pairs_out, int32_t* colmap_out, int32_t* src_out, uint64_t* mask_out, int64_t cap,
+                                   int32_t* tiling_out) {
+    if (K < 1 || T < 1 || n_cont < 0 || n_cat < 0 || (n_cat > 0 && !cat_levels) || K + T > 65535) return -1;
+    const GramColumns gc = gram_cell_columns(K, T, n_cont, std::vector<int>(cat_levels, cat_levels + n_cat), outcome_only != 0);
+    if (gc.nt_run < 0) return 0;
+    const int64_t len = (int64_t)gc.colmap.size();
+    for (int64_t c = 0; c < len && c < cap; ++c) {
+        if (pairs_out) { pairs_out[2 * c] = gc.pairs[2 * (size_t)c]; pairs_out[2 * c + 1] = gc.pairs[2 * (size_t)c + 1]; }
+        if (colmap_out) colmap_out[c] = gc.colmap[(size_t)c];
+        if (src_out) src_out[c] = c < (int64_t)gc.src.size() ? gc.src[(size_t)c] : -1;
+        if (mask_out) mask_out[c] = c < (int64_t)gc.mask.size() ? gc.mask[(size_t)c] : 0;
+    }
+    if (tiling_out) { tiling_out[0] = gc.Pc; tiling_out[1] = gc.nfull; tiling_out[2] = gc.tail_q; tiling_out[3] = gc.nt_run; }
+    return len;
+}
+
+int64_t ob_debug_gram_cell_schedule(int32_t K, int32_t T, int32_t n_cont, const int32_t* cat_levels, int32_t n_cat,
+                                    const uint8_t* cell_a, int64_t n_a, const uint8_t* cell_b, int64_t n_b, int64_t slots,
+                                    int32_t grid, int64_t* out10, int64_t cap, int64_t* n_cpad_out) {
+    if (K < 1 || T < 1 || n_cont < 0 || n_cat < 0 || (n_cat > 0 && !cat_levels) || n_a < 1 || n_b < 1 || !cell_a || !cell_b ||
+        slots < 1 || grid < 1 || !n_cpad_out) return -1;
+    const std::vector<int> lv(cat_levels, cat_levels + n_cat);
+    const int nc = cell_count(lv);
+    const int64_t ns[2] = {n_a, n_b};
+    const uint8_t* cells[2] = {cell_a, cell_b};
+    GroupData gd[2];
+    for (int g = 0; g < 2; ++g) {
+        for (int64_t i = 0; i < ns[g]; ++i) if (cells[g][i] >= nc) return -1;
+        gd[g].shard = row_shard(ns[g], 0, 1);
+        gd[g].n = ns[g]; gd[g].n_pad = pad_rows(ns[g]);
+    }
+    const int64_t panels = (slots + BM - 1) / BM;
+    return gram_cell_schedule_debug(K, T, n_cont, lv, (int)panels, slots - (panels - 1) * BM, gd, cells, grid, out10, cap, n_cpad_out);
 }
 
 ob_status ob_debug_counts(ob_ctx* ctx, const ob_design* d, uint64_t seed, int64_t rep, int32_t group,
diff --git a/oaxaca_blinder_rs_b200/csrc/gram.cu b/oaxaca_blinder_rs_b200/csrc/gram.cu
--- a/oaxaca_blinder_rs_b200/csrc/gram.cu
+++ b/oaxaca_blinder_rs_b200/csrc/gram.cu
@@ -2,6 +2,7 @@
 #include "internal.h"
 
 #include <algorithm>
+#include <cassert>
 #include <cstdlib>
 #include <type_traits>
 
@@ -25,7 +26,18 @@
     int tail_mi;
     double* partials;
     const uint16_t* pairs;
+    int nt_run;
+    int nruns[2];
+    const CellRun* runs;
+    const int64_t* leaf_off[2];
+    double* run_partials;
 };
+
+#if defined(OB_GRAM_BOUNDS_CHECK) && defined(__CUDA_ARCH__)
+#define GRAM_CHECK(cond) assert(cond)
+#else
+#define GRAM_CHECK(cond) ((void)0)
+#endif
 
 template <typename CountT>
 __device__ __forceinline__ double count_to_f64(CountT c, const double* __restrict__ tab) {
@@ -49,15 +61,39 @@
 
 __host__ __device__ __forceinline__ bool ws_decode(const GramKernelParams& p, long long i, int ldx, size_t count_bytes, GramUnit& u) {
     const int pt = p.tail_mi < 16 ? 1 : 0, pf = p.panels - pt;
+    const int nt_base = p.nt_run >= 0 ? p.nt_run : 0;
+    const int run_wide = p.nt_run >= 0 && p.nfull > 0, run_tail = p.nt_run >= 0 && p.nfull == 0;
+    const long long nruns = p.nt_run >= 0 ? (long long)p.nruns[0] + p.nruns[1] : 0;
+    const long long r0 = nruns * pf, r1 = nruns * pt;
+    if (i < r0 + r1) {
+        const int tp = i >= r0 ? 1 : 0;
+        if (tp) i -= r0;
+        const int np = tp ? pt : pf;
+        const long long run = i / np;
+        const int panel = (tp ? pf : 0) + (int)(i - run * np);
+        const int g = run >= p.nruns[0] ? 1 : 0;
+        const CellRun cr = p.runs[run];
+        const long long n_pad = g ? p.n_pad[1] : p.n_pad[0];
+        GRAM_CHECK(cr.nstages >= 1 && cr.row0 >= 0 && cr.row0 % KT == 0 && cr.row0 + (long long)cr.nstages * KT <= n_pad);
+        u.nstages = cr.nstages;
+        u.nt = nt_base; u.tq = run_tail ? p.tail_q : 4;
+        u.mi = panel >= pf ? p.tail_mi : 16;
+        u.Xg = (g ? p.X[1] : p.X[0]) + cr.row0 * ldx;
+        u.Cg = reinterpret_cast<const unsigned char*>(g ? p.C[1] : p.C[0]) + (((long long)panel * n_pad + cr.row0) * BM) * (long long)count_bytes;
+        u.out = p.run_partials + (size_t)((long long)panel * nruns + run) * (BM * BN);
+        return true;
+    }
+    i -= r0 + r1;
+    const int nwide = p.nfull - run_wide;
     const long long segs01 = (long long)p.seg_n[0] + p.seg_n[1];
-    const long long n0 = segs01 * pf * p.nfull, n1 = segs01 * pt * p.nfull;
-    const long long n2 = p.tail_q ? segs01 * pf : 0, n3 = p.tail_q ? segs01 * pt : 0;
+    const long long n0 = segs01 * pf * nwide, n1 = segs01 * pt * nwide;
+    const long long n2 = p.tail_q && !run_tail ? segs01 * pf : 0, n3 = p.tail_q && !run_tail ? segs01 * pt : 0;
     if (i >= n0 + n1 + n2 + n3) return false;
     int np, p0, nt_cnt, nt0;
-    if (i < n0) { np = pf; p0 = 0; nt_cnt = p.nfull; nt0 = 0; }
-    else if ((i -= n0) < n1) { np = pt; p0 = pf; nt_cnt = p.nfull; nt0 = 0; }
-    else if ((i -= n1) < n2) { np = pf; p0 = 0; nt_cnt = 1; nt0 = p.nfull; }
-    else { i -= n2; np = pt; p0 = pf; nt_cnt = 1; nt0 = p.nfull; }
+    if (i < n0) { np = pf; p0 = 0; nt_cnt = nwide; nt0 = nt_base + run_wide; }
+    else if ((i -= n0) < n1) { np = pt; p0 = pf; nt_cnt = nwide; nt0 = nt_base + run_wide; }
+    else if ((i -= n1) < n2) { np = pf; p0 = 0; nt_cnt = 1; nt0 = nt_base + p.nfull; }
+    else { i -= n2; np = pt; p0 = pf; nt_cnt = 1; nt0 = nt_base + p.nfull; }
     const long long per_seg = (long long)np * nt_cnt;
     const long long g0 = (long long)p.seg_n[0] * per_seg;
     const int g = i >= g0 ? 1 : 0;
@@ -68,14 +104,23 @@
     const int panel = p0 + (int)(r2 / nt_cnt), nt = nt0 + (int)(r2 % nt_cnt);
     const int segs = g ? p.segs[1] : p.segs[0], seg_rows = g ? p.seg_rows[1] : p.seg_rows[0];
     const long long n_pad = g ? p.n_pad[1] : p.n_pad[0];
-    const long long row0 = (long long)seg * seg_rows;
-    const long long row1 = row0 + seg_rows < n_pad ? row0 + seg_rows : n_pad;
+    long long row0, row1;
+    if (p.nt_run >= 0) {
+        const int64_t* lo = g ? p.leaf_off[1] : p.leaf_off[0];
+        row0 = lo[seg]; row1 = lo[seg + 1];
+    } else {
+        row0 = (long long)seg * seg_rows;
+        row1 = row0 + seg_rows < n_pad ? row0 + seg_rows : n_pad;
+    }
+    GRAM_CHECK(row0 >= 0 && row0 % KT == 0 && row1 % KT == 0 && row1 > row0 && row1 <= n_pad && seg < segs);
     u.nstages = (int)((row1 - row0) / KT);
-    u.nt = nt; u.tq = (p.tail_q && nt == p.nfull) ? p.tail_q : 4;
+    u.nt = nt; u.tq = (p.tail_q && nt == nt_base + p.nfull) ? p.tail_q : 4;
     u.mi = panel >= pf ? p.tail_mi : 16;
     u.Xg = (g ? p.X[1] : p.X[0]) + row0 * ldx;
     u.Cg = reinterpret_cast<const unsigned char*>(g ? p.C[1] : p.C[0]) + (((long long)panel * n_pad + row0) * BM) * (long long)count_bytes;
-    u.out = p.partials + (size_t)((g ? p.units0 : 0) + ((long long)panel * segs + seg) * p.ntiles + nt) * (BM * BN);
+    const long long part = (g ? p.units0 : 0) + ((long long)panel * segs + seg) * p.ntiles + nt;
+    GRAM_CHECK(part >= 0 && part < p.units_total);
+    u.out = p.partials + (size_t)part * (BM * BN);
     return true;
 }
 
@@ -299,6 +344,39 @@
     }
 }
 
+__global__ void __launch_bounds__(256) gram_cell_fold_kernel(const double* __restrict__ run_partials, const CellRun* __restrict__ runs,
+                                                             const int32_t* __restrict__ leaf_run, int nruns_all,
+                                                             const int32_t* __restrict__ src, const unsigned long long* __restrict__ mask,
+                                                             double* __restrict__ partials, int segs0, int segs1, int ntiles,
+                                                             int nt_run, int run_tw) {
+    const int leaf = blockIdx.x, panel = blockIdx.y, panels = gridDim.y;
+    const int g = leaf >= segs0 ? 1 : 0, seg = leaf - (g ? segs0 : 0);
+    const int32_t* lr = leaf_run + (g ? segs0 + 1 : 0);
+    const int r_lo = lr[seg], r_hi = lr[seg + 1];
+    GRAM_CHECK(r_lo >= 0 && r_lo <= r_hi && r_hi <= nruns_all);
+    const size_t units0 = (size_t)panels * ntiles * segs0;
+    const double* rp = run_partials + (size_t)panel * nruns_all * (BM * BN);
+    const int total = (nt_run + 1) * BM * BN;
+    for (int e = threadIdx.x; e < total; e += blockDim.x) {
+        const int t = e / (BM * BN), rem = e - t * (BM * BN);
+        const int tw = t == nt_run ? run_tw : BN;
+        const int m = rem / BN, c = rem - m * BN;
+        if (c >= tw) continue;
+        double s = 0.0;
+        if (t == nt_run) {
+            for (int r = r_lo; r < r_hi; ++r) s += rp[(size_t)r * (BM * BN) + m * run_tw + c];
+        } else {
+            const int k = t * BN + c;
+            const unsigned long long mk = mask[k];
+            const int sc = src[k];
+            for (int r = r_lo; r < r_hi; ++r)
+                if ((mk >> runs[r].cell) & 1ull) s += rp[(size_t)r * (BM * BN) + m * run_tw + sc];
+        }
+        const size_t part = (g ? units0 : 0) + ((size_t)panel * (g ? segs1 : segs0) + seg) * ntiles + t;
+        partials[part * (BM * BN) + m * tw + c] = s;
+    }
+}
+
 __global__ void __launch_bounds__(256) gram_reduce_kernel(const double* __restrict__ partials, int segs0, int segs1,
                                                           double* __restrict__ gram, int panels, int ntiles, int span,
                                                           int Pld, int tail_q, const int32_t* __restrict__ colmap) {
@@ -393,6 +471,108 @@
     return gc;
 }
 
+int cell_count(const std::vector<int>& cat_levels) {
+    int64_t c = 1;
+    for (int m : cat_levels) { c *= m > 1 ? m : 1; if (c > MAX_CELLS) return MAX_CELLS + 1; }
+    return (int)c;
+}
+
+GramColumns gram_cell_columns(int K, int T, int n_cont, const std::vector<int>& cat_levels, bool outcome_only) {
+    GramColumns none;
+    int64_t dummies = 0;
+    for (int m : cat_levels) dummies += m > 1 ? m - 1 : 0;
+    if (cat_levels.empty() || dummies == 0 || 1 + (int64_t)n_cont + dummies != K) return none;
+    const int ncells = cell_count(cat_levels);
+    if (ncells > MAX_CELLS) return none;
+    std::vector<int> block((size_t)K, -1), level((size_t)K, 0), stride(cat_levels.size(), 1);
+    {
+        int c = 1 + n_cont, st = 1;
+        for (size_t q = 0; q < cat_levels.size(); ++q) {
+            stride[q] = st;
+            for (int lvl = 1; lvl < cat_levels[q]; ++lvl) { block[(size_t)c] = (int)q; level[(size_t)c++] = lvl; }
+            st *= cat_levels[q] > 1 ? cat_levels[q] : 1;
+        }
+    }
+    auto cells_of = [&](int j) {
+        uint64_t mk = 0;
+        const int q = block[(size_t)j];
+        const int m = cat_levels[(size_t)q] > 1 ? cat_levels[(size_t)q] : 1;
+        for (int c = 0; c < ncells; ++c)
+            if ((c / stride[(size_t)q]) % m == level[(size_t)j]) mk |= 1ull << c;
+        return mk;
+    };
+    std::vector<uint16_t> pj, pl; std::vector<int32_t> cm;
+    struct Der { int a, b; int32_t target; };
+    std::vector<Der> der;
+    auto add = [&](int j, int l, int64_t target) {
+        const bool dj = j < K && block[(size_t)j] >= 0, dl = l < K && block[(size_t)l] >= 0;
+        if (dj && dl && j != l && block[(size_t)j] == block[(size_t)l]) return;
+        if (dj || dl) { der.push_back(Der{dj ? j : l, dj ? l : j, (int32_t)target}); return; }
+        pj.push_back((uint16_t)j); pl.push_back((uint16_t)l); cm.push_back((int32_t)target);
+    };
+    for (int j = 0; j < K; ++j) {
+        const int64_t base = pair_base(K, T, j);
+        if (!outcome_only)
+            for (int l = j; l < K; ++l) add(j, l, base + (l - j));
+        for (int o = 0; o < T; ++o) add(j, K + o, base + (K - j) + o);
+    }
+    pj.push_back((uint16_t)K); pl.push_back((uint16_t)K); cm.push_back((int32_t)(num_pairs(K, T) - 1));
+    GramColumns gc;
+    gc.Pc = (int)cm.size();
+    gram_col_tiling(gc.Pc, gc.nfull, gc.tail_q);
+    const int run_tw = gc.nfull > 0 ? BN : gc.tail_q * BQ;
+    std::vector<int> src_of((size_t)(K + T), -1);
+    for (int c = 0; c < gc.Pc && c < run_tw; ++c)
+        if (pj[(size_t)c] == 0) src_of[(size_t)pl[(size_t)c]] = c;
+    const int nder = (int)der.size();
+    gc.nt_run = (nder + BN - 1) / BN;
+    gc.ntiles = gc.nt_run + gc.nfull + (gc.tail_q > 0);
+    const size_t cols = (size_t)gc.ntiles * BN;
+    gc.pairs.assign(cols * 2, (uint16_t)K);
+    gc.colmap.assign(cols, -1);
+    gc.src.assign((size_t)gc.nt_run * BN, 0);
+    gc.mask.assign((size_t)gc.nt_run * BN, 0);
+    for (int k = 0; k < nder; ++k) {
+        const Der& d = der[(size_t)k];
+        const bool both = d.b < K && block[(size_t)d.b] >= 0;
+        const int s = src_of[(size_t)(both ? 0 : d.b)];
+        if (s < 0) return none;
+        gc.src[(size_t)k] = s;
+        gc.mask[(size_t)k] = cells_of(d.a) & (both ? cells_of(d.b) : ~0ull);
+        gc.colmap[(size_t)k] = d.target;
+    }
+    const size_t c0 = (size_t)gc.nt_run * BN;
+    for (size_t c = 0; c < cm.size(); ++c) { gc.pairs[2 * (c0 + c)] = pj[c]; gc.pairs[2 * (c0 + c) + 1] = pl[c]; gc.colmap[c0 + c] = cm[c]; }
+    return gc;
+}
+
+int64_t cell_order(const uint8_t* cell, int64_t n, int segs, int seg_rows, int ncells, std::vector<int32_t>& perm,
+                   std::vector<int32_t>& inv_perm, std::vector<int64_t>& leaf_off, std::vector<CellRun>& runs) {
+    leaf_off.assign((size_t)segs + 1, 0);
+    inv_perm.assign((size_t)n, -1);
+    std::vector<int64_t> cnt((size_t)ncells);
+    int64_t pos = 0;
+    perm.clear();
+    for (int s = 0; s < segs; ++s) {
+        const int64_t lo = std::min<int64_t>((int64_t)s * seg_rows, n), hi = std::min<int64_t>((int64_t)(s + 1) * seg_rows, n);
+        leaf_off[(size_t)s] = pos;
+        std::fill(cnt.begin(), cnt.end(), 0);
+        for (int64_t i = lo; i < hi; ++i) ++cnt[cell[i]];
+        std::vector<int64_t> at((size_t)ncells);
+        for (int c = 0; c < ncells; ++c) {
+            if (!cnt[(size_t)c]) continue;
+            const int64_t len = (cnt[(size_t)c] + KT - 1) / KT * KT;
+            runs.push_back(CellRun{pos, (int32_t)(len / KT), c});
+            at[(size_t)c] = pos;
+            pos += len;
+        }
+        perm.resize((size_t)pos, -1);
+        for (int64_t i = lo; i < hi; ++i) { const int64_t p = at[cell[i]]++; perm[(size_t)p] = (int32_t)i; inv_perm[(size_t)i] = (int32_t)p; }
+    }
+    leaf_off[(size_t)segs] = pos;
+    return pos;
+}
+
 std::vector<int32_t> gram_cache_map(int K, int T) {
     std::vector<int32_t> m;
     m.reserve((size_t)gram_cache_xx_cells(K) + gram_cache_y_cells(K, T));
@@ -433,7 +613,7 @@
 void gram_cache_assemble_launch(const GramCacheCopy& a, cudaStream_t st) { gram_cache_copy(a, false, st); }
 
 GramPlan gram_make_plan(int K, int T, int ldx, int panels, const GroupData gd[2], int count_bytes, int num_sms,
-                        const GramColumns& cols) {
+                        const GramColumns& cols, const CellLayout* cl) {
     GramPlan pl;
     pl.K = K; pl.T = T; pl.ldx = ldx; pl.panels = panels;
     pl.nfull = cols.nfull; pl.tail_q = cols.tail_q; pl.ntiles = cols.ntiles;
@@ -451,6 +631,13 @@
     pl.ring = gram_ws_smem(pl.ldx, count_bytes, WS_R) <= GRAM_SMEM_MAX ? WS_R : 2;
     pl.smem_bytes = gram_ws_smem(pl.ldx, count_bytes, pl.ring);
     pl.num_partials = (int64_t)total;
+    if (cols.nt_run >= 0 && cl && cl->ncells > 0) {
+        pl.nt_run = cols.nt_run;
+        for (int g = 0; g < 2; ++g) { pl.n_pad[g] = cl->n_cpad[g]; pl.nruns[g] = cl->nruns[g]; }
+        pl.num_run_partials = (int64_t)panels * (pl.nruns[0] + pl.nruns[1]);
+        total = pl.num_run_partials + ((int64_t)pl.segs[0] + pl.segs[1]) * panels * (cols.nfull + (cols.tail_q > 0) - 1);
+        pl.grid = (int)std::min<int64_t>(num_sms, std::max<int64_t>(total, 1));
+    }
     return pl;
 }
 
@@ -467,12 +654,23 @@
     p.nfull = pl.nfull; p.tail_q = pl.tail_q;
     p.partials = a.partials; p.pairs = a.d_pairs;
     p.tail_mi = a.tail_mi >= 1 && a.tail_mi <= 16 ? a.tail_mi : 16;
+    p.nt_run = pl.nt_run;
+    p.nruns[0] = pl.nruns[0]; p.nruns[1] = pl.nruns[1];
+    p.runs = nullptr; p.leaf_off[0] = p.leaf_off[1] = nullptr; p.run_partials = nullptr;
+    if (pl.nt_run >= 0) {
+        if (!a.cells) throw StatusError{OB_ERR_INVALID_ARG, "cell-mode Gram plan without its cell layout"};
+        if ((seg_lo && (seg_lo[0] || seg_lo[1])) || (seg_n && (seg_n[0] != pl.segs[0] || seg_n[1] != pl.segs[1])))
+            throw StatusError{OB_ERR_INVALID_ARG, "a cell-mode Gram launch covers every leaf"};
+        p.runs = a.cells->runs; p.leaf_off[0] = a.cells->leaf_off[0]; p.leaf_off[1] = a.cells->leaf_off[1];
+        p.run_partials = a.run_partials;
+    }
     return p;
 }
 
 void gram_launch_leaves(const GramPlan& pl, const GramArgs& a, const int seg_lo[2], const int seg_n[2], cudaStream_t st) {
     const GramKernelParams p = gram_params(pl, a, seg_lo, seg_n);
-    const int64_t units = ((int64_t)p.seg_n[0] + p.seg_n[1]) * pl.panels * pl.ntiles;
+    const int64_t units = pl.nt_run >= 0 ? pl.num_run_partials + ((int64_t)p.seg_n[0] + p.seg_n[1]) * pl.panels * (pl.ntiles - pl.nt_run - 1)
+                                         : ((int64_t)p.seg_n[0] + p.seg_n[1]) * pl.panels * pl.ntiles;
     if (units <= 0) return;
     const int grid = (int)std::min<int64_t>(pl.grid, units);
     const size_t ws_smem = pl.smem_bytes;
@@ -499,6 +697,13 @@
 
 void gram_reduce_launch(const GramPlan& pl, const GramArgs& a, cudaStream_t st) {
     OB_CUDA(cudaMemsetAsync(a.gram, 0, sizeof(double) * 2 * (size_t)pl.panels * BM * (size_t)pl.Pld, st));
+    if (pl.nt_run >= 0 && pl.segs[0] + pl.segs[1] > 0) {
+        const int run_tw = pl.nfull > 0 ? BN : pl.tail_q * BQ;
+        gram_cell_fold_kernel<<<dim3((unsigned)(pl.segs[0] + pl.segs[1]), (unsigned)pl.panels), 256, 0, st>>>(
+            a.run_partials, a.cells->runs, a.cells->leaf_run, pl.nruns[0] + pl.nruns[1], a.d_src, a.d_mask, a.partials,
+            pl.segs[0], pl.segs[1], pl.ntiles, pl.nt_run, run_tw);
+        OB_CUDA(cudaGetLastError());
+    }
     dim3 rgw(2 * pl.panels * pl.ntiles, 16);
     gram_reduce_kernel<<<rgw, 256, 0, st>>>(a.partials, pl.segs[0], pl.segs[1], a.gram, pl.panels, pl.ntiles, pl.leaf_span,
                                             pl.Pld, pl.tail_q, a.d_colmap);
@@ -536,6 +741,7 @@
     p.ldx = pl.ldx; p.panels = pl.panels; p.ntiles = pl.ntiles; p.nfull = pl.nfull; p.tail_q = pl.tail_q;
     p.tail_mi = (int)std::min<int64_t>(16, ((slots_last_panel + 7) / 8 + 3) / 4 * 4);
     p.partials = nullptr;
+    p.nt_run = -1;
     int64_t count = 0;
     for (int b = 0; b < grid; ++b) {
         GramUnit u;
@@ -555,4 +761,57 @@
     return count;
 }
 
-}
+int64_t gram_cell_schedule_debug(int K, int T, int n_cont, const std::vector<int>& cat_levels, int panels, int64_t slots_last_panel,
+                                 const GroupData gd[2], const uint8_t* const cell[2], int grid, int64_t* out10, int64_t cap,
+                                 int64_t n_cpad_out[2]) {
+    const GramColumns cols = gram_cell_columns(K, T, n_cont, cat_levels, false);
+    if (cols.nt_run < 0) return -1;
+    CellLayout cl;
+    cl.ncells = cell_count(cat_levels);
+    std::vector<int32_t> perm, inv;
+    GroupData g2[2] = {gd[0], gd[1]};
+    for (int g = 0; g < 2; ++g) {
+        const int segs = gd[g].shard.leaf_hi - gd[g].shard.leaf_lo;
+        const size_t r0 = cl.h_runs.size();
+        cl.n_cpad[g] = cell_order(cell[g], gd[g].n, segs, gd[g].shard.seg_rows, cl.ncells, perm, inv, cl.h_leaf_off[g], cl.h_runs);
+        cl.nruns[g] = (int)(cl.h_runs.size() - r0);
+        n_cpad_out[g] = cl.n_cpad[g];
+    }
+    GramPlan pl = gram_make_plan(K, T, design_ldx(K + T), panels, g2, 1, grid, cols, &cl);
+    GramKernelParams p{};
+    for (int g = 0; g < 2; ++g) {
+        p.n_pad[g] = pl.n_pad[g]; p.segs[g] = pl.segs[g]; p.seg_rows[g] = pl.seg_rows[g]; p.seg_lo[g] = 0; p.seg_n[g] = pl.segs[g];
+        p.nruns[g] = pl.nruns[g]; p.leaf_off[g] = cl.h_leaf_off[g].data();
+    }
+    p.units0 = pl.units[0]; p.units_total = pl.units[0] + pl.units[1];
+    p.ldx = pl.ldx; p.panels = pl.panels; p.ntiles = pl.ntiles; p.nfull = pl.nfull; p.tail_q = pl.tail_q;
+    p.tail_mi = (int)std::min<int64_t>(16, ((slots_last_panel + 7) / 8 + 3) / 4 * 4);
+    p.nt_run = pl.nt_run; p.runs = cl.h_runs.data();
+    p.partials = nullptr; p.run_partials = p.partials + (size_t)pl.num_partials * (BM * BN);
+    const long long nruns = (long long)pl.nruns[0] + pl.nruns[1];
+    int64_t count = 0;
+    for (int b = 0; b < grid; ++b) {
+        GramUnit u;
+        for (long long i = b; ws_decode(p, i, pl.ldx, 1, u); i += grid) {
+            if (count < cap) {
+                int64_t* o = out10 + 10 * count;
+                const long long idx = (long long)(u.out - (double*)nullptr) / (BM * BN);
+                const long long row0 = (long long)(u.Xg - (const double*)nullptr) / pl.ldx;
+                o[0] = b; o[6] = row0; o[7] = u.nstages; o[8] = u.mi; o[9] = u.tq < 4 ? u.tq : 0; o[3] = u.nt;
+                if (idx >= pl.num_partials) {
+                    const long long r = idx - pl.num_partials, run = r % nruns;
+                    o[1] = run >= pl.nruns[0] ? 1 : 0; o[2] = r / nruns; o[4] = -1; o[5] = run;
+                } else {
+                    const int gg = idx >= p.units0 ? 1 : 0;
+                    const long long r = idx - (gg ? p.units0 : 0);
+                    const long long sweep = r / p.ntiles;
+                    o[1] = gg; o[2] = sweep / p.segs[gg]; o[4] = sweep % p.segs[gg]; o[5] = -1;
+                }
+            }
+            ++count;
+        }
+    }
+    return count;
+}
+
+}
diff --git a/oaxaca_blinder_rs_b200/csrc/internal.h b/oaxaca_blinder_rs_b200/csrc/internal.h
--- a/oaxaca_blinder_rs_b200/csrc/internal.h
+++ b/oaxaca_blinder_rs_b200/csrc/internal.h
@@ -82,6 +82,8 @@
     int first_slot;
     int64_t rep0;
     int group; uint64_t seed;
+    const int32_t* perm = nullptr;
+    const int32_t* inv_perm = nullptr;
 };
 void counts_clear(const CountsArgs& a, cudaStream_t st);
 void counts_from_indices(const CountsArgs& a, const uint32_t* d_idx, int* d_overflow, cudaStream_t st);
@@ -119,9 +121,33 @@
     int ntiles = 0;
     std::vector<uint16_t> pairs;
     std::vector<int32_t> colmap;
+    int nt_run = -1;
+    std::vector<int32_t> src;
+    std::vector<uint64_t> mask;
 };
 GramColumns gram_columns(int K, int T, int n_cont, const std::vector<int>& cat_levels);
 GramColumns gram_outcome_columns(int K, int T);
+
+constexpr int MAX_CELLS = 64;
+struct CellRun { int64_t row0; int32_t nstages, cell; };
+struct CellLayout {
+    int ncells = 0;
+    int64_t n_cpad[2] = {0, 0};
+    int32_t* perm[2] = {nullptr, nullptr};
+    int32_t* inv_perm[2] = {nullptr, nullptr};
+    int64_t* leaf_off[2] = {nullptr, nullptr};
+    CellRun* runs = nullptr;
+    int32_t* leaf_run = nullptr;
+    int nruns[2] = {0, 0};
+    std::vector<int64_t> h_leaf_off[2];
+    std::vector<CellRun> h_runs;
+    std::vector<int32_t> h_leaf_run;
+};
+int cell_count(const std::vector<int>& cat_levels);
+int64_t cell_order(const uint8_t* cell, int64_t n, int segs, int seg_rows, int ncells, std::vector<int32_t>& perm,
+                   std::vector<int32_t>& inv_perm, std::vector<int64_t>& leaf_off, std::vector<CellRun>& runs);
+GramColumns gram_cell_columns(int K, int T, int n_cont, const std::vector<int>& cat_levels, bool outcome_only);
+inline int64_t gram_quanta(const GramColumns& c) { return (int64_t)c.nfull * 4 + c.tail_q; }
 
 inline int gram_cache_xx_cells(int K) { return K * (K + 1) / 2; }
 inline int gram_cache_y_cells(int K, int T) { return K * T + 1; }
@@ -145,6 +171,9 @@
     int grid;
     int64_t num_partials;
     size_t smem_bytes; int ring;
+    int nt_run = -1;
+    int nruns[2] = {0, 0};
+    int64_t num_run_partials = 0;
 };
 inline void gram_col_tiling(int64_t Pc, int& nfull, int& tail_q) {
     const int64_t quanta = (Pc + BQ - 1) / BQ;
@@ -153,7 +182,7 @@
 inline int gram_ntiles(int K, int T) { int f, q; gram_col_tiling(num_pairs(K, T), f, q); return f + (q > 0); }
 inline int gram_pld(int K, int T) { return (int)((num_pairs(K, T) + BQ - 1) / BQ * BQ); }
 GramPlan gram_make_plan(int K, int T, int ldx, int panels, const GroupData g[2], int count_bytes, int num_sms,
-                        const GramColumns& cols);
+                        const GramColumns& cols, const CellLayout* cl = nullptr);
 bool gram_fits(int ldx, int count_bytes);
 struct GramArgs {
     const double* X[2]; const void* C[2];
@@ -163,6 +192,10 @@
     const int32_t* d_colmap;
     double* gram;
     int tail_mi = 16;
+    const CellLayout* cells = nullptr;
+    double* run_partials = nullptr;
+    const int32_t* d_src = nullptr;
+    const unsigned long long* d_mask = nullptr;
 };
 void gram_launch(const GramPlan& plan, const GramArgs& args, cudaStream_t st, cudaEvent_t ev_main_begin = nullptr,
                  cudaEvent_t ev_main_end = nullptr);
@@ -172,6 +205,9 @@
 void gram_combine_launch(const double* gathered, int world, const int ranks_with_rows[2], int64_t per_group_elems,
                          double* gram, cudaStream_t st);
 int64_t gram_schedule_debug(int K, int panels, int64_t slots_last_panel, const GroupData gd[2], int grid, int64_t* out8, int64_t cap);
+int64_t gram_cell_schedule_debug(int K, int T, int n_cont, const std::vector<int>& cat_levels, int panels, int64_t slots_last_panel,
+                                 const GroupData gd[2], const uint8_t* const cell[2], int grid, int64_t* out10, int64_t cap,
+                                 int64_t n_cpad_out[2]);
 
 struct SolveArgs {
     const double* gram;
@@ -227,6 +263,9 @@
 void scale_rows_range_launch(const GroupData& g, int ldx, int64_t row0, int64_t rows, cudaStream_t st);
 void residuals_launch(const GroupData& g, int K, int ycol, int ldx, const double* d_beta, double* d_out, cudaStream_t st);
 void relayout_launch(const double* src, int ld_src, double* dst, int ld_dst, int64_t rows, int K, cudaStream_t st);
+void cell_ids_launch(const double* X, int64_t n, int ldx, int n_cont, const std::vector<int>& cat_levels, uint8_t* cell,
+                     cudaStream_t st);
+void gather_rows_launch(const double* src, const int32_t* perm, int64_t rows, int64_t n, int ldx, double* Xc, cudaStream_t st);
 
 constexpr int INGEST_MAX_COLS = 288;
 struct IngestScanArgs {
diff --git a/oaxaca_blinder_rs_b200/csrc/pack.cu b/oaxaca_blinder_rs_b200/csrc/pack.cu
--- a/oaxaca_blinder_rs_b200/csrc/pack.cu
+++ b/oaxaca_blinder_rs_b200/csrc/pack.cu
@@ -2,6 +2,7 @@
 #include "internal.h"
 
 #include <algorithm>
+#include <cassert>
 
 namespace ob {
 
@@ -322,4 +323,63 @@
     OB_CUDA(cudaGetLastError());
 }
 
-}
+constexpr int CELL_MAX_CATS = 6;
+struct CellSpec { int ncat; int first[CELL_MAX_CATS], levels[CELL_MAX_CATS], stride[CELL_MAX_CATS]; };
+
+__global__ void __launch_bounds__(256) cell_ids_kernel(const double* __restrict__ X, long long n, int ldx, const CellSpec cs,
+                                                       uint8_t* __restrict__ cell) {
+    for (long long i = (long long)blockIdx.x * blockDim.x + threadIdx.x; i < n; i += (long long)gridDim.x * blockDim.x) {
+        const double* row = X + i * ldx;
+        int c = 0;
+        for (int q = 0; q < cs.ncat; ++q)
+            for (int lvl = 1; lvl < cs.levels[q]; ++lvl)
+                if (row[cs.first[q] + lvl - 1] != 0.0) c += lvl * cs.stride[q];
+        cell[i] = (uint8_t)c;
+    }
+}
+
+void cell_ids_launch(const double* X, int64_t n, int ldx, int n_cont, const std::vector<int>& cat_levels, uint8_t* cell,
+                     cudaStream_t st) {
+    CellSpec cs{};
+    int col = 1 + n_cont, stride = 1;
+    for (int m : cat_levels) {
+        if (m > 1) {
+            if (cs.ncat == CELL_MAX_CATS) throw StatusError{OB_ERR_INVALID_ARG, "more categoricals than the cell layout takes"};
+            cs.first[cs.ncat] = col; cs.levels[cs.ncat] = m; cs.stride[cs.ncat] = stride; ++cs.ncat;
+            stride *= m;
+        }
+        col += m > 1 ? m - 1 : 0;
+    }
+    if (n <= 0) return;
+    const unsigned blocks = (unsigned)std::min<int64_t>((n + 255) / 256, 148 * 16);
+    cell_ids_kernel<<<blocks, 256, 0, st>>>(X, n, ldx, cs, cell);
+    OB_CUDA(cudaGetLastError());
+}
+
+__global__ void __launch_bounds__(256) gather_rows_kernel(const double* __restrict__ src, const int32_t* __restrict__ perm,
+                                                          long long rows, long long n, int ldx, double* __restrict__ Xc) {
+    const int lane = threadIdx.x & 31;
+    const long long w0 = ((long long)blockIdx.x * blockDim.x + threadIdx.x) >> 5, nw = ((long long)gridDim.x * blockDim.x) >> 5;
+    for (long long p = w0; p < rows; p += nw) {
+        const long long r = perm[p];
+#if defined(OB_GRAM_BOUNDS_CHECK) && defined(__CUDA_ARCH__)
+        assert(r < n);
+#endif
+        double* dst = Xc + p * ldx;
+        if (r >= 0 && r < n) {
+            const double* s = src + r * ldx;
+            for (int c = lane; c < ldx; c += 32) dst[c] = s[c];
+        } else {
+            for (int c = lane; c < ldx; c += 32) dst[c] = 0.0;
+        }
+    }
+}
+
+void gather_rows_launch(const double* src, const int32_t* perm, int64_t rows, int64_t n, int ldx, double* Xc, cudaStream_t st) {
+    if (rows <= 0) return;
+    const unsigned blocks = (unsigned)std::min<int64_t>((rows + 7) / 8, 148 * 16);
+    gather_rows_kernel<<<blocks, 256, 0, st>>>(src, perm, rows, n, ldx, Xc);
+    OB_CUDA(cudaGetLastError());
+}
+
+}
diff --git a/oaxaca_blinder_rs_b200/csrc/resample.cu b/oaxaca_blinder_rs_b200/csrc/resample.cu
--- a/oaxaca_blinder_rs_b200/csrc/resample.cu
+++ b/oaxaca_blinder_rs_b200/csrc/resample.cu
@@ -1,9 +1,16 @@
 #include "common.cuh"
 #include "internal.h"
 
+#include <cassert>
 #include <cstdlib>
 
 #include <cmath>
+
+#if defined(OB_GRAM_BOUNDS_CHECK) && defined(__CUDA_ARCH__)
+#define GRAM_CHECK(cond) assert(cond)
+#else
+#define GRAM_CHECK(cond) ((void)0)
+#endif
 
 namespace ob {
 
@@ -63,7 +70,7 @@
                                                           uint32_t k0, uint32_t k1, int lambda_zero,
                                                           const unsigned char* __restrict__ lut_g,
                                                           long long* __restrict__ colsum, int rows_per_block,
-                                                          long long row_begin_global) {
+                                                          long long row_begin_global, const int32_t* __restrict__ perm) {
     __shared__ __align__(16) unsigned char lut[LUT_SIZE];
     __shared__ int ssum[BM];
     for (int b = threadIdx.x; b < LUT_SIZE / 16; b += blockDim.x)
@@ -93,8 +100,10 @@
         unsigned cnt[16];
 #pragma unroll
         for (int e = 0; e < 16; ++e) cnt[e] = 0;
-        if (row < n) {
-            const unsigned long long grow = (unsigned long long)(row + row_begin_global);
+        const long long lrow = perm ? (long long)perm[row] : row;
+        GRAM_CHECK(!perm || lrow < n);
+        if (lrow >= 0 && lrow < n) {
+            const unsigned long long grow = (unsigned long long)(lrow + row_begin_global);
             const uint32_t c1 = c1base | (uint32_t)(grow >> 32);
             if (!lambda_zero && valid) {
                 uint32_t w[4 * NOCT];
@@ -178,7 +187,8 @@
                                                            long long slots, long long rep0, int first_slot, int group,
                                                            uint32_t k0, uint32_t k1,
                                                            const long long* __restrict__ colsum, int* __restrict__ flags,
-                                                           long long n_global, long long row_begin_global) {
+                                                           long long n_global, long long row_begin_global,
+                                                           const int32_t* __restrict__ inv_perm) {
     const long long slot = first_slot + blockIdx.x;
     if (slot >= slots) return;
     const long long need = n_global - colsum[slot];
@@ -190,23 +200,25 @@
         const Philox4 r = philox4x32_10((uint32_t)j, c1base | (uint32_t)((unsigned long long)j >> 32), (uint32_t)rep,
                                         STREAM_FIXUP ^ (uint32_t)((unsigned long long)rep >> 32), k0, k1);
         const unsigned long long U = ((unsigned long long)r.x << 32) | r.y;
-        const long long row = (long long)__umul64hi(U, (unsigned long long)n_global) - row_begin_global;
+        long long row = (long long)__umul64hi(U, (unsigned long long)n_global) - row_begin_global;
         if (row < 0 || row >= n) continue;
+        if (inv_perm) { row = inv_perm[row]; GRAM_CHECK(row >= 0 && row < n_pad); }
         if (bump_count<CountT>(C, (panel * n_pad + row) * BM + col)) atomicOr(&flags[1], 1);
     }
 }
 
 template <typename CountT>
-__global__ void __launch_bounds__(256) counts_point_kernel(CountT* __restrict__ C, long long n) {
+__global__ void __launch_bounds__(256) counts_point_kernel(CountT* __restrict__ C, long long n, const int32_t* __restrict__ inv_perm) {
     const long long i = (long long)blockIdx.x * blockDim.x + threadIdx.x;
-    if (i < n) C[i * BM] = 1;
+    if (i < n) C[(inv_perm ? (long long)inv_perm[i] : i) * BM] = 1;
 }
 
 template <typename CountT>
 __global__ void __launch_bounds__(256) counts_index_kernel(CountT* __restrict__ C, long long n, long long n_pad,
                                                            long long r0, int first_slot,
                                                            const uint32_t* __restrict__ idx, int* __restrict__ flags,
-                                                           long long n_global, long long row_begin_global) {
+                                                           long long n_global, long long row_begin_global,
+                                                           const int32_t* __restrict__ inv_perm) {
     const long long r = r0 + blockIdx.y;
     const long long slot = first_slot + r, panel = slot / BM, col = slot % BM;
     for (long long i = (long long)blockIdx.x * blockDim.x + threadIdx.x; i < n_global; i += (long long)gridDim.x * blockDim.x) {
@@ -214,6 +226,7 @@
         if (row >= n_global) { atomicOr(&flags[2], 1); continue; }
         row -= row_begin_global;
         if (row < 0 || row >= n) continue;
+        if (inv_perm) { row = inv_perm[row]; GRAM_CHECK(row >= 0 && row < n_pad); }
         if (bump_count<CountT>(C, (panel * n_pad + row) * BM + col)) atomicOr(&flags[1], 1);
     }
 }
@@ -308,8 +321,8 @@
     const int pbg = (int)std::max<long long>((a.n_global + 255) / 256, 1);
     const long long reps = a.slots - a.first_slot;
     if (a.first_slot == 1 && pb > 0) {
-        if (a.count_bytes == 1) counts_point_kernel<uint8_t><<<pb, 256, 0, st>>>((uint8_t*)a.C, a.n);
-        else counts_point_kernel<uint16_t><<<pb, 256, 0, st>>>((uint16_t*)a.C, a.n);
+        if (a.count_bytes == 1) counts_point_kernel<uint8_t><<<pb, 256, 0, st>>>((uint8_t*)a.C, a.n, a.inv_perm);
+        else counts_point_kernel<uint16_t><<<pb, 256, 0, st>>>((uint16_t*)a.C, a.n, a.inv_perm);
         OB_CUDA(cudaGetLastError());
     }
     for (long long done = 0; done < reps; done += 32768) {
@@ -317,10 +330,10 @@
         dim3 grid((unsigned)std::min<long long>(pbg, 1024), (unsigned)nb);
         if (a.count_bytes == 1)
             counts_index_kernel<uint8_t><<<grid, 256, 0, st>>>((uint8_t*)a.C, a.n, a.n_pad, done, a.first_slot, d_idx, d_flags,
-                                                               a.n_global, a.row_begin);
+                                                               a.n_global, a.row_begin, a.inv_perm);
         else
             counts_index_kernel<uint16_t><<<grid, 256, 0, st>>>((uint16_t*)a.C, a.n, a.n_pad, done, a.first_slot, d_idx, d_flags,
-                                                                a.n_global, a.row_begin);
+                                                                a.n_global, a.row_begin, a.inv_perm);
         OB_CUDA(cudaGetLastError());
     }
 }
@@ -356,7 +369,7 @@
     auto body = [&](auto ct) {
         using CT = decltype(ct);
 #define OB_BODY(SHV) counts_philox_body<CT, SHV><<<grid, 256, 0, st>>>((CT*)a.C, a.n, a.n_pad, a.slots, a.rep0, \
-            a.first_slot, a.group, k0, k1, tab.lambda_zero, d_lut, d_colsum, rows_per_block, a.row_begin)
+            a.first_slot, a.group, k0, k1, tab.lambda_zero, d_lut, d_colsum, rows_per_block, a.row_begin, a.perm)
         switch (sh) {
         case 0: OB_BODY(0); break; case 1: OB_BODY(1); break; case 2: OB_BODY(2); break; case 3: OB_BODY(3); break;
         case 4: OB_BODY(4); break; case 5: OB_BODY(5); break; case 6: OB_BODY(6); break; default: OB_BODY(7);
@@ -374,10 +387,10 @@
     dim3 fgrid((unsigned)nrep, 16);
     if (a.count_bytes == 1)
         counts_philox_fixup<uint8_t><<<fgrid, 256, 0, st>>>((uint8_t*)a.C, a.n, a.n_pad, a.slots, a.rep0, a.first_slot,
-                                                            a.group, k0, k1, d_colsum, d_flags, a.n_global, a.row_begin);
+                                                            a.group, k0, k1, d_colsum, d_flags, a.n_global, a.row_begin, a.inv_perm);
     else
         counts_philox_fixup<uint16_t><<<fgrid, 256, 0, st>>>((uint16_t*)a.C, a.n, a.n_pad, a.slots, a.rep0, a.first_slot,
-                                                             a.group, k0, k1, d_colsum, d_flags, a.n_global, a.row_begin);
+                                                             a.group, k0, k1, d_colsum, d_flags, a.n_global, a.row_begin, a.inv_perm);
     OB_CUDA(cudaGetLastError());
 }
 
```

Result: faster. 1530, median of 6 (+22.7%).
